# Mak-GIBA/research_image_retrieval

Measured on AMD Instinct MI355X. Metric: images embedded+ranked/sec on 1.6M×2048 gallery; mAP on ROxf/RPar, higher is better.
Workload: dtype fp32

## Files before the change

include/rr.h:

```cpp
#ifndef RR_H_
#define RR_H_

#include <stddef.h>
#include <stdint.h>

#ifdef __cplusplus
extern "C" {
#endif

#define RR_OK 0
#define RR_EINVAL (-1)
#define RR_EHIP (-2)
#define RR_EWORKSPACE (-3)
#define RR_EOVERFLOW (-4)

#define RR_AMAX_SLOTS 64

typedef struct rr_handle_s* rr_handle_t;

#define RR_ABI_VERSION 7
int rr_abi_version(void);

const char* rr_version(void);
int rr_create(int device, rr_handle_t* out);
int rr_destroy(rr_handle_t h);
const char* rr_last_error(rr_handle_t h);

int rr_timing_enable(rr_handle_t h, int enable);
int rr_timing_collect(rr_handle_t h, int cls, double* ms, long long* launches);

int rr_get_device(rr_handle_t h, int* device);

#define RR_TUNE_GEMM_CFG 1
#define RR_TUNE_GEMM_BK 2
#define RR_TUNE_LP_CFG 3
#define RR_TUNE_S3_CFG 4
#define RR_TUNE_S3_STAGGER 5
#define RR_TUNE_SWEEP_MF16 8
#define RR_TUNE_SWEEP_IL 9
#define RR_TUNE_CONV_IL 10
#define RR_TUNE_HALO_MF 11
#define RR_TUNE_S3_CFG_RES 13
#define RR_TUNE_SWEEP_FORM 14
#define RR_TUNE_HALO_2D 15
int rr_set_tuning(rr_handle_t h, int key, int value);

size_t rr_cosine_topk_workspace_size(int nq, long long n, int d, int k);
size_t rr_cosine_topk_workspace_size_cap(int nq, long long n, int d, int k, long long cap);
long long rr_cosine_topk_cap_for(int nq, long long n, int d, int k, size_t workspace_bytes);
size_t rr_cosine_topk_counts_offset(int nq, long long n, int d, int k);
size_t rr_cosine_topk_overflow_offset(int nq, long long n, int d, int k);
int rr_cosine_topk(rr_handle_t h, const float* queries, int nq,
                   const float* gallery, long long n, int d, int k,
                   long long idx_offset, float* out_scores, long long* out_idx,
                   void* workspace, size_t workspace_bytes, void* stream);

int rr_cosine_scores(rr_handle_t h, const float* queries, int nq,
                     const float* gallery, long long n, int d, float* scores,
                     void* stream);

int rr_topk_merge(rr_handle_t h, const float* part_scores,
                  const long long* part_idx, int nparts, int nq, int k_in,
                  int k_out, float* out_scores, long long* out_idx,
                  void* stream);

int rr_quantize_rows(rr_handle_t h, const float* x, long long rows, int d,
                     int dtype, void* y, float* row_scale, void* stream);

int rr_cosine_topk_lp(rr_handle_t h, const void* queries, const float* q_scale,
                      int nq, const void* gallery, const float* g_scale,
                      long long n, int d, int dtype, int k, long long idx_offset,
                      float* out_scores, long long* out_idx, void* workspace,
                      size_t workspace_bytes, void* stream);

int rr_alpha_qe(rr_handle_t h, const float* queries, int nq,
                const float* gallery, long long n_rows, int d, const long long* top_idx,
                const float* top_scores, int k, int n, float alpha,
                long long idx_offset, float* out, void* stream);

int rr_prefilter_gallery_bound(rr_handle_t h, const float* gallery,
                               const void* gallery_bf16, long long n, int d,
                               double* bound3, void* stream);
size_t rr_cosine_topk_prefilter_workspace_size(int nq, long long n, int d, int k);
size_t rr_cosine_topk_prefilter_counts_offset(int nq, long long n, int d, int k);
size_t rr_cosine_topk_prefilter_overflow_offset(int nq, long long n, int d, int k);
size_t rr_cosine_topk_prefilter_workspace_size_cap(int nq, long long n, int d, int k, long long cap);
long long rr_cosine_topk_prefilter_cap_for(int nq, long long n, int d, int k, size_t workspace_bytes);
int rr_cosine_topk_prefilter(rr_handle_t h, const float* queries, int nq,
                             const float* gallery, const void* gallery_bf16,
                             const double* bound3, long long n, int d, int k,
                             long long idx_offset, float* out_scores,
                             long long* out_idx, void* workspace,
                             size_t workspace_bytes, void* stream);

size_t rr_pcaw_gram_workspace_size(long long n, int d);
int rr_pcaw_gram(rr_handle_t h, const float* x, long long n, int d,
                 void* workspace, size_t workspace_bytes, double* mean_out,
                 double* gram_out, void* stream);

int rr_preprocess_u8(rr_handle_t h, const uint8_t* img_nhwc, int b, int hgt,
                     int wid, const float* mean3, const float* std3,
                     float* out_nhwc, void* stream);

int rr_preprocess_u8_ex(rr_handle_t h, const uint8_t* img_nhwc, int b, int hgt,
                        int wid, const float* mean3, const float* std3,
                        int out_c, float* out_nhwc, void* stream);

int rr_nchw_to_nhwc(rr_handle_t h, const float* in, int b, int c, int hgt,
                    int wid, float* out, void* stream);
int rr_nchw_to_nhwc_ex(rr_handle_t h, const float* in, int b, int c, int hgt,
                       int wid, int out_c, float* out, void* stream);

int rr_conv2d(rr_handle_t h, const float* x, int b, int hgt, int wid, int cin,
              const float* w, const float* bias, int cout, int kh, int kw,
              int stride, int pad, const float* residual, int relu, float* y,
              void* stream);

int rr_resize_bilinear(rr_handle_t h, const float* x, int b, int hgt, int wid,
                       int c, int out_h, int out_w, float inv_scale_h,
                       float inv_scale_w, float* y, void* stream);

int rr_conv2d_h2(rr_handle_t h, const float* x, const unsigned* x_amax, int b,
                 int hgt, int wid, int cin, const void* w2,
                 const float* w_iscale, const float* bias, int cout, int kh,
                 int kw, int stride, int pad, const float* residual, int relu,
                 float* y, unsigned* y_amax, void* stream);

int rr_bottleneck_out_h2(rr_handle_t h, const float* y, const unsigned* y_amax,
                         int b, int oh, int ow, int planes, const float* x,
                         const unsigned* x_amax, int hx, int wx, int cin,
                         int stride, const void* w2, const float* w_iscale,
                         const float* bias, int cout, float* out,
                         unsigned* out_amax, void* stream);

int rr_stem_pool_h2(rr_handle_t h, const float* x, const unsigned* x_amax,
                    int b, int hgt, int wid, const void* w2,
                    const float* w_iscale, const float* bias, int cout, int kh,
                    int kw, int stride, int pad, float* y_pool,
                    unsigned* y_amax, void* stream);

int rr_split2_f16(rr_handle_t h, const float* w, int rows, int k, int kpad,
                  void* planes, float* iscale, void* stream);

int rr_amax_f32(rr_handle_t h, const float* x, long long n, unsigned* amax,
                void* stream);

int rr_maxpool2d(rr_handle_t h, const float* x, int b, int hgt, int wid, int c,
                 int k, int stride, int pad, float* y, void* stream);

int rr_gem_pool(rr_handle_t h, const float* x, int b, int hw, int c, float p,
                float eps, float* out, void* stream);

int rr_linear(rr_handle_t h, const float* x, int m, int k, const float* w,
              const float* bias, int n, float* y, void* stream);

int rr_linear_ex(rr_handle_t h, const float* x, int m, int k, const float* w,
                 const float* bias, int n, const float* residual, int act,
                 float* y, void* stream);

int rr_linear_bf16(rr_handle_t h, const void* x, int m, int k, const void* w,
                   const float* bias, int n, const float* residual, int act,
                   int out_bf16, void* y, void* stream);

int rr_linear_bf16_ln(rr_handle_t h, const void* x, int m, int k, const void* w,
                      const float* bias, int n, const float* residual, int act,
                      int out_bf16, void* y, const float* stats_in,
                      const float* colsum, float eps, float* stats_out,
                      void* xb_out, void* stream);

int rr_ln_partials_bf16(rr_handle_t h, const float* x, int m, int d, void* xb,
                        float* stats, void* stream);

int rr_layernorm(rr_handle_t h, const float* x, long long ldx, int m, int d,
                 const float* gamma, const float* beta, float eps, float* y,
                 void* stream);

int rr_layernorm_ex(rr_handle_t h, const float* x, long long ldx, int m, int d,
                    const float* gamma, const float* beta, float eps,
                    int out_dtype, void* y, void* stream);

int rr_patchify(rr_handle_t h, const float* x, int b, int hgt, int wid, int c,
                int patch, float* y, void* stream);

int rr_patchify_ex(rr_handle_t h, const float* x, int b, int hgt, int wid,
                   int c, int patch, int out_dtype, void* y, void* stream);

int rr_vit_tokens(rr_handle_t h, const float* patches, int b, int npatch,
                  int width, const float* cls, const float* pos, float* y,
                  void* stream);

int rr_vit_tokens_ex(rr_handle_t h, const float* patches, int b, int npatch,
                     int width, const float* cls, const float* pos,
                     const float* gamma, const float* beta, float eps,
                     float* y, void* stream);

int rr_attention(rr_handle_t h, const float* qkv, int b, int seq, int heads,
                 int head_dim, float* out, void* stream);
int rr_attention_ex(rr_handle_t h, const float* qkv, int b, int seq, int heads,
                    int head_dim, int out_dtype, void* out, void* stream);

int rr_attention_bf16(rr_handle_t h, const float* qkv, int b, int seq, int heads,
                      int head_dim, int out_dtype, void* out, void* stream);
int rr_attention_bf16_qkv16(rr_handle_t h, const void* qkv_bf16, int b, int seq,
                            int heads, int head_dim, int out_dtype, void* out,
                            void* stream);

int rr_l2_normalize(rr_handle_t h, const float* x, int m, int d, float eps,
                    float* y, void* stream);

int rr_dolg_local_pool(rr_handle_t h, const float* y, int b, int hw, int c,
                       const float* w2, float b2, float* out, void* stream);

int rr_dolg_orth_fuse(rr_handle_t h, const float* fg, const float* m, int b,
                      int c, float* out, void* stream);

#ifdef __cplusplus
}
#endif
#endif
```

research_image_retrieval_amd/_lib.py:

```python
import ctypes
import os
import subprocess
import threading

_HERE = os.path.dirname(os.path.abspath(__file__))
LIB_PATH = os.environ.get("RR_LIB_PATH") or os.path.join(_HERE, "librr.so")
CSRC = os.path.join(_HERE, "csrc")

RR_OK, RR_EINVAL, RR_EHIP, RR_EWORKSPACE, RR_EOVERFLOW = 0, -1, -2, -3, -4
ABI_VERSION = 7
AMAX_SLOTS = 64

TIME_COSINE, TIME_GEMM, TIME_SELECT, TIME_ELEM, TIME_COSINE_SEED, TIME_ATTN = 0, 1, 2, 3, 4, 5
TUNE_GEMM_CFG, TUNE_GEMM_BK, TUNE_LP_CFG, TUNE_S3_CFG, TUNE_S3_STAGGER, \
    TUNE_SWEEP_MF16, TUNE_SWEEP_IL, TUNE_CONV_IL, TUNE_HALO_MF, TUNE_S3_CFG_RES, TUNE_SWEEP_FORM, TUNE_HALO_2D = \
    1, 2, 3, 4, 5, 8, 9, 10, 11, 13, 14, 15

_lib = None
_lock = threading.RLock()

_vp = ctypes.c_void_p
_i = ctypes.c_int
_ll = ctypes.c_longlong
_f = ctypes.c_float
_sz = ctypes.c_size_t

SIGNATURES = {
    "rr_version": (ctypes.c_char_p, []),
    "rr_abi_version": (_i, []),
    "rr_create": (_i, [_i, ctypes.POINTER(_vp)]),
    "rr_destroy": (_i, [_vp]),
    "rr_last_error": (ctypes.c_char_p, [_vp]),
    "rr_timing_enable": (_i, [_vp, _i]),
    "rr_timing_collect": (_i, [_vp, _i, ctypes.POINTER(ctypes.c_double), ctypes.POINTER(_ll)]),
    "rr_get_device": (_i, [_vp, ctypes.POINTER(_i)]),
    "rr_set_tuning": (_i, [_vp, _i, _i]),
    "rr_cosine_topk_workspace_size": (_sz, [_i, _ll, _i, _i]),
    "rr_cosine_topk_workspace_size_cap": (_sz, [_i, _ll, _i, _i, _ll]),
    "rr_cosine_topk_cap_for": (_ll, [_i, _ll, _i, _i, _sz]),
    "rr_cosine_topk_counts_offset": (_sz, [_i, _ll, _i, _i]),
    "rr_cosine_topk_overflow_offset": (_sz, [_i, _ll, _i, _i]),
    "rr_cosine_topk": (_i, [_vp, _vp, _i, _vp, _ll, _i, _i, _ll, _vp, _vp, _vp, _sz, _vp]),
    "rr_cosine_scores": (_i, [_vp, _vp, _i, _vp, _ll, _i, _vp, _vp]),
    "rr_topk_merge": (_i, [_vp, _vp, _vp, _i, _i, _i, _i, _vp, _vp, _vp]),
    "rr_preprocess_u8": (_i, [_vp, _vp, _i, _i, _i, _vp, _vp, _vp, _vp]),
    "rr_nchw_to_nhwc": (_i, [_vp, _vp, _i, _i, _i, _i, _vp, _vp]),
    "rr_preprocess_u8_ex": (_i, [_vp, _vp, _i, _i, _i, _vp, _vp, _i, _vp, _vp]),
    "rr_nchw_to_nhwc_ex": (_i, [_vp, _vp, _i, _i, _i, _i, _i, _vp, _vp]),
    "rr_conv2d": (_i, [_vp, _vp, _i, _i, _i, _i, _vp, _vp, _i, _i, _i, _i, _i, _vp, _i, _vp, _vp]),
    "rr_conv2d_h2": (_i, [_vp, _vp, _vp, _i, _i, _i, _i, _vp, _vp, _vp, _i, _i, _i, _i, _i, _vp, _i, _vp, _vp, _vp]),
    "rr_split2_f16": (_i, [_vp, _vp, _i, _i, _i, _vp, _vp, _vp]),
    "rr_stem_pool_h2": (_i, [_vp, _vp, _vp, _i, _i, _i, _vp, _vp, _vp, _i, _i, _i, _i, _i, _vp, _vp, _vp]),
    "rr_bottleneck_out_h2": (_i, [_vp, _vp, _vp, _i, _i, _i, _i, _vp, _vp, _i, _i, _i, _i, _vp, _vp, _vp, _i, _vp,
                                  _vp, _vp]),
    "rr_amax_f32": (_i, [_vp, _vp, _ll, _vp, _vp]),
    "rr_resize_bilinear": (_i, [_vp, _vp, _i, _i, _i, _i, _i, _i, _f, _f, _vp, _vp]),
    "rr_maxpool2d": (_i, [_vp, _vp, _i, _i, _i, _i, _i, _i, _i, _vp, _vp]),
    "rr_gem_pool": (_i, [_vp, _vp, _i, _i, _i, _f, _f, _vp, _vp]),
    "rr_linear": (_i, [_vp, _vp, _i, _i, _vp, _vp, _i, _vp, _vp]),
    "rr_l2_normalize": (_i, [_vp, _vp, _i, _i, _f, _vp, _vp]),
    "rr_dolg_local_pool": (_i, [_vp, _vp, _i, _i, _i, _vp, _f, _vp, _vp]),
    "rr_dolg_orth_fuse": (_i, [_vp, _vp, _vp, _i, _i, _vp, _vp]),
    "rr_linear_ex": (_i, [_vp, _vp, _i, _i, _vp, _vp, _i, _vp, _i, _vp, _vp]),
    "rr_layernorm": (_i, [_vp, _vp, _ll, _i, _i, _vp, _vp, _f, _vp, _vp]),
    "rr_patchify": (_i, [_vp, _vp, _i, _i, _i, _i, _i, _vp, _vp]),
    "rr_vit_tokens": (_i, [_vp, _vp, _i, _i, _i, _vp, _vp, _vp, _vp]),
    "rr_patchify_ex": (_i, [_vp, _vp, _i, _i, _i, _i, _i, _i, _vp, _vp]),
    "rr_vit_tokens_ex": (_i, [_vp, _vp, _i, _i, _i, _vp, _vp, _vp, _vp, _f, _vp, _vp]),
    "rr_attention": (_i, [_vp, _vp, _i, _i, _i, _i, _vp, _vp]),
    "rr_attention_ex": (_i, [_vp, _vp, _i, _i, _i, _i, _i, _vp, _vp]),
    "rr_attention_bf16": (_i, [_vp, _vp, _i, _i, _i, _i, _i, _vp, _vp]),
    "rr_attention_bf16_qkv16": (_i, [_vp, _vp, _i, _i, _i, _i, _i, _vp, _vp]),
    "rr_layernorm_ex": (_i, [_vp, _vp, _ll, _i, _i, _vp, _vp, _f, _i, _vp, _vp]),
    "rr_linear_bf16": (_i, [_vp, _vp, _i, _i, _vp, _vp, _i, _vp, _i, _i, _vp, _vp]),
    "rr_linear_bf16_ln": (_i, [_vp, _vp, _i, _i, _vp, _vp, _i, _vp, _i, _i, _vp, _vp, _vp, _f, _vp, _vp, _vp]),
    "rr_ln_partials_bf16": (_i, [_vp, _vp, _i, _i, _vp, _vp, _vp]),
    "rr_alpha_qe": (_i, [_vp, _vp, _i, _vp, _ll, _i, _vp, _vp, _i, _i, _f, _ll, _vp, _vp]),
    "rr_prefilter_gallery_bound": (_i, [_vp, _vp, _vp, _ll, _i, _vp, _vp]),
    "rr_cosine_topk_prefilter_workspace_size": (_sz, [_i, _ll, _i, _i]),
    "rr_cosine_topk_prefilter_counts_offset": (_sz, [_i, _ll, _i, _i]),
    "rr_cosine_topk_prefilter_overflow_offset": (_sz, [_i, _ll, _i, _i]),
    "rr_cosine_topk_prefilter_workspace_size_cap": (_sz, [_i, _ll, _i, _i, _ll]),
    "rr_cosine_topk_prefilter_cap_for": (_ll, [_i, _ll, _i, _i, _sz]),
    "rr_cosine_topk_prefilter": (_i, [_vp, _vp, _i, _vp, _vp, _vp, _ll, _i, _i, _ll, _vp, _vp, _vp, _sz, _vp]),
    "rr_pcaw_gram_workspace_size": (_sz, [_ll, _i]),
    "rr_pcaw_gram": (_i, [_vp, _vp, _ll, _i, _vp, _sz, _vp, _vp, _vp]),
    "rr_quantize_rows": (_i, [_vp, _vp, _ll, _i, _i, _vp, _vp, _vp]),
    "rr_cosine_topk_lp": (_i, [_vp, _vp, _vp, _i, _vp, _vp, _ll, _i, _i, _i, _ll, _vp, _vp, _vp, _sz, _vp]),
}


class RRError(RuntimeError):
    pass


def build(force=False):
    if force or not os.path.exists(LIB_PATH):
        subprocess.run(["make", "-s", "-C", CSRC, "-j4"], check=True)


def lib():
    global _lib
    if _lib is not None:
        return _lib
    with _lock:
        if _lib is None:
            if not os.path.exists(LIB_PATH):
                raise RRError(
                    f"librr.so not found at {LIB_PATH}: build it with `make -C {CSRC}` "
                    "(there is deliberately no CPU/eager fallback)")
            L = ctypes.CDLL(LIB_PATH)
            for name, (res, args) in SIGNATURES.items():
                if os.environ.get("RR_LIB_PATH") and not hasattr(L, name):
                    continue
                fn = getattr(L, name)
                fn.restype = res
                fn.argtypes = args
            if not os.environ.get("RR_LIB_PATH") and L.rr_abi_version() != ABI_VERSION:
                raise RRError(f"librr.so ABI {L.rr_abi_version()} != {ABI_VERSION} this binding was written "
                              f"against: rebuild it with `make -C {CSRC}`")
            _lib = L
    return _lib


_handles = {}


def handle(device_index):
    h = _handles.get(device_index)
    if h is None:
        with _lock:
            h = _handles.get(device_index)
            if h is None:
                out = _vp()
                rc = lib().rr_create(int(device_index), ctypes.byref(out))
                if rc != RR_OK:
                    raise RRError(f"rr_create(device={device_index}) failed with {rc}")
                h = out.value
                _handles[device_index] = h
    return h


def check(rc, h, what):
    if rc != RR_OK:
        msg = lib().rr_last_error(h)
        raise RRError(f"{what} failed ({rc}): {msg.decode() if msg else ''}")
```

research_image_retrieval_amd/csrc/embed_ops.hip:

```cpp
#include "rr_internal.hpp"

namespace rr {

__global__ void preprocess_u8_kernel(const uint8_t* __restrict__ in, long long n_px, float m0, float m1, float m2,
                                     float s0, float s1, float s2, int out_c, float* __restrict__ out) {
  const long long stride = (long long)gridDim.x * blockDim.x;
  for (long long p = (long long)blockIdx.x * blockDim.x + threadIdx.x; p < n_px; p += stride) {
    const uint8_t* px = in + p * 3;
    const float r = ((float)px[0] / 255.0f - m0) / s0;
    const float g = ((float)px[1] / 255.0f - m1) / s1;
    const float b = ((float)px[2] / 255.0f - m2) / s2;
    if (out_c == 4) {
      *reinterpret_cast<float4*>(out + p * 4) = make_float4(r, g, b, 0.f);
    } else {
      float* o = out + p * 3;
      o[0] = r;
      o[1] = g;
      o[2] = b;
    }
  }
}

__global__ void nchw_to_nhwc_kernel(const float* __restrict__ in, int C, int CO, long long HW, long long total,
                                    float* __restrict__ out) {
  const long long stride = (long long)gridDim.x * blockDim.x;
  for (long long o = (long long)blockIdx.x * blockDim.x + threadIdx.x; o < total; o += stride) {
    const int c = (int)(o % CO);
    const long long t = o / CO;
    const long long hw = t % HW;
    const long long b = t / HW;
    out[o] = c < C ? in[(b * C + c) * HW + hw] : 0.f;
  }
}

__global__ void resize_bilinear_kernel(const float* __restrict__ x, int B, int H, int W, int C, int OH, int OW,
                                       float sh, float sw, float* __restrict__ y) {
  const long long total = (long long)B * OH * OW * C;
  const long long gstride = (long long)gridDim.x * blockDim.x;
  for (long long o = (long long)blockIdx.x * blockDim.x + threadIdx.x; o < total; o += gstride) {
    const int c = (int)(o % C);
    long long t = o / C;
    const int ow = (int)(t % OW);
    t /= OW;
    const int oh = (int)(t % OH);
    const int b = (int)(t / OH);
    float rh = sh * ((float)oh + 0.5f) - 0.5f;
    float rw = sw * ((float)ow + 0.5f) - 0.5f;
    rh = rh < 0.f ? 0.f : rh;
    rw = rw < 0.f ? 0.f : rw;
    const int h0 = (int)rh, w0 = (int)rw;
    const int h1 = h0 + (h0 < H - 1 ? 1 : 0), w1 = w0 + (w0 < W - 1 ? 1 : 0);
    const float lh1 = fminf(fmaxf(rh - (float)h0, 0.f), 1.f), lw1 = fminf(fmaxf(rw - (float)w0, 0.f), 1.f);
    const float lh0 = 1.f - lh1, lw0 = 1.f - lw1;
    const float* xb = x + (long long)b * H * W * C + c;
    const float v00 = xb[((long long)h0 * W + w0) * C], v01 = xb[((long long)h0 * W + w1) * C];
    const float v10 = xb[((long long)h1 * W + w0) * C], v11 = xb[((long long)h1 * W + w1) * C];
    y[o] = (v00 * lw0 + v01 * lw1) * lh0 + (v10 * lw0 + v11 * lw1) * lh1;
  }
}

__global__ __launch_bounds__(256) void maxpool4_row_kernel(const float* __restrict__ x, int H, int W, int C, int k,
                                                           int stride, int pad, int OH, int OW, float* __restrict__ y) {
  const int C4 = C >> 2;
  const int row = blockIdx.x;
  const int b = row / OH, oh = row - b * OH;
  const float* xb = x + (long long)b * H * W * C;
  float* yr = y + (long long)row * OW * C;
  const int n = OW * C4;
  for (int o = threadIdx.x; o < n; o += blockDim.x) {
    const int ow = o / C4, c4 = o - ow * C4;
    float4 m = make_float4(-__builtin_inff(), -__builtin_inff(), -__builtin_inff(), -__builtin_inff());
    for (int dh = 0; dh < k; ++dh) {
      const int ih = oh * stride - pad + dh;
      if ((unsigned)ih >= (unsigned)H) continue;
      const float* xr = xb + (long long)ih * W * C + c4 * 4;
      for (int dw = 0; dw < k; ++dw) {
        const int iw = ow * stride - pad + dw;
        if ((unsigned)iw >= (unsigned)W) continue;
        const float4 v = *reinterpret_cast<const float4*>(xr + iw * C);
        m.x = fmaxf(m.x, v.x);
        m.y = fmaxf(m.y, v.y);
        m.z = fmaxf(m.z, v.z);
        m.w = fmaxf(m.w, v.w);
      }
    }
    *reinterpret_cast<float4*>(yr + o * 4) = m;
  }
}

typedef float mp_f32x4 __attribute__((ext_vector_type(4)));
__global__ __launch_bounds__(256) void maxpool3s2_kernel(const float* __restrict__ x, int H, int W, int C, int OH,
                                                         int OW, float* __restrict__ y) {
  const int C4 = C >> 2;
  const int OH2 = (OH + 1) >> 1, OW2 = (OW + 1) >> 1;
  const int b = blockIdx.x / OH2, oh0 = 2 * (blockIdx.x - b * OH2);
  const float* xb = x + (long long)b * H * W * C;
  float* yb = y + (long long)b * OH * OW * C;
  const float ninf = -__builtin_inff();
  const int n = OW2 * C4;
  for (int o = threadIdx.x; o < n; o += blockDim.x) {
    const int owp = o / C4, c4 = o - owp * C4;
    const int ow0 = 2 * owp;
    mp_f32x4 m[2][2];
#pragma unroll
    for (int r = 0; r < 2; ++r)
#pragma unroll
      for (int q = 0; q < 2; ++q) m[r][q] = mp_f32x4{ninf, ninf, ninf, ninf};
#pragma unroll
    for (int dr = 0; dr < 5; ++dr) {
      const int ih = 2 * oh0 - 1 + dr;
      if ((unsigned)ih >= (unsigned)H) continue;
      const float* xr = xb + (long long)ih * W * C + c4 * 4;
      mp_f32x4 col[5];
#pragma unroll
      for (int dc = 0; dc < 5; ++dc) {
        const int iw = 2 * ow0 - 1 + dc;
        col[dc] = (unsigned)iw < (unsigned)W ? *reinterpret_cast<const mp_f32x4*>(xr + iw * C) : mp_f32x4{ninf, ninf, ninf, ninf};
      }
      mp_f32x4 p0, p1;
#pragma unroll
      for (int e = 0; e < 4; ++e) {
        p0[e] = fmaxf(fmaxf(col[0][e], col[1][e]), col[2][e]);
        p1[e] = fmaxf(fmaxf(col[2][e], col[3][e]), col[4][e]);
      }
#pragma unroll
      for (int e = 0; e < 4; ++e) {
        if (dr <= 2) {
          m[0][0][e] = fmaxf(m[0][0][e], p0[e]);
          m[0][1][e] = fmaxf(m[0][1][e], p1[e]);
        }
        if (dr >= 2) {
          m[1][0][e] = fmaxf(m[1][0][e], p0[e]);
          m[1][1][e] = fmaxf(m[1][1][e], p1[e]);
        }
      }
    }
#pragma unroll
    for (int r = 0; r < 2; ++r) {
      if (oh0 + r >= OH) continue;
#pragma unroll
      for (int q = 0; q < 2; ++q) {
        if (ow0 + q >= OW) continue;
        *reinterpret_cast<mp_f32x4*>(yb + ((long long)(oh0 + r) * OW + ow0 + q) * C + c4 * 4) = m[r][q];
      }
    }
  }
}

__global__ void maxpool4_kernel(const float* __restrict__ x, int B, int H, int W, int C, int k, int stride, int pad,
                                int OH, int OW, float* __restrict__ y) {
  const int C4 = C >> 2;
  const long long total = (long long)B * OH * OW * C4;
  const long long gstride = (long long)gridDim.x * blockDim.x;
  for (long long o = (long long)blockIdx.x * blockDim.x + threadIdx.x; o < total; o += gstride) {
    const int c4 = (int)(o % C4);
    long long t = o / C4;
    const int ow = (int)(t % OW);
    t /= OW;
    const int oh = (int)(t % OH);
    const int b = (int)(t / OH);
    float4 m = make_float4(-__builtin_inff(), -__builtin_inff(), -__builtin_inff(), -__builtin_inff());
    for (int dh = 0; dh < k; ++dh) {
      const int ih = oh * stride - pad + dh;
      if ((unsigned)ih >= (unsigned)H) continue;
      for (int dw = 0; dw < k; ++dw) {
        const int iw = ow * stride - pad + dw;
        if ((unsigned)iw >= (unsigned)W) continue;
        const float4 v = *reinterpret_cast<const float4*>(x + (((long long)b * H + ih) * W + iw) * C + c4 * 4);
        m.x = fmaxf(m.x, v.x);
        m.y = fmaxf(m.y, v.y);
        m.z = fmaxf(m.z, v.z);
        m.w = fmaxf(m.w, v.w);
      }
    }
    *reinterpret_cast<float4*>(y + o * 4) = m;
  }
}

__global__ void maxpool_kernel(const float* __restrict__ x, int B, int H, int W, int C, int k, int stride, int pad,
                               int OH, int OW, float* __restrict__ y) {
  const long long total = (long long)B * OH * OW * C;
  const long long gstride = (long long)gridDim.x * blockDim.x;
  for (long long o = (long long)blockIdx.x * blockDim.x + threadIdx.x; o < total; o += gstride) {
    const int c = (int)(o % C);
    long long t = o / C;
    const int ow = (int)(t % OW);
    t /= OW;
    const int oh = (int)(t % OH);
    const int b = (int)(t / OH);
    float m = -__builtin_inff();
    for (int dh = 0; dh < k; ++dh) {
      const int ih = oh * stride - pad + dh;
      if ((unsigned)ih >= (unsigned)H) continue;
      for (int dw = 0; dw < k; ++dw) {
        const int iw = ow * stride - pad + dw;
        if ((unsigned)iw >= (unsigned)W) continue;
        m = fmaxf(m, x[(((long long)b * H + ih) * W + iw) * C + c]);
      }
    }
    y[o] = m;
  }
}

__global__ void gem_kernel(const float* __restrict__ x, int B, int HW, int C, float p, float eps, int p_is_3,
                           float* __restrict__ out) {
  const long long total = (long long)B * C;
  const long long gstride = (long long)gridDim.x * blockDim.x;
  const float inv_p = 1.0f / p;
  for (long long o = (long long)blockIdx.x * blockDim.x + threadIdx.x; o < total; o += gstride) {
    const int c = (int)(o % C);
    const long long b = o / C;
    const float* xp = x + b * (long long)HW * C + c;
    float acc = 0.f;
    for (int i = 0; i < HW; ++i) {
      const float v = fmaxf(xp[(long long)i * C], eps);
      acc += p_is_3 ? (v * v) * v : powf(v, p);
    }
    out[o] = powf(acc / (float)HW, inv_p);
  }
}

__global__ __launch_bounds__(256) void l2norm_kernel(const float* __restrict__ x, int M, int D, float eps,
                                                     float* __restrict__ y) {
  const int wave = (blockIdx.x * blockDim.x + threadIdx.x) >> 6;
  const int lane = threadIdx.x & 63;
  if (wave >= M) return;
  const float* xr = x + (long long)wave * D;
  float* yr = y + (long long)wave * D;
  float ss = 0.f;
  for (int i = lane; i < D; i += 64) ss = fmaf(xr[i], xr[i], ss);
#pragma unroll
  for (int off = 32; off > 0; off >>= 1) ss += __shfl_xor(ss, off, 64);
  const float nrm = fmaxf(sqrtf(ss), eps);
  for (int i = lane; i < D; i += 64) yr[i] = xr[i] / nrm;
}

static dim3 grid_for(long long n, int block) {
  long long g = (n + block - 1) / block;
  if (g > 256 * 16) g = 256 * 16;
  if (g < 1) g = 1;
  return dim3((unsigned)g);
}

}

using namespace rr;

extern "C" int rr_preprocess_u8(rr_handle_t h, const uint8_t* img, int b, int hgt, int wid, const float* mean3,
                                const float* std3, float* out, void* stream) {
  return rr_preprocess_u8_ex(h, img, b, hgt, wid, mean3, std3, 3, out, stream);
}

extern "C" int rr_preprocess_u8_ex(rr_handle_t h, const uint8_t* img, int b, int hgt, int wid, const float* mean3,
                                   const float* std3, int out_c, float* out, void* stream) {
  RR_ENTRY(h);
  if (!img || !out || !mean3 || !std3 || b < 0 || hgt < 0 || wid < 0 || (out_c != 3 && out_c != 4) ||
      (out_c == 4 && ((uintptr_t)out & 15)))
    return set_error(h, RR_EINVAL, "rr_preprocess_u8: bad argument (out_c 3 or 4, 16-B aligned out)");
  const long long npx = (long long)b * hgt * wid;
  if (npx == 0) return RR_OK;
  hipStream_t s = (hipStream_t)stream;
  TimedLaunch tl(h, kTimeElem, s);
  hipLaunchKernelGGL(preprocess_u8_kernel, grid_for(npx, 256), dim3(256), 0, s, img, npx, mean3[0], mean3[1],
                     mean3[2], std3[0], std3[1], std3[2], out_c, out);
  return check_hip(h, hipGetLastError(), "preprocess launch");
}

extern "C" int rr_nchw_to_nhwc(rr_handle_t h, const float* in, int b, int c, int hgt, int wid, float* out,
                               void* stream) {
  return rr_nchw_to_nhwc_ex(h, in, b, c, hgt, wid, c, out, stream);
}

extern "C" int rr_nchw_to_nhwc_ex(rr_handle_t h, const float* in, int b, int c, int hgt, int wid, int out_c,
                                  float* out, void* stream) {
  RR_ENTRY(h);
  if (!in || !out || b < 0 || c <= 0 || hgt < 0 || wid < 0 || out_c < c)
    return set_error(h, RR_EINVAL, "rr_nchw_to_nhwc: bad argument");
  const long long total = (long long)b * out_c * hgt * wid;
  if (total == 0) return RR_OK;
  hipStream_t s = (hipStream_t)stream;
  TimedLaunch tl(h, kTimeElem, s);
  hipLaunchKernelGGL(nchw_to_nhwc_kernel, grid_for(total, 256), dim3(256), 0, s, in, c, out_c, (long long)hgt * wid,
                     total, out);
  return check_hip(h, hipGetLastError(), "nchw_to_nhwc launch");
}

extern "C" int rr_maxpool2d(rr_handle_t h, const float* x, int b, int hgt, int wid, int c, int k, int stride, int pad,
                            float* y, void* stream) {
  RR_ENTRY(h);
  if (!x || !y || b < 0 || c <= 0 || k <= 0 || stride <= 0 || pad < 0 || 2 * pad > k)
    return set_error(h, RR_EINVAL, "rr_maxpool2d: bad argument");
  const int oh = (hgt + 2 * pad - k) / stride + 1, ow = (wid + 2 * pad - k) / stride + 1;
  if (oh <= 0 || ow <= 0) return set_error(h, RR_EINVAL, "rr_maxpool2d: empty output");
  const long long total = (long long)b * oh * ow * c;
  if (total == 0) return RR_OK;
  hipStream_t s = (hipStream_t)stream;
  TimedLaunch tl(h, kTimeElem, s);
  const bool vec = (c & 3) == 0 && ((uintptr_t)x & 15) == 0 && ((uintptr_t)y & 15) == 0;
  if (vec && k == 3 && stride == 2 && pad == 1 && (long long)b * ((oh + 1) / 2) <= 0x7fffffffLL &&
      (long long)wid * c < 0x7fffffffLL)
    hipLaunchKernelGGL(maxpool3s2_kernel, dim3((unsigned)((long long)b * ((oh + 1) / 2))), dim3(256), 0, s, x, hgt,
                       wid, c, oh, ow, y);
  else if (vec && (long long)b * oh <= 0x7fffffffLL && (long long)wid * c < 0x7fffffffLL)
    hipLaunchKernelGGL(maxpool4_row_kernel, dim3((unsigned)((long long)b * oh)), dim3(256), 0, s, x, hgt, wid, c, k,
                       stride, pad, oh, ow, y);
  else if (vec)
    hipLaunchKernelGGL(maxpool4_kernel, grid_for(total / 4, 256), dim3(256), 0, s, x, b, hgt, wid, c, k, stride, pad,
                       oh, ow, y);
  else
    hipLaunchKernelGGL(maxpool_kernel, grid_for(total, 256), dim3(256), 0, s, x, b, hgt, wid, c, k, stride, pad, oh,
                       ow, y);
  return check_hip(h, hipGetLastError(), "maxpool launch");
}

extern "C" int rr_gem_pool(rr_handle_t h, const float* x, int b, int hw, int c, float p, float eps, float* out,
                           void* stream) {
  RR_ENTRY(h);
  if (!x || !out || b < 0 || hw <= 0 || c <= 0 || !(p > 0.f)) return set_error(h, RR_EINVAL, "rr_gem_pool: bad argument");
  const long long total = (long long)b * c;
  if (total == 0) return RR_OK;
  hipStream_t s = (hipStream_t)stream;
  TimedLaunch tl(h, kTimeElem, s);
  hipLaunchKernelGGL(gem_kernel, grid_for(total, 256), dim3(256), 0, s, x, b, hw, c, p, eps, p == 3.0f ? 1 : 0, out);
  return check_hip(h, hipGetLastError(), "gem launch");
}

extern "C" int rr_l2_normalize(rr_handle_t h, const float* x, int m, int d, float eps, float* y, void* stream) {
  RR_ENTRY(h);
  if (!x || !y || m < 0 || d <= 0) return set_error(h, RR_EINVAL, "rr_l2_normalize: bad argument");
  if (m == 0) return RR_OK;
  hipStream_t s = (hipStream_t)stream;
  TimedLaunch tl(h, kTimeElem, s);
  const long long threads = (long long)m * 64;
  hipLaunchKernelGGL(l2norm_kernel, dim3((unsigned)((threads + 255) / 256)), dim3(256), 0, s, x, m, d, eps, y);
  return check_hip(h, hipGetLastError(), "l2norm launch");
}

extern "C" int rr_resize_bilinear(rr_handle_t h, const float* x, int b, int hgt, int wid, int c, int out_h, int out_w,
                                  float inv_scale_h, float inv_scale_w, float* y, void* stream) {
  RR_ENTRY(h);
  if (!x || !y || b < 0 || hgt <= 0 || wid <= 0 || c <= 0 || out_h <= 0 || out_w <= 0)
    return set_error(h, RR_EINVAL, "rr_resize_bilinear: bad argument");
  const float sh = inv_scale_h > 0.f ? inv_scale_h : (float)hgt / (float)out_h;
  const float sw = inv_scale_w > 0.f ? inv_scale_w : (float)wid / (float)out_w;
  const long long total = (long long)b * out_h * out_w * c;
  if (total == 0) return RR_OK;
  hipStream_t s = (hipStream_t)stream;
  TimedLaunch tl(h, kTimeElem, s);
  hipLaunchKernelGGL(resize_bilinear_kernel, grid_for(total, 256), dim3(256), 0, s, x, b, hgt, wid, c, out_h, out_w, sh,
                     sw, y);
  return check_hip(h, hipGetLastError(), "resize launch");
}

namespace rr {
__global__ __launch_bounds__(256) void alpha_qe_kernel(const float* __restrict__ q, const float* __restrict__ g,
                                                       const long long* __restrict__ idx,
                                                       const float* __restrict__ sc, int k, int n, int d,
                                                       float alpha, long long idx_offset, long long n_rows,
                                                       float* __restrict__ out) {
  __shared__ float red[256 / 64];
  const int qi = blockIdx.x;
  const int d4 = d >> 2;
  float ss = 0.f;
  for (int c = threadIdx.x; c < d4; c += 256) {
    float4 acc = reinterpret_cast<const float4*>(q + (long long)qi * d)[c];
    for (int r = 0; r < n; ++r) {
      const long long j = idx[(long long)qi * k + r] - idx_offset;
      if (j < 0 || j >= n_rows) continue;
      const float s = sc[(long long)qi * k + r];
      const float w = s > 0.f ? powf(s, alpha) : 0.f;
      const float4 v = reinterpret_cast<const float4*>(g + j * d)[c];
      acc.x = fmaf(w, v.x, acc.x);
      acc.y = fmaf(w, v.y, acc.y);
      acc.z = fmaf(w, v.z, acc.z);
      acc.w = fmaf(w, v.w, acc.w);
    }
    reinterpret_cast<float4*>(out + (long long)qi * d)[c] = acc;
    ss = fmaf(acc.x, acc.x, fmaf(acc.y, acc.y, fmaf(acc.z, acc.z, fmaf(acc.w, acc.w, ss))));
  }
#pragma unroll
  for (int off = 32; off > 0; off >>= 1) ss += __shfl_xor(ss, off, 64);
  if ((threadIdx.x & 63) == 0) red[threadIdx.x >> 6] = ss;
  __syncthreads();
  const float tot = red[0] + red[1] + red[2] + red[3];
  const float inv = 1.0f / fmaxf(sqrtf(tot), 1e-12f);
  for (int c = threadIdx.x; c < d4; c += 256) {
    float4 v = reinterpret_cast<float4*>(out + (long long)qi * d)[c];
    v.x *= inv;
    v.y *= inv;
    v.z *= inv;
    v.w *= inv;
    reinterpret_cast<float4*>(out + (long long)qi * d)[c] = v;
  }
}
}

extern "C" int rr_alpha_qe(rr_handle_t h, const float* queries, int nq, const float* gallery, long long n_rows,
                           int d, const long long* top_idx, const float* top_scores, int k, int n, float alpha,
                           long long idx_offset, float* out, void* stream) {
  RR_ENTRY(h);
  if (!queries || !top_idx || !top_scores || !out || nq < 0 || n_rows < 0 || (n_rows > 0 && !gallery) || d <= 0 ||
      (d & 3) || k <= 0 || n < 0 ||
      n > k || ((uintptr_t)queries & 15) || ((uintptr_t)gallery & 15) || ((uintptr_t)out & 15))
    return set_error(h, RR_EINVAL, "rr_alpha_qe: bad argument (d % 4 == 0, 0 <= n <= k, 16-B aligned rows)");
  if (nq == 0) return RR_OK;
  hipStream_t s = (hipStream_t)stream;
  TimedLaunch tl(h, kTimeElem, s);
  hipLaunchKernelGGL(alpha_qe_kernel, dim3((unsigned)nq), dim3(256), 0, s, queries, gallery, top_idx, top_scores, k,
                     n, d, alpha, idx_offset, n_rows, out);
  return check_hip(h, hipGetLastError(), "alpha_qe launch");
}
```

research_image_retrieval_amd/csrc/h2_dispatch.hip:

```cpp
#include <algorithm>

#include "gemm_epilogue.hpp"
#include "rr_internal.hpp"

namespace rr {

static int pick_s3(const GemmArgs& g, int forced) {
  if (forced >= 1 && forced <= 8) return forced;
  if ((g.N % 256) == 0) return 4;
  auto cost = [&](long long bm, long long bn, long long per_cu, double speed) {
    const long long slots = 256 * per_cu;
    const long long t = ((g.M + bm - 1) / bm) * ((g.N + bn - 1) / bn);
    return (double)((t + slots - 1) / slots) * bm * bn * per_cu / speed;
  };
  double best = cost(128, 128, 2, 1.0);
  int cfg = 1;
  if (cost(256, 128, 1, 1.15) < best) best = cost(256, 128, 1, 1.15), cfg = 3;
  if (cost(256, 64, 2, 1.0) < best) best = cost(256, 64, 2, 1.0), cfg = 7;
  return cfg;
}
static int pick_h2(const GemmArgs& g, int forced) {
  if (forced == 9) return (g.N % 256) == 0 ? 9 : pick_h2(g, 0);
  if (forced == 10) return (g.N % 256) == 0 ? 10 : pick_h2(g, 0);
  if (forced == 11) return (g.N % 128) == 0 ? 11 : pick_h2(g, 0);
  if (forced == 12) return (g.N % 256) == 0 ? 12 : pick_h2(g, 0);
  if (forced == 0 && g.N == 128) return 11;
  int cfg = pick_s3(g, forced);
  if (cfg == 3 || cfg == 4 || cfg == 7 || cfg == 8) return cfg;
  cfg = pick_s3(g, 0);
  if (cfg == 1) cfg = (g.N % 128) == 0 ? 3 : 7;
  return cfg;
}

static bool s3_persist_ok(const GemmArgs& g, int amode) { return (g.N % 256) == 0 && amode == A_DENSE; }

static hipError_t launch_h2_am(int am, const GemmArgs& g, hipStream_t s, int forced, int n_cu, int st) {
  const bool hpers = forced == 0;
  if (am == A_DENSE && (forced == 15 || forced == 0) && s3q_shape(g) && !s3q_fits(g)) {
    const long long per = ((1LL << 32) - 1) / (4LL * std::max(g.lda, g.ldc)) / 256 * 256;
    if (per >= 256) {
      for (long long m0 = 0; m0 < g.M; m0 += per) {
        GemmArgs c = g;
        c.M = (int)std::min<long long>(per, g.M - m0);
        c.A = g.A + m0 * g.lda;
        c.C = g.C + m0 * g.ldc;
        if (g.residual != nullptr) c.residual = g.residual + m0 * g.ldc;
        if (const hipError_t e = launch_h2_am(am, c, s, forced, n_cu, st)) return e;
      }
      return hipSuccess;
    }
  }
  if (forced == 15 || forced == 0) {
    if (am == A_DENSE && s3q_shape(g) && s3q_fits(g)) return launch_s3q(g, s, n_cu, st);
    if (forced == 15) forced = 0;
  }
  if (am == A_CONV) {
    if (forced == 0 && g.halo_2d != 0 && h2_halo_2d_ok(g) && (g.halo_2d == 1 || !h2_halo_rows(g)))
      return launch_h2_halo_2d(g, s);
    if (forced == 13 || forced == 14 || (forced == 0 && ((g.N % 256) == 0 || g.N == 64 || g.N == 128))) {
      if (const int hr = h2_halo_rows(g))
        return launch_h2_halo(g, s, hr,
                              forced == 14 ? 1 : forced == 13 ? 0 : g.halo_mf >= 0 ? g.halo_mf : (hr == 288 || hr == 320 ? 1 : 0),
                              hpers, n_cu);
    }
  }
  if (forced == 13 || forced == 14) forced = 0;
  int cfg = pick_h2(g, forced);
  const bool big = (g.N % 256) == 0 && g.K >= 256;
  if (forced == 0 && big) cfg = 12;
  else if (forced == 0 && s3_persist_ok(g, am)) cfg = 8;
  if (cfg == 8) {
    if (s3_persist_ok(g, am)) return launch_s3p(g, s, n_cu, st);
    cfg = pick_h2(g, 0);
  }
  return launch_h2_tile(cfg, am, g, s, n_cu, st);
}

int launch_gemm_s3(rr_handle_s* h, int amode, const GemmArgs& g, hipStream_t s, int timer_cls) {
  if (g.M < 0 || g.N <= 0 || g.K <= 0) return set_error(h, RR_EINVAL, "gemm_s3: bad shape");
  if (g.K % 32) return set_error(h, RR_EINVAL, "gemm_s3: K must be a multiple of 32");
  if (amode == A_DENSE && ((g.lda & 3) || ((uintptr_t)g.A & 15)))
    return set_error(h, RR_EINVAL, "gemm_s3: dense A needs lda % 4 == 0 and 16-B alignment");
  if (amode == A_CONV && (g.Cin % 32)) return set_error(h, RR_EINVAL, "gemm_s3: conv A needs Cin % 32 == 0");
  if (amode == A_CONV_C4 && (g.Cin != 4 || g.K < g.KH * g.KW * 4 || ((uintptr_t)g.A & 15)))
    return set_error(h, RR_EINVAL, "gemm_s3: NHWC4 A needs Cin == 4, K >= KH*KW*4, 16-B alignment");
  if (amode != A_DENSE && amode != A_CONV && amode != A_CONV_C4)
    return set_error(h, RR_EINVAL, "gemm_s3: unsupported A mode");
  if ((g.ldb & 7) || (g.b_plane & 7) || ((uintptr_t)g.B & 15))
    return set_error(h, RR_EINVAL, "gemm_s3: B planes need ldb % 8 == 0, plane stride % 8 == 0, 16-B alignment");
  if (g.col_scale == nullptr || g.a_amax == nullptr || ((uintptr_t)g.col_scale & 15))
    return set_error(h, RR_EINVAL, "gemm_h2: needs 16-B aligned column scales and the A max-|x| record");
  if (g.relu == 2 || g.out_bf16 || (g.N & 3) || (g.ldc & 3))
    return set_error(h, RR_EINVAL, "gemm_h2: fp32 output, ReLU or none, N % 4 == 0");
  if (g.M == 0) return RR_OK;
  const int st = h->tune.s3_stagger >= 0 ? h->tune.s3_stagger : (g.residual != nullptr ? 8 : 0);
  hipError_t e;
  {
    TimedLaunch tl(h, timer_cls, s);
    const int f = (g.residual != nullptr && h->tune.s3_cfg_res > 0) ? h->tune.s3_cfg_res : h->tune.s3_cfg;
    const int n_cu = device_cu_count(h);
    {
      GemmArgs g2 = g;
      g2.issue_spread = h->tune.conv_il == 1;
      g2.halo_mf = h->tune.halo_mf;
      g2.halo_2d = h->tune.halo_2d;
      e = launch_h2_am(amode, g2, s, f, n_cu, st);
    }
  }
  return check_hip(h, e, "gemm_h2 launch");
}

__global__ __launch_bounds__(256) void split2h_kernel(const float* __restrict__ w, int rows, int k, int kpad,
                                                      uint16_t* __restrict__ planes, float* __restrict__ iscale) {
  __shared__ float red[4];
  const int n = blockIdx.x, tid = threadIdx.x;
  const float* wr = w + (long long)n * k;
  float am = 0.f;
  for (int i = tid; i < k; i += 256) am = amax_acc(am, wr[i]);
#pragma unroll
  for (int o = 32; o > 0; o >>= 1) am = fmaxf(am, __shfl_xor(am, o));
  if ((tid & 63) == 0) red[tid >> 6] = am;
  __syncthreads();
  am = fmaxf(fmaxf(red[0], red[1]), fmaxf(red[2], red[3]));
  const int e = h2_exp(am);
  const float sc = __builtin_amdgcn_ldexpf(1.f, e);
  if (tid == 0) iscale[n] = __builtin_amdgcn_ldexpf(1.f, -e);
  const long long plane = (long long)rows * kpad;
  uint16_t* p0 = planes + (long long)n * kpad;
  for (int i = tid; i < kpad; i += 256) {
    const float v = i < k ? wr[i] * sc : 0.f;
    const _Float16 hi = (_Float16)v;
    const _Float16 lo = (_Float16)(v - (float)hi);
    p0[i] = __builtin_bit_cast(uint16_t, hi);
    p0[plane + i] = __builtin_bit_cast(uint16_t, lo);
  }
}

int launch_split2h(rr_handle_s* h, const float* w, int rows, int k, int kpad, uint16_t* planes, float* iscale,
                   hipStream_t s) {
  if (rows <= 0) return RR_OK;
  hipLaunchKernelGGL(split2h_kernel, dim3((unsigned)rows), dim3(256), 0, s, w, rows, k, kpad, planes, iscale);
  return check_hip(h, hipGetLastError(), "split2h launch");
}

__global__ __launch_bounds__(256) void amax_kernel(const float* __restrict__ x, long long n, uint32_t* slots) {
  float am = 0.f;
  const long long gs = (long long)gridDim.x * blockDim.x;
  const long long i0 = (long long)blockIdx.x * blockDim.x + threadIdx.x;
  if (((uintptr_t)x & 15) == 0) {
    const long long n4 = n >> 2;
    const f32x4* x4 = reinterpret_cast<const f32x4*>(x);
    for (long long i = i0; i < n4; i += gs) {
      const f32x4 v = x4[i];
      am = amax_acc(amax_acc(am, v[0]), v[1]);
      am = amax_acc(amax_acc(am, v[2]), v[3]);
    }
    for (long long i = (n4 << 2) + i0; i < n; i += gs) am = amax_acc(am, x[i]);
  } else {
    for (long long i = i0; i < n; i += gs) am = amax_acc(am, x[i]);
  }
  amax_publish(slots, am, blockIdx.x * 4 + (threadIdx.x >> 6));
}

int launch_amax(rr_handle_s* h, const float* x, long long n, uint32_t* slots, hipStream_t s) {
  if (n <= 0) return RR_OK;
  const long long blocks = std::min<long long>((n / 4 + 255) / 256 + 1, 2048);
  hipLaunchKernelGGL(amax_kernel, dim3((unsigned)blocks), dim3(256), 0, s, x, n, slots);
  return check_hip(h, hipGetLastError(), "amax launch");
}

#if RR_S3_PHASES
int h2_tile_phases(unsigned long long* out);
int h2_stream_phases(unsigned long long* out);
int h2_stream256_phases(unsigned long long* out);
int h2_halo_phases(unsigned long long* out);
#endif

}

#if RR_S3_PHASES
extern "C" int rr_debug_phases(unsigned long long* out) {
  if (const int e = rr::h2_tile_phases(out)) return e;
  if (const int e = rr::h2_stream_phases(out + 8)) return e;
  if (const int e = rr::h2_stream256_phases(out + 16)) return e;
  return rr::h2_halo_phases(out + 24);
}
#endif
```

research_image_retrieval_amd/csrc/h2_stem.hip:

```cpp
#include <algorithm>

#include "h2_common.hpp"

namespace rr {

template <int EPI, int NW = 8, int BREG = 0>
__global__ __launch_bounds__(64 * NW, 1) void stem_pool_halo_kernel(GemmArgs g, int ntiles) {
  constexpr int NT = 64 * NW, BN = 64, HR = 39, HC = 35, HP = HR * HC;
  constexpr int WR = BREG ? 64 : 256 / NW, FM = WR / 32;
  constexpr int JN = BREG ? 1 : 2;
  static_assert(NW == 8 || (NW == 4 && !BREG), "8 waves of 32 rows or 4 of 64");
  constexpr int HS = 36, HPS = HR * HS;
  constexpr int KP = 224, BS = KP + 8;
  constexpr int NKS = 13;
  constexpr int B_U16 = BREG == 1 ? 0 : 2 * BN * BS;
  constexpr int A_U16 = 2 * (HPS + 1) * 4;
  constexpr int CS = BN + 4;
  constexpr int C_U16 = 256 * CS * 2;
  constexpr int A_PASS = (HP + NT - 1) / NT;
  constexpr int C4 = BN / 4, NPOOL = 56 * C4;
  constexpr int QI = (NPOOL + NT - 1) / NT;
  constexpr int PS = NKS / QI;
  __shared__ __attribute__((aligned(16))) uint16_t lds[B_U16 + A_U16 + C_U16];
  uint16_t* lb = lds;
  uint16_t* la = lds + B_U16;
  float* ct = reinterpret_cast<float*>(lds + B_U16 + A_U16);
  typedef f16x8 frag_t;
  typedef _Float16 f16x4 __attribute__((ext_vector_type(4)));

  const int tid = threadIdx.x, lane = tid & 63, wave = tid >> 6;
  const int lr = lane & 31, lh = lane >> 5;
  const int wrg = BREG ? wave % 4 : wave, wn = BREG ? wave / 4 : 0;
  const uint32_t a_amax_w = amax_load_slot(g.a_amax);
  float a_sc, a_isc;
  {
    uint32_t u = a_amax_w;
    const int lo = s3_opaque(lane);
#pragma unroll
    for (int o = 32; o > 0; o >>= 1) {
      const uint32_t v = (uint32_t)__builtin_amdgcn_ds_bpermute((lo ^ o) << 2, (int)u);
      u = v > u ? v : u;
    }
    const int e = __builtin_amdgcn_readfirstlane(h2_exp(__uint_as_float(u)));
    a_sc = __int_as_float((127 + e) << 23);
    a_isc = __int_as_float((127 - e) << 23);
  }

  constexpr int BRP = BREG == 1 ? 2 : 1;
  frag_t breg[BREG ? NKS : 1][BRP];
  if constexpr (BREG != 0) {
    const uint16_t* Bp = reinterpret_cast<const uint16_t*>(g.B) + (long long)(32 * wn + lr) * g.ldb + 8 * lh;
#pragma unroll
    for (int ks = 0; ks < NKS; ++ks)
#pragma unroll
      for (int p = 0; p < BRP; ++p) breg[ks][p] = *reinterpret_cast<const frag_t*>(Bp + p * g.b_plane + 16 * ks);
  }
  if constexpr (BREG != 1) {
    const uint16_t* Bp = reinterpret_cast<const uint16_t*>(g.B);
    for (int i = tid; i < 2 * BN * (KP / 8); i += NT) {
      const int row = i / (KP / 8), c8 = i - row * (KP / 8);
      const int p = row / BN, n = row - p * BN;
      *reinterpret_cast<u32x4*>(lb + row * BS + c8 * 8) =
          *reinterpret_cast<const u32x4*>(Bp + p * g.b_plane + (long long)n * g.ldb + c8 * 8);
    }
  }

  const int tpi = g.pool_tr * g.pool_tc;
  f32x4 px[A_PASS];
  auto load_patch = [&](int tl) {
    const int b = tl / tpi, t2 = tl - b * tpi, pr = t2 / g.pool_tc, pc = t2 - pr * g.pool_tc;
#pragma unroll
    for (int q = 0; q < A_PASS; ++q) {
      const int p = tid + q * NT, hr = p / HC, hc = p - hr * HC;
      const int ih = 32 * pr - 5 + hr, iw = 28 * pc - 5 + hc;
      const bool ok = tl < ntiles && p < HP && (unsigned)ih < (unsigned)g.H && (unsigned)iw < (unsigned)g.W;
      const f32x4* src = ok ? reinterpret_cast<const f32x4*>(g.A + (((long long)b * g.H + ih) * g.W + iw) * 4)
                            : s3_zero_page();
      asm volatile("global_load_dwordx4 %0, %1, off" : "=&v"(px[q]) : "v"(src) : "memory");
    }
  };
  auto store_patch = [&]() {
    asm volatile("s_waitcnt vmcnt(0)" ::: "memory");
#pragma unroll
    for (int q = 0; q < A_PASS; ++q) {
      asm volatile("" : "+v"(px[q]));
      const int p = tid + q * NT, hr = p / HC, hc = p - hr * HC;
      const int slot = hr * HS + (hc & 1) * (HS / 2) + (hc >> 1);
      const f32x4 v = px[q] * a_sc;
      const f16x4 hi = __builtin_convertvector(v, f16x4);
      const f16x4 lo = __builtin_convertvector(v - __builtin_convertvector(hi, f32x4), f16x4);
      if (p < HP) {
        *reinterpret_cast<f16x4*>(la + slot * 4) = hi;
        *reinterpret_cast<f16x4*>(la + (HPS + 1) * 4 + slot * 4) = lo;
      }
    }
    if (tid < 2) *reinterpret_cast<uint2*>(la + tid * (HPS + 1) * 4 + HPS * 4) = uint2{0u, 0u};
  };

  int sbase[FM];
#pragma unroll
  for (int i = 0; i < FM; ++i) {
    const int row = wrg * WR + 32 * i + lr, rq = row / 15, rc = row - rq * 15;
    sbase[i] = row < 255 ? (2 * rq) * HS + rc : -1;
  }

  float am = 0.f;
  auto pool_item = [&](int tl, int it) __attribute__((always_inline)) {
    const int b = tl / tpi, t2 = tl - b * tpi, pr = t2 / g.pool_tc, pc = t2 - pr * g.pool_tc;
    const int qd = it / C4, c4 = it - qd * C4, pi = qd / 7, pj = qd - 7 * pi;
    const int ph = 8 * pr + pi, pw = 7 * pc + pj;
    if (ph >= g.POH || pw >= g.POW) return;
    f32x4 mx = {-__builtin_inff(), -__builtin_inff(), -__builtin_inff(), -__builtin_inff()};
#pragma unroll
    for (int dr = -1; dr <= 1; ++dr)
#pragma unroll
      for (int dc = -1; dc <= 1; ++dc) {
        const int oh = 2 * ph + dr, ow = 2 * pw + dc;
        if ((unsigned)oh >= (unsigned)g.OH || (unsigned)ow >= (unsigned)g.OW) continue;
        const f32x4 v = *reinterpret_cast<const f32x4*>(ct + ((2 * pi + dr + 1) * 15 + 2 * pj + dc + 1) * CS + c4 * 4);
#pragma unroll
        for (int e = 0; e < 4; ++e) mx[e] = __builtin_fmaxf(mx[e], v[e]);
      }
    const f32x4 sc = *reinterpret_cast<const f32x4*>(g.col_scale + c4 * 4) * a_isc;
    const f32x4 bv = g.bias != nullptr ? *reinterpret_cast<const f32x4*>(g.bias + c4 * 4) : f32x4{0.f, 0.f, 0.f, 0.f};
    f32x4 o;
#pragma unroll
    for (int e = 0; e < 4; ++e) {
      o[e] = __builtin_fmaxf(mx[e] * sc[e] + bv[e], 0.f);
      am = amax_acc(am, o[e]);
    }
    *reinterpret_cast<f32x4*>(g.pool_out + (((long long)b * g.POH + ph) * g.POW + pw) * BN + c4 * 4) = o;
  };

  const int G = gridDim.x;
  int tl = blockIdx.x;
  int prev = -1;
  load_patch(tl);
  store_patch();
  __syncthreads();
  for (; tl < ntiles; tl += G) {
    load_patch(tl + G);
    f32x16 hi[FM][JN], lo[FM][JN];
#pragma unroll
    for (int i = 0; i < FM; ++i)
#pragma unroll
      for (int j = 0; j < JN; ++j)
#pragma unroll
        for (int r = 0; r < 16; ++r) hi[i][j][r] = lo[i][j][r] = 0.f;
#pragma unroll
    for (int ks = 0; ks < NKS; ++ks) {
      frag_t a[2][FM], b[2][2];
      const int t0 = 4 * ks + 2 * lh;
#pragma unroll
      for (int i = 0; i < FM; ++i) {
        int pix[2];
#pragma unroll
        for (int u = 0; u < 2; ++u) {
          const int t = t0 + u, kh = t / 7, kw = t - kh * 7;
          pix[u] = (sbase[i] >= 0 && t < 49) ? sbase[i] + kh * HS + (kw & 1) * (HS / 2) + (kw >> 1) : HPS;
        }
#pragma unroll
        for (int p = 0; p < 2; ++p) {
          const uint16_t* pl = la + p * (HPS + 1) * 4;
          const f16x4 x0 = *reinterpret_cast<const f16x4*>(pl + pix[0] * 4);
          const f16x4 x1 = *reinterpret_cast<const f16x4*>(pl + pix[1] * 4);
          a[p][i] = __builtin_shufflevector(x0, x1, 0, 1, 2, 3, 4, 5, 6, 7);
        }
      }
#pragma unroll
      for (int p = 0; p < 2; ++p)
#pragma unroll
        for (int j = 0; j < JN; ++j)
          b[p][j] = (BREG == 1 || (BREG == 2 && p == 0))
                        ? breg[ks][BREG == 1 ? p : 0]
                        : *reinterpret_cast<const frag_t*>(lb + (p * BN + 32 * (j + wn) + lr) * BS + 16 * ks + 8 * lh);
#pragma unroll
      for (int i = 0; i < FM; ++i)
#pragma unroll
        for (int j = 0; j < JN; ++j) hi[i][j] = s3_mf32(a[0][i], b[0][j], hi[i][j]);
#pragma unroll
      for (int i = 0; i < FM; ++i)
#pragma unroll
        for (int j = 0; j < JN; ++j) {
          lo[i][j] = s3_mf32(a[0][i], b[1][j], lo[i][j]);
          lo[i][j] = s3_mf32(a[1][i], b[0][j], lo[i][j]);
        }
      if (prev >= 0) {
#pragma unroll
        for (int q = 0; q < QI; ++q)
          if (ks == q * PS + PS / 2 && tid + q * NT < NPOOL) pool_item(prev, tid + q * NT);
      }
    }
    __syncthreads();
#pragma unroll
    for (int i = 0; i < FM; ++i)
#pragma unroll
      for (int j = 0; j < JN; ++j)
#pragma unroll
        for (int r = 0; r < 16; ++r)
          ct[(wrg * WR + 32 * i + acc_row<false>(0, r, lane)) * CS + 32 * wn + acc_col<false>(j, r, lane)] =
              hi[i][j][r] + lo[i][j][r];
    store_patch();
    prev = tl;
    __syncthreads();
  }
  if (prev >= 0) {
#pragma unroll
    for (int q = 0; q < QI; ++q)
      if (tid + q * NT < NPOOL) pool_item(prev, tid + q * NT);
  }
  asm volatile("s_waitcnt vmcnt(0)" ::: "memory");
  if constexpr ((EPI & EP_AMAX) != 0) {
    if (g.c_amax != nullptr) amax_publish(g.c_amax, am, blockIdx.x * NW + wave);
  }
}

int launch_stem_pool_h2(rr_handle_s* h, const GemmArgs& g, hipStream_t s, int timer_cls) {
  if (g.N != 64 || g.Cin != 4 || g.K % 32 || g.K < g.KH * g.KW * 4 || g.relu != 1 || g.residual != nullptr ||
      g.col_scale == nullptr || g.a_amax == nullptr || g.pool_out == nullptr || g.POH <= 0 || g.POW <= 0 ||
      g.pool_tr != (g.POH + 7) / 8 || g.pool_tc != (g.POW + 6) / 7 || ((uintptr_t)g.A & 15) || (g.ldb & 7) ||
      (g.b_plane & 7) || ((uintptr_t)g.B & 15) || ((uintptr_t)g.col_scale & 15) || ((uintptr_t)g.pool_out & 15))
    return set_error(h, RR_EINVAL, "stem_pool_h2: NHWC4 input, 64 output channels, ReLU, aligned operands");
  GemmArgs q = g;
  const long long tiles = (long long)(g.M / ((long long)g.OH * g.OW)) * g.pool_tr * g.pool_tc;
  if (tiles * 256 > 0x7fffffffLL) return set_error(h, RR_EINVAL, "stem_pool_h2: too many tiles");
  if (tiles == 0) return RR_OK;
  q.M = (int)(tiles * 256);
  hipError_t e;
  {
    TimedLaunch tl(h, timer_cls, s);
    if (h->tune.s3_cfg != 7 && g.KH == 7 && g.KW == 7 && g.stride == 2 && g.pad == 3 && g.K == 224 && g.ldb == 224) {
      const int grid = (int)std::min<long long>(tiles, device_cu_count(h));
      hipLaunchKernelGGL((stem_pool_halo_kernel<H2_EP | EP_RELU, 8, 2>), dim3((unsigned)grid), dim3(512), 0, s, g, (int)tiles);
      e = hipGetLastError();
    } else {
      e = launch_h2_tile_stem_pool(q, s, device_cu_count(h));
    }
  }
  return check_hip(h, e, "stem_pool_h2 launch");
}

}
```

research_image_retrieval_amd/csrc/rr_api.hip:

```cpp
#include <algorithm>
#include <cstring>
#include <initializer_list>

#include "gemm_epilogue.hpp"
#include "rr_internal.hpp"

namespace rr {

int set_error(rr_handle_s* h, int code, const std::string& msg) {
  if (h) h->last_error = msg;
  return code;
}

int check_hip(rr_handle_s* h, hipError_t e, const char* what) {
  if (e == hipSuccess) return RR_OK;
  return set_error(h, RR_EHIP, std::string(what) + ": " + hipGetErrorString(e));
}

TimedLaunch::TimedLaunch(rr_handle_s* h_, int cls_, hipStream_t s_) : h(h_), cls(cls_), s(s_) {
  if (!h || !h->timing || cls < 0 || cls >= rr_handle_s::kClasses) return;
  const int i = h->n_ev[cls];
  if (i >= (int)h->ev_start[cls].size()) {
    hipEvent_t a = nullptr, b = nullptr;
    if (hipEventCreate(&a) != hipSuccess) return;
    if (hipEventCreate(&b) != hipSuccess) {
      (void)hipEventDestroy(a);
      return;
    }
    h->ev_start[cls].push_back(a);
    h->ev_stop[cls].push_back(b);
  }
  if (hipEventRecord(h->ev_start[cls][i], s) != hipSuccess) return;
  slot = i;
}

TimedLaunch::~TimedLaunch() {
  if (slot < 0) return;
  if (hipEventRecord(h->ev_stop[cls][slot], s) == hipSuccess) h->n_ev[cls] = slot + 1;
}

static long long seed_rows(long long n, int k) { return seed_sample_rows(n, k); }

static inline size_t align256(size_t x) { return (x + 255) & ~(size_t)255; }

struct TopkWs {
  long long s, ld, cap;
  size_t off_scores, off_tau, off_cnt, off_ovf, off_cand, total;
};

static TopkWs topk_layout(int nq, long long n, int k, long long cap = -1) {
  TopkWs w{};
  w.s = seed_rows(n, k);
  w.ld = (w.s + 3) & ~3LL;
  w.cap = k + (n - w.s);
  if (cap >= 0 && cap < w.cap) w.cap = cap;
  size_t o = 0;
  w.off_scores = o;
  o = align256(o + (size_t)nq * w.ld * 4);
  w.off_tau = o;
  o = align256(o + (size_t)nq * 4);
  w.off_cnt = o;
  o = align256(o + (size_t)nq * 4);
  w.off_ovf = o;
  o = align256(o + 4);
  w.off_cand = o;
  o = align256(o + (size_t)nq * w.cap * 8);
  w.total = o;
  return w;
}

}

using namespace rr;

extern "C" {

const char* rr_version(void) { return "librr 0.4.0 (gfx950: fp32 / f16x2 / bf16 / fp8 MFMA)"; }

int rr_abi_version(void) { return RR_ABI_VERSION; }

int rr_create(int device, rr_handle_t* out) {
  if (!out) return RR_EINVAL;
  *out = nullptr;
  int ndev = 0;
  if (hipGetDeviceCount(&ndev) != hipSuccess || device < 0 || device >= ndev) return RR_EHIP;
  rr_handle_s* h = new (std::nothrow) rr_handle_s();
  if (!h) return RR_EINVAL;
  h->device = device;
  *out = h;
  return RR_OK;
}

int rr_destroy(rr_handle_t h) {
  RR_ENTRY(h);
  for (int c = 0; c < rr_handle_s::kClasses; ++c)
    for (size_t i = 0; i < h->ev_start[c].size(); ++i) {
      (void)hipEventDestroy(h->ev_start[c][i]);
      (void)hipEventDestroy(h->ev_stop[c][i]);
    }
  dolg_slab_release(h);
  delete h;
  return RR_OK;
}

const char* rr_last_error(rr_handle_t h) { return h ? h->last_error.c_str() : "null handle"; }

int rr_timing_enable(rr_handle_t h, int enable) {
  RR_ENTRY(h);
  h->timing = enable != 0;
  for (int c = 0; c < rr_handle_s::kClasses; ++c) {
    h->n_ev[c] = 0;
    h->acc_ms[c] = 0;
    h->acc_launches[c] = 0;
  }
  return RR_OK;
}

int rr_get_device(rr_handle_t h, int* device) {
  if (!h || !device) return RR_EINVAL;
  *device = h->device;
  return RR_OK;
}

int rr_set_tuning(rr_handle_t h, int key, int value) {
  if (!h) return RR_EINVAL;
  auto in = [&](std::initializer_list<int> ok) {
    for (int v : ok)
      if (v == value) return true;
    return false;
  };
  switch (key) {
    case RR_TUNE_GEMM_CFG:
      if (!in({0, 22, 41, 88})) break;
      h->tune.gemm_cfg = value;
      return RR_OK;
    case RR_TUNE_GEMM_BK:
      if (!in({0, 16, 32})) break;
      h->tune.gemm_bk = value;
      return RR_OK;
    case RR_TUNE_LP_CFG:
      if (value < 0 || value > 6) break;
      h->tune.lp_cfg = value;
      return RR_OK;
    case RR_TUNE_S3_CFG:
      if (value < 0 || value > 15) break;
      h->tune.s3_cfg = value;
      return RR_OK;
    case RR_TUNE_S3_STAGGER:
      if (value < -1 || value > 200) break;
      h->tune.s3_stagger = value;
      return RR_OK;
    case RR_TUNE_SWEEP_MF16:
      if (!in({-1, 0, 1})) break;
      h->tune.sweep_mf16 = value;
      return RR_OK;
    case RR_TUNE_SWEEP_IL:
      if (!in({-1, 0, 1})) break;
      h->tune.sweep_il = value;
      return RR_OK;
    case RR_TUNE_CONV_IL:
      if (!in({-1, 0, 1})) break;
      h->tune.conv_il = value;
      return RR_OK;
    case RR_TUNE_HALO_MF:
      if (!in({-1, 0, 1, 2, 3, 4})) break;
      h->tune.halo_mf = value;
      return RR_OK;
    case RR_TUNE_S3_CFG_RES:
      if (value < 0 || value > 15) break;
      h->tune.s3_cfg_res = value;
      return RR_OK;
    case RR_TUNE_SWEEP_FORM:
      if (!in({-1, 0, 1, 2})) break;
      h->tune.sweep_form = value;
      return RR_OK;
    case RR_TUNE_HALO_2D:
      if (!in({-1, 0, 1})) break;
      h->tune.halo_2d = value;
      return RR_OK;
    default:
      return set_error(h, RR_EINVAL, "rr_set_tuning: unknown key");
  }
  return set_error(h, RR_EINVAL, "rr_set_tuning: value out of range for this key");
}

int rr_timing_collect(rr_handle_t h, int cls, double* ms, long long* launches) {
  if (!h || cls < 0 || cls >= rr_handle_s::kClasses) return RR_EINVAL;
  DeviceGuard dg(h);
  for (int i = 0; i < h->n_ev[cls]; ++i) {
    if (int rc = check_hip(h, hipEventSynchronize(h->ev_stop[cls][i]), "timing sync")) return rc;
    float t = 0.f;
    if (int rc = check_hip(h, hipEventElapsedTime(&t, h->ev_start[cls][i], h->ev_stop[cls][i]), "timing elapsed"))
      return rc;
    h->acc_ms[cls] += t;
    h->acc_launches[cls] += 1;
  }
  h->n_ev[cls] = 0;
  if (ms) *ms = h->acc_ms[cls];
  if (launches) *launches = h->acc_launches[cls];
  h->acc_ms[cls] = 0;
  h->acc_launches[cls] = 0;
  return RR_OK;
}

size_t rr_cosine_topk_workspace_size(int nq, long long n, int d, int k) {
  (void)d;
  if (nq <= 0 || k <= 0) return 256;
  return topk_layout(nq, n > 0 ? n : 1, k).total;
}

size_t rr_cosine_topk_workspace_size_cap(int nq, long long n, int d, int k, long long cap) {
  (void)d;
  if (nq <= 0 || k <= 0 || cap < k) return 0;
  return topk_layout(nq, n > 0 ? n : 1, k, cap).total;
}

long long rr_cosine_topk_cap_for(int nq, long long n, int d, int k, size_t workspace_bytes) {
  (void)d;
  if (nq <= 0 || k <= 0) return 0;
  const TopkWs L = topk_layout(nq, n > 0 ? n : 1, k);
  return workspace_bytes >= L.total ? L.cap : cap_that_fits(L.off_cand, nq, workspace_bytes, L.cap);
}

size_t rr_cosine_topk_counts_offset(int nq, long long n, int d, int k) {
  (void)d;
  if (nq <= 0 || k <= 0) return 0;
  return topk_layout(nq, n > 0 ? n : 1, k).off_cnt;
}

size_t rr_cosine_topk_overflow_offset(int nq, long long n, int d, int k) {
  (void)d;
  if (nq <= 0 || k <= 0) return 0;
  return topk_layout(nq, n > 0 ? n : 1, k).off_ovf;
}

}

namespace rr {
static int cosine_topk_impl(rr_handle_t h, const void* queries, const float* q_scale, int nq, const void* gallery,
                            const float* g_scale, long long n, int d, int k, long long idx_offset, float* out_scores,
                            long long* out_idx, void* workspace, size_t workspace_bytes, hipStream_t s, int dt) {
  if (nq < 0 || n < 0 || d <= 0 || (d & 3) || k < 1 || k > 16384)
    return set_error(h, RR_EINVAL, "rr_cosine_topk: need nq,n >= 0, d % 4 == 0, 1 <= k <= 16384");
  if (n >= 0xffffffffLL) return set_error(h, RR_EINVAL, "rr_cosine_topk: gallery shard must have < 2^32 rows");
  if (nq == 0) return RR_OK;
  if (!queries || !out_scores || !out_idx || (n > 0 && !gallery))
    return set_error(h, RR_EINVAL, "rr_cosine_topk: null pointer");
  if (((uintptr_t)queries & 15) || ((uintptr_t)gallery & 15))
    return set_error(h, RR_EINVAL, "rr_cosine_topk: queries/gallery must be 16-byte aligned");
  const int es = dt == DT_F32 ? 4 : (dt == DT_BF16 ? 2 : 1);
  TopkWs L = topk_layout(nq, n > 0 ? n : 1, k);
  if (workspace && workspace_bytes < L.total) {
    const long long cap = cap_that_fits(L.off_cand, nq, workspace_bytes, L.cap);
    if (cap >= k) L = topk_layout(nq, n > 0 ? n : 1, k, cap);
  }
  if (!workspace || workspace_bytes < L.total)
    return set_error(h, RR_EWORKSPACE,
                     "rr_cosine_topk: workspace too small (at least rr_cosine_topk_workspace_size_cap(..., k))");
  char* ws = (char*)workspace;
  float* scores_t = (float*)(ws + L.off_scores);
  float* tau = (float*)(ws + L.off_tau);
  int* cnt = (int*)(ws + L.off_cnt);
  int* ovf = (int*)(ws + L.off_ovf);
  unsigned long long* cand = (unsigned long long*)(ws + L.off_cand);
  if (int rc = check_hip(h, hipMemsetAsync(ovf, 0, 4, s), "memset")) return rc;
  if (n == 0) {
    if (int rc = check_hip(h, hipMemsetAsync(cnt, 0, (size_t)nq * 4, s), "memset")) return rc;
    return launch_select_final(h, cand, L.cap, cnt, nq, k, idx_offset, out_scores, out_idx, ovf, s);
  }
  GemmArgs g;
  g.A = (const float*)gallery;
  g.lda = d;
  g.M = (int)L.s;
  g.K = d;
  g.B = (const float*)queries;
  g.ldb = d;
  g.N = nq;
  g.C = scores_t;
  g.ldc = L.ld;
  g.scale_a = g_scale;
  g.scale_b = q_scale;
  if (int rc = launch_gemm(h, A_DENSE, E_SCORES_T, g, s, kTimeCosineSeed, dt)) return rc;
  if (int rc = launch_select_dense_seed(h, scores_t, L.ld, (int)L.s, nq, k, 0, cand, L.cap, cnt, tau, s)) return rc;
  long long done = L.s;
  while (done < n) {
    const long long rows = std::min<long long>(n - done, 0x7fffff00LL);
    GemmArgs f;
    f.A = (const float*)((const char*)gallery + done * d * es);
    f.lda = d;
    f.M = (int)rows;
    f.K = d;
    f.B = (const float*)queries;
    f.ldb = d;
    f.N = nq;
    f.tau = tau;
    f.cand = cand;
    f.cnt = cnt;
    f.cap = L.cap;
    f.row_offset = done;
    f.scale_a = g_scale ? g_scale + done : nullptr;
    f.scale_b = q_scale;
    if (int rc = launch_gemm(h, A_DENSE, E_FILTER, f, s, kTimeCosine, dt)) return rc;
    done += rows;
  }
  return launch_select_final(h, cand, L.cap, cnt, nq, k, idx_offset, out_scores, out_idx, ovf, s);
}
}

extern "C" {

int rr_cosine_topk(rr_handle_t h, const float* queries, int nq, const float* gallery, long long n, int d, int k,
                   long long idx_offset, float* out_scores, long long* out_idx, void* workspace,
                   size_t workspace_bytes, void* stream) {
  RR_ENTRY(h);
  return cosine_topk_impl(h, queries, nullptr, nq, gallery, nullptr, n, d, k, idx_offset, out_scores, out_idx,
                          workspace, workspace_bytes, (hipStream_t)stream, DT_F32);
}

int rr_cosine_topk_lp(rr_handle_t h, const void* queries, const float* q_scale, int nq, const void* gallery,
                      const float* g_scale, long long n, int d, int dtype, int k, long long idx_offset,
                      float* out_scores, long long* out_idx, void* workspace, size_t workspace_bytes,
                      void* stream) {
  RR_ENTRY(h);
  if (dtype != DT_BF16 && dtype != DT_FP8) return set_error(h, RR_EINVAL, "rr_cosine_topk_lp: dtype must be 1 or 2");
  if (dtype == DT_FP8 && (!q_scale || !g_scale))
    return set_error(h, RR_EINVAL, "rr_cosine_topk_lp: fp8 needs per-row scales");
  if ((d % (dtype == DT_BF16 ? 8 : 16)) != 0)
    return set_error(h, RR_EINVAL, "rr_cosine_topk_lp: rows must be multiples of 16 bytes");
  return cosine_topk_impl(h, queries, q_scale, nq, gallery, g_scale, n, d, k, idx_offset, out_scores, out_idx,
                          workspace, workspace_bytes, (hipStream_t)stream, dtype);
}

int rr_linear_bf16(rr_handle_t h, const void* x, int m, int k, const void* w, const float* bias, int n,
                   const float* residual, int act, int out_bf16, void* y, void* stream) {
  RR_ENTRY(h);
  if (!x || !w || !y || m < 0 || k <= 0 || n <= 0 || (k & 7) || act < 0 || act > 2)
    return set_error(h, RR_EINVAL, "rr_linear_bf16: bad argument (k % 8 == 0)");
  if (((uintptr_t)x & 15) || ((uintptr_t)w & 15)) return set_error(h, RR_EINVAL, "rr_linear_bf16: 16-B alignment");
  GemmArgs g;
  g.A = (const float*)x;
  g.lda = k;
  g.M = m;
  g.K = k;
  g.B = (const float*)w;
  g.ldb = k;
  g.N = n;
  g.C = (float*)y;
  g.ldc = n;
  g.bias = bias;
  g.residual = residual;
  g.relu = act;
  g.out_bf16 = out_bf16 ? 1 : 0;
  return launch_gemm(h, A_DENSE, E_STORE, g, (hipStream_t)stream, kTimeGemm, DT_BF16);
}

int rr_linear_bf16_ln(rr_handle_t h, const void* x, int m, int k, const void* w, const float* bias, int n,
                      const float* residual, int act, int out_bf16, void* y, const float* stats_in,
                      const float* colsum, float eps, float* stats_out, void* xb_out, void* stream) {
  RR_ENTRY(h);
  if (!x || !w || !y || m < 0 || k <= 0 || n <= 0 || (k & 7) || act < 0 || act > 2)
    return set_error(h, RR_EINVAL, "rr_linear_bf16_ln: bad argument (k % 8 == 0)");
  if (((uintptr_t)x & 15) || ((uintptr_t)w & 15) || ((uintptr_t)y & 15) || (bias && ((uintptr_t)bias & 15)) ||
      (residual && ((uintptr_t)residual & 15)))
    return set_error(h, RR_EINVAL, "rr_linear_bf16_ln: 16-B alignment");
  if ((stats_in == nullptr) == (stats_out == nullptr))
    return set_error(h, RR_EINVAL, "rr_linear_bf16_ln: exactly one of stats_in (fold) and stats_out (produce)");
  if (stats_out) {
    if (!xb_out || !residual || !bias || act != 0 || out_bf16 || (n % 256) || (k % 64) || ((uintptr_t)xb_out & 15) ||
        ((uintptr_t)stats_out & 7))
      return set_error(h, RR_EINVAL,
                       "rr_linear_bf16_ln: stats_out needs bias, residual, fp32 output, n % 256 == 0, k % 64 == 0");
  } else {
    if (!colsum || !bias || residual || !out_bf16 || (k % 64) || k > 256 * LN_TMAX || (n & 3) ||
        ((uintptr_t)colsum & 15) || !(eps >= 0.f))
      return set_error(h, RR_EINVAL,
                       "rr_linear_bf16_ln: stats_in needs colsum, bias, bf16 output, k % 64 == 0, k <= 768");
  }
  if (m == 0) return RR_OK;
  GemmArgs g;
  g.A = (const float*)x;
  g.lda = k;
  g.M = m;
  g.K = k;
  g.B = (const float*)w;
  g.ldb = k;
  g.N = n;
  g.C = (float*)y;
  g.ldc = n;
  g.bias = bias;
  g.residual = residual;
  g.relu = act;
  g.out_bf16 = out_bf16 ? 1 : 0;
  g.stats_out = stats_out;
  g.c2 = (uint16_t*)xb_out;
  g.stats_in = stats_in;
  g.colsum = colsum;
  g.stats_k = k;
  g.ln_eps = eps;
  return launch_gemm(h, A_DENSE, E_STORE, g, (hipStream_t)stream, kTimeGemm, DT_BF16);
}

int rr_cosine_scores(rr_handle_t h, const float* queries, int nq, const float* gallery, long long n, int d,
                     float* scores, void* stream) {
  RR_ENTRY(h);
  if (nq < 0 || n < 0 || n > 0x7fffffffLL || d <= 0 || (d & 3))
    return set_error(h, RR_EINVAL, "rr_cosine_scores: bad shape");
  if (nq == 0 || n == 0) return RR_OK;
  if (!queries || !gallery || !scores) return set_error(h, RR_EINVAL, "rr_cosine_scores: null pointer");
  GemmArgs g;
  g.A = gallery;
  g.lda = d;
  g.M = (int)n;
  g.K = d;
  g.B = queries;
  g.ldb = d;
  g.N = nq;
  g.C = scores;
  g.ldc = nq;
  return launch_gemm(h, A_DENSE, E_STORE, g, (hipStream_t)stream, kTimeCosineSeed);
}

int rr_topk_merge(rr_handle_t h, const float* ps, const long long* pi, int nparts, int nq, int k_in, int k_out,
                  float* os, long long* oi, void* stream) {
  RR_ENTRY(h);
  if (!ps || !pi || !os || !oi) return set_error(h, RR_EINVAL, "rr_topk_merge: null pointer");
  return launch_merge(h, ps, pi, nparts, nq, k_in, k_out, os, oi, (hipStream_t)stream);
}

int rr_conv2d(rr_handle_t h, const float* x, int b, int hgt, int wid, int cin, const float* w, const float* bias,
              int cout, int kh, int kw, int stride, int pad, const float* residual, int relu, float* y,
              void* stream) {
  RR_ENTRY(h);
  if (!x || !w || !y || b < 0 || hgt <= 0 || wid <= 0 || cin <= 0 || cout <= 0 || kh <= 0 || kw <= 0 ||
      stride <= 0 || pad < 0)
    return set_error(h, RR_EINVAL, "rr_conv2d: bad argument");
  const int oh = (hgt + 2 * pad - kh) / stride + 1, ow = (wid + 2 * pad - kw) / stride + 1;
  if (oh <= 0 || ow <= 0) return set_error(h, RR_EINVAL, "rr_conv2d: empty output");
  const long long M = (long long)b * oh * ow;
  if (M > 0x7fffffffLL) return set_error(h, RR_EINVAL, "rr_conv2d: too many output pixels");
  GemmArgs g;
  g.A = x;
  g.M = (int)M;
  g.K = kh * kw * cin;
  g.H = hgt;
  g.W = wid;
  g.Cin = cin;
  g.OH = oh;
  g.OW = ow;
  g.KH = kh;
  g.KW = kw;
  g.stride = stride;
  g.pad = pad;
  g.B = w;
  g.ldb = g.K;
  g.N = cout;
  g.C = y;
  g.ldc = cout;
  g.bias = bias;
  g.residual = residual;
  g.relu = relu;
  int amode;
  if (kh == 1 && kw == 1 && stride == 1 && pad == 0 && (cin & 3) == 0) {
    amode = A_DENSE;
    g.lda = cin;
  } else if (cin % 32 == 0) {
    amode = A_CONV;
  } else if (cin == 4) {
    amode = A_CONV_C4;
  } else {
    amode = A_CONV_GENERIC;
  }
  if (amode != A_CONV_GENERIC && (((uintptr_t)x & 15) || ((uintptr_t)w & 15)))
    return set_error(h, RR_EINVAL, "rr_conv2d: x/w must be 16-byte aligned");
  if ((cout & 3) == 0 && (((uintptr_t)y & 15) || (bias && ((uintptr_t)bias & 15)) || (residual && ((uintptr_t)residual & 15))))
    return set_error(h, RR_EINVAL, "rr_conv2d: bias/residual/y must be 16-byte aligned");
  return launch_gemm(h, amode, E_STORE, g, (hipStream_t)stream, kTimeGemm);
}

int rr_conv2d_h2(rr_handle_t h, const float* x, const unsigned* x_amax, int b, int hgt, int wid, int cin,
                 const void* w2, const float* w_iscale, const float* bias, int cout, int kh, int kw, int stride,
                 int pad, const float* residual, int relu, float* y, unsigned* y_amax, void* stream) {
  RR_ENTRY(h);
  if (!x || !x_amax || !w2 || !w_iscale || !y || b < 0 || hgt <= 0 || wid <= 0 || cin <= 0 || cout <= 0 ||
      kh <= 0 || kw <= 0 || stride <= 0 || pad < 0 || relu < 0 || relu > 1)
    return set_error(h, RR_EINVAL, "rr_conv2d_h2: bad argument");
  if (cin % 32 && cin != 4) return set_error(h, RR_EINVAL, "rr_conv2d_h2: cin must be a multiple of 32, or 4 (NHWC4 stem)");
  if (cout % 4) return set_error(h, RR_EINVAL, "rr_conv2d_h2: cout must be a multiple of 4");
  const int oh = (hgt + 2 * pad - kh) / stride + 1, ow = (wid + 2 * pad - kw) / stride + 1;
  if (oh <= 0 || ow <= 0) return set_error(h, RR_EINVAL, "rr_conv2d_h2: empty output");
  const long long M = (long long)b * oh * ow;
  if (M > 0x7fffffffLL) return set_error(h, RR_EINVAL, "rr_conv2d_h2: too many output pixels");
  if (((uintptr_t)x & 15) || ((uintptr_t)w2 & 15) || ((uintptr_t)w_iscale & 15) || ((uintptr_t)y & 15) ||
      (bias && ((uintptr_t)bias & 15)) || (residual && ((uintptr_t)residual & 15)))
    return set_error(h, RR_EINVAL, "rr_conv2d_h2: x/w2/w_iscale/bias/residual/y must be 16-byte aligned");
  GemmArgs g;
  g.A = x;
  g.M = (int)M;
  g.K = kh * kw * cin;
  g.H = hgt;
  g.W = wid;
  g.Cin = cin;
  g.OH = oh;
  g.OW = ow;
  g.KH = kh;
  g.KW = kw;
  g.stride = stride;
  g.pad = pad;
  if (cin == 4) g.K = (g.K + 31) / 32 * 32;
  g.B = reinterpret_cast<const float*>(w2);
  g.ldb = g.K;
  g.b_plane = (long long)cout * g.K;
  g.N = cout;
  g.C = y;
  g.ldc = cout;
  g.bias = bias;
  g.residual = residual;
  g.relu = relu;
  g.col_scale = w_iscale;
  g.a_amax = x_amax;
  g.c_amax = y_amax;
  const bool dense = kh == 1 && kw == 1 && stride == 1 && pad == 0 && cin != 4;
  if (dense) g.lda = cin;
  return launch_gemm_s3(h, dense ? A_DENSE : (cin == 4 ? A_CONV_C4 : A_CONV), g, (hipStream_t)stream, kTimeGemm);
}

int rr_stem_pool_h2(rr_handle_t h, const float* x, const unsigned* x_amax, int b, int hgt, int wid, const void* w2,
                    const float* w_iscale, const float* bias, int cout, int kh, int kw, int stride, int pad,
                    float* y_pool, unsigned* y_amax, void* stream) {
  RR_ENTRY(h);
  if (!x || !x_amax || !w2 || !w_iscale || !y_pool || b < 0 || hgt <= 0 || wid <= 0 || kh <= 0 || kw <= 0 ||
      stride <= 0 || pad < 0)
    return set_error(h, RR_EINVAL, "rr_stem_pool_h2: bad argument");
  if (cout != 64) return set_error(h, RR_EINVAL, "rr_stem_pool_h2: cout must be 64");
  const int oh = (hgt + 2 * pad - kh) / stride + 1, ow = (wid + 2 * pad - kw) / stride + 1;
  if (oh <= 0 || ow <= 0) return set_error(h, RR_EINVAL, "rr_stem_pool_h2: empty output");
  const int ph = (oh - 1) / 2 + 1, pw = (ow - 1) / 2 + 1;
  if ((long long)b * oh * ow > 0x7fffffffLL || (long long)b * ph * pw * cout > (1LL << 40))
    return set_error(h, RR_EINVAL, "rr_stem_pool_h2: too many output pixels");
  if (((uintptr_t)x & 15) || ((uintptr_t)w2 & 15) || ((uintptr_t)w_iscale & 15) || ((uintptr_t)y_pool & 15) ||
      (bias && ((uintptr_t)bias & 15)))
    return set_error(h, RR_EINVAL, "rr_stem_pool_h2: x/w2/w_iscale/bias/y_pool must be 16-byte aligned");
  GemmArgs g;
  g.A = x;
  g.M = (int)((long long)b * oh * ow);
  g.K = (kh * kw * 4 + 31) / 32 * 32;
  g.H = hgt;
  g.W = wid;
  g.Cin = 4;
  g.OH = oh;
  g.OW = ow;
  g.KH = kh;
  g.KW = kw;
  g.stride = stride;
  g.pad = pad;
  g.B = reinterpret_cast<const float*>(w2);
  g.ldb = g.K;
  g.b_plane = (long long)cout * g.K;
  g.N = cout;
  g.ldc = cout;
  g.bias = bias;
  g.relu = 1;
  g.col_scale = w_iscale;
  g.a_amax = x_amax;
  g.c_amax = y_amax;
  g.pool_out = y_pool;
  g.POH = ph;
  g.POW = pw;
  g.pool_tr = (ph + 7) / 8;
  g.pool_tc = (pw + 6) / 7;
  return launch_stem_pool_h2(h, g, (hipStream_t)stream, kTimeGemm);
}

int rr_bottleneck_out_h2(rr_handle_t h, const float* y, const unsigned* y_amax, int b, int oh, int ow, int planes,
                         const float* x, const unsigned* x_amax, int hx, int wx, int cin, int stride, const void* w2,
                         const float* w_iscale, const float* bias, int cout, float* out, unsigned* out_amax,
                         void* stream) {
  RR_ENTRY(h);
  if (!y || !y_amax || !x || !x_amax || !w2 || !w_iscale || !out || b < 0 || oh <= 0 || ow <= 0 || planes <= 0 ||
      hx <= 0 || wx <= 0 || cin <= 0 || stride <= 0 || cout <= 0)
    return set_error(h, RR_EINVAL, "rr_bottleneck_out_h2: bad argument");
  if ((planes % 32) || (cin % 32) || (cout % 256))
    return set_error(h, RR_EINVAL, "rr_bottleneck_out_h2: planes % 32, cin % 32 and cout % 256 must be 0");
  if ((long long)(oh - 1) * stride >= hx || (long long)(ow - 1) * stride >= wx)
    return set_error(h, RR_EINVAL, "rr_bottleneck_out_h2: the strided samples leave x");
  const long long M = (long long)b * oh * ow;
  if (M > 0x7fffffffLL || (long long)b * hx * wx > 0x7fffffffLL)
    return set_error(h, RR_EINVAL, "rr_bottleneck_out_h2: too many pixels");
  if (((uintptr_t)y & 15) || ((uintptr_t)x & 15) || ((uintptr_t)w2 & 15) || ((uintptr_t)w_iscale & 15) ||
      ((uintptr_t)out & 15) || (bias && ((uintptr_t)bias & 15)))
    return set_error(h, RR_EINVAL, "rr_bottleneck_out_h2: y/x/w2/w_iscale/bias/out must be 16-byte aligned");
  GemmArgs g;
  g.A = y;
  g.lda = planes;
  g.M = (int)M;
  g.K = planes + cin;
  g.K1 = planes;
  g.A2 = x;
  g.lda2 = cin;
  g.H2 = hx;
  g.W2 = wx;
  g.s2 = stride;
  g.OH = oh;
  g.OW = ow;
  g.B = reinterpret_cast<const float*>(w2);
  g.ldb = g.K;
  g.b_plane = (long long)cout * g.K;
  g.N = cout;
  g.C = out;
  g.ldc = cout;
  g.bias = bias;
  g.relu = 1;
  g.col_scale = w_iscale;
  g.a_amax = y_amax;
  g.a2_amax = x_amax;
  g.c_amax = out_amax;
  return launch_gemm_h2_seg2(h, g, (hipStream_t)stream, kTimeGemm);
}

int rr_split2_f16(rr_handle_t h, const float* w, int rows, int k, int kpad, void* planes, float* iscale,
                  void* stream) {
  RR_ENTRY(h);
  if (!w || !planes || !iscale || rows < 0 || k <= 0 || kpad < k) return set_error(h, RR_EINVAL, "rr_split2_f16: bad argument");
  TimedLaunch tl(h, kTimeElem, (hipStream_t)stream);
  return launch_split2h(h, w, rows, k, kpad, reinterpret_cast<uint16_t*>(planes), iscale, (hipStream_t)stream);
}

int rr_amax_f32(rr_handle_t h, const float* x, long long n, unsigned* amax, void* stream) {
  RR_ENTRY(h);
  if (!x || !amax || n < 0) return set_error(h, RR_EINVAL, "rr_amax_f32: bad argument");
  TimedLaunch tl(h, kTimeElem, (hipStream_t)stream);
  return launch_amax(h, x, n, amax, (hipStream_t)stream);
}


int rr_linear(rr_handle_t h, const float* x, int m, int k, const float* w, const float* bias, int n, float* y,
              void* stream) {
  return rr_linear_ex(h, x, m, k, w, bias, n, nullptr, 0, y, stream);
}

int rr_linear_ex(rr_handle_t h, const float* x, int m, int k, const float* w, const float* bias, int n,
                 const float* residual, int act, float* y, void* stream) {
  RR_ENTRY(h);
  if (!x || !w || !y || m < 0 || k <= 0 || n <= 0 || (k & 3)) return set_error(h, RR_EINVAL, "rr_linear: bad argument");
  if (((uintptr_t)x & 15) || ((uintptr_t)w & 15)) return set_error(h, RR_EINVAL, "rr_linear: x/w must be 16-byte aligned");
  GemmArgs g;
  g.A = x;
  g.lda = k;
  g.M = m;
  g.K = k;
  g.B = w;
  g.ldb = k;
  g.N = n;
  g.C = y;
  g.ldc = n;
  g.bias = bias;
  g.residual = residual;
  if (act < 0 || act > 2) return set_error(h, RR_EINVAL, "rr_linear_ex: act must be 0, 1 or 2");
  g.relu = act;
  return launch_gemm(h, A_DENSE, E_STORE, g, (hipStream_t)stream, kTimeGemm);
}

}
```

research_image_retrieval_amd/csrc/rr_internal.hpp:

```cpp
#pragma once

#include <type_traits>

#include <hip/hip_runtime.h>
#include <stdint.h>
#include <string>
#include <vector>

#include "../../include/rr.h"

struct rr_handle_s {
  int device = 0;
  std::string last_error;
  struct Tuning {
    int gemm_cfg = 0;
    int gemm_bk = 0;
    int lp_cfg = 0;
    int s3_cfg = 0;
    int s3_stagger = -1;
    int sweep_mf16 = -1;
    int sweep_il = -1;
    int conv_il = -1;
    int halo_mf = -1;
    int halo_2d = -1;
    int s3_cfg_res = 0;
    int sweep_form = -1;
  } tune;
  int n_cu = 0;
  bool timing = false;
  static constexpr int kClasses = 6;
  std::vector<hipEvent_t> ev_start[kClasses], ev_stop[kClasses];
  int n_ev[kClasses] = {};
  double acc_ms[kClasses] = {};
  long long acc_launches[kClasses] = {};
};

namespace rr {

struct DeviceGuard {
  int prev = -1;
  int rc = 0;
  explicit DeviceGuard(const rr_handle_s* h) {
    int cur = -1;
    if (hipGetDevice(&cur) != hipSuccess) {
      rc = RR_EHIP;
      return;
    }
    if (cur != h->device) {
      if (hipSetDevice(h->device) != hipSuccess) {
        rc = RR_EHIP;
        return;
      }
      prev = cur;
    }
  }
  ~DeviceGuard() {
    if (prev >= 0) (void)hipSetDevice(prev);
  }
};
#define RR_ENTRY(h)                                                                 \
  if (!(h)) return RR_EINVAL;                                                       \
  rr::DeviceGuard rr_device_guard_(h);                                              \
  if (rr_device_guard_.rc) return rr::set_error(h, rr_device_guard_.rc, "cannot select the handle's device")

enum TimerClass { kTimeCosine = 0, kTimeGemm = 1, kTimeSelect = 2, kTimeElem = 3, kTimeCosineSeed = 4, kTimeAttn = 5 };

struct TimedLaunch {
  rr_handle_s* h;
  int cls;
  hipStream_t s;
  int slot = -1;
  TimedLaunch(rr_handle_s* h_, int cls_, hipStream_t s_);
  ~TimedLaunch();
};

int set_error(rr_handle_s* h, int code, const std::string& msg);
int check_hip(rr_handle_s* h, hipError_t e, const char* what);

__host__ __device__ inline uint32_t ord_f32(float f) {
  uint32_t u;
  __builtin_memcpy(&u, &f, 4);
  if ((u & 0x7fffffffu) > 0x7f800000u) return 0u;
  if (u == 0x80000000u) u = 0u;
  return (u & 0x80000000u) ? ~u : (u | 0x80000000u);
}
__host__ __device__ inline float unord_f32(uint32_t o) {
  uint32_t u = (o & 0x80000000u) ? (o & 0x7fffffffu) : ~o;
  float f;
  __builtin_memcpy(&f, &u, 4);
  return f;
}
__host__ __device__ inline float next_down(float f) {
  uint32_t u;
  __builtin_memcpy(&u, &f, 4);
  if ((u & 0x7fffffffu) == 0) u = 0x80000001u;
  else if (u == 0xff800000u || (u & 0x7fffffffu) > 0x7f800000u) {
  } else if (u & 0x80000000u) ++u;
  else --u;
  __builtin_memcpy(&f, &u, 4);
  return f;
}
__host__ __device__ inline float next_up(float f) { return -next_down(-f); }
__host__ __device__ inline unsigned long long make_key(float s, uint32_t idx) {
  return ((unsigned long long)ord_f32(s) << 32) | (unsigned long long)(~idx);
}
__host__ __device__ inline uint32_t key_idx(unsigned long long k) {
  return ~(uint32_t)(k & 0xffffffffull);
}
__host__ __device__ inline float key_score(unsigned long long k) {
  return unord_f32((uint32_t)(k >> 32));
}

inline long long seed_sample_rows(long long n, int k) {
  long long s = n / 48;
  if (s > 32768) s = 32768;
  if (s < 4096) s = 4096;
  if (s < k) s = k;
  return n < s ? n : s;
}

inline int device_cu_count(rr_handle_s* h) {
  if (h->n_cu <= 0) {
    int v = 0;
    if (hipDeviceGetAttribute(&v, hipDeviceAttributeMultiprocessorCount, h->device) != hipSuccess || v <= 0) v = 256;
    h->n_cu = v;
  }
  return h->n_cu;
}

inline long long cap_that_fits(size_t off_cand, int nq, size_t bytes, long long worst) {
  const size_t usable = bytes & ~(size_t)255;
  if (nq <= 0 || usable <= off_cand) return 0;
  const long long cap = (long long)((usable - off_cand) / ((size_t)nq * 8));
  return cap < worst ? cap : worst;
}

enum AMode { A_DENSE = 0, A_CONV = 1, A_CONV_GENERIC = 2, A_CONV_C4 = 3 };
enum EMode { E_STORE = 0, E_SCORES_T = 1, E_FILTER = 2 };
enum DType { DT_F32 = 0, DT_BF16 = 1, DT_FP8 = 2 };

struct GemmArgs {
  const float* A = nullptr;
  long long lda = 0;
  int M = 0, K = 0;
  int H = 0, W = 0, Cin = 0, OH = 0, OW = 0, KH = 1, KW = 1, stride = 1, pad = 0;
  const float* B = nullptr;
  long long ldb = 0;
  int N = 0;
  float* C = nullptr;
  long long ldc = 0;
  const float* bias = nullptr;
  const float* residual = nullptr;
  int relu = 0;
  const float* tau = nullptr;
  unsigned long long* cand = nullptr;
  int* cnt = nullptr;
  long long cap = 0;
  long long row_offset = 0;
  const float* scale_a = nullptr;
  const float* scale_b = nullptr;
  int out_bf16 = 0;
  int k_split = 0;
  long long c_split_stride = 0;
  int sym = 0;
  long long b_plane = 0;
  const float* col_scale = nullptr;
  const uint32_t* a_amax = nullptr;
  uint32_t* c_amax = nullptr;
  int stagger_blocks = 0, stagger_sleeps = 0;
  const float* A2 = nullptr;
  long long lda2 = 0;
  int K1 = 0, H2 = 0, W2 = 0, s2 = 1;
  const uint32_t* a2_amax = nullptr;
  float* pool_out = nullptr;
  int POH = 0, POW = 0, pool_tr = 0, pool_tc = 0;
  uint16_t* c2 = nullptr;
  float* stats_out = nullptr;
  const float* stats_in = nullptr;
  const float* colsum = nullptr;
  int stats_k = 0;
  float ln_eps = 0.f;
  int mf16_sweep = 0;
  int issue_spread = 0;
  int halo_mf = -1;
  int halo_2d = -1;
};

__device__ __forceinline__ float wave_sum(float x) {
  auto shr = [](float v, auto ctrl) {
    return __int_as_float(__builtin_amdgcn_mov_dpp(__float_as_int(v), decltype(ctrl)::value, 0xf, 0xf, true));
  };
  x += shr(x, std::integral_constant<int, 0x111>{});
  x += shr(x, std::integral_constant<int, 0x112>{});
  x += shr(x, std::integral_constant<int, 0x114>{});
  x += shr(x, std::integral_constant<int, 0x118>{});
  const int xi = __float_as_int(x);
  return (__int_as_float(__builtin_amdgcn_readlane(xi, 15)) + __int_as_float(__builtin_amdgcn_readlane(xi, 31))) +
         (__int_as_float(__builtin_amdgcn_readlane(xi, 47)) + __int_as_float(__builtin_amdgcn_readlane(xi, 63)));
}

__device__ __forceinline__ void tile_coords(int bid, int nwg, int tiles_n, int& tm, int& tn) {
  const int xcd = bid & 7, q8 = nwg >> 3, r8 = nwg & 7;
  const int wgid = (xcd < r8 ? xcd * (q8 + 1) : r8 * (q8 + 1) + (xcd - r8) * q8) + (bid >> 3);
  tn = wgid % tiles_n;
  tm = wgid / tiles_n;
}

int launch_gemm(rr_handle_s* h, int amode, int emode, const GemmArgs& a, hipStream_t s, int timer_cls,
                int dt = DT_F32);

int launch_gemm_s3(rr_handle_s* h, int amode, const GemmArgs& g, hipStream_t s, int timer_cls);
hipError_t launch_h2_tile(int cfg, int amode, const GemmArgs& g, hipStream_t s, int n_cu, int st);
hipError_t launch_h2_tile_stem_pool(const GemmArgs& q, hipStream_t s, int n_cu);
hipError_t launch_s3p(const GemmArgs& g, hipStream_t s, int n_cu, int st);
bool s3q_shape(const GemmArgs& g);
bool s3q_fits(const GemmArgs& g);
hipError_t launch_s3q(const GemmArgs& g, hipStream_t s, int n_cu, int st);
int h2_halo_rows(const GemmArgs& g);
hipError_t launch_h2_halo(const GemmArgs& g, hipStream_t s, int hr, int mf, bool pers, int n_cu);
bool h2_halo_2d_ok(const GemmArgs& g);
hipError_t launch_h2_halo_2d(const GemmArgs& g, hipStream_t s);
int launch_gemm_h2_seg2(rr_handle_s* h, const GemmArgs& g, hipStream_t s, int timer_cls);
int launch_stem_pool_h2(rr_handle_s* h, const GemmArgs& g, hipStream_t s, int timer_cls);
int launch_split2h(rr_handle_s* h, const float* w, int rows, int k, int kpad, uint16_t* planes, float* iscale,
                   hipStream_t s);
int launch_amax(rr_handle_s* h, const float* x, long long n, uint32_t* slots, hipStream_t s);

bool gemm_8p_eligible(const GemmArgs& g, int dt);
hipError_t launch_gemm_8p(const GemmArgs& g, int emode, hipStream_t s, int dt);

int launch_select_dense_seed(rr_handle_s* h, const float* scores_t, long long ld, int rows, int nq,
                             int k, long long row_offset, unsigned long long* cand, long long cap,
                             int* cnt, float* tau, hipStream_t s);
int launch_select_final(rr_handle_s* h, const unsigned long long* cand, long long cap,
                        const int* cnt, int nq, int k, long long idx_offset, float* out_scores,
                        long long* out_idx, int* overflow_flag, hipStream_t s);
int launch_prefilter_rescore(rr_handle_s* h, unsigned long long* cand, long long cap, const int* cnt, int nq, int k,
                             const float* eps2, float* t2, const float* q, const float* g, int d, hipStream_t s);
int launch_merge(rr_handle_s* h, const float* ps, const long long* pi, int nparts, int nq, int kin,
                 int kout, float* os, long long* oi, hipStream_t s);

bool sweep16_eligible(const GemmArgs& g);
hipError_t launch_sweep16(const GemmArgs& g, hipStream_t s, int rows128);

bool lpp_eligible(const GemmArgs& g);
hipError_t launch_lpp(const GemmArgs& g, hipStream_t s, int n_cu);
bool lpp3_eligible(const GemmArgs& g);
hipError_t launch_lpp3(const GemmArgs& g, hipStream_t s, int n_cu);

void dolg_slab_release(rr_handle_s* h);

}
```

research_image_retrieval_amd/models.py:

```python
import torch

from . import ops
from . import weights as W
from .networks import ResNet, _Extractor, EPS_L2


class GeMPooling:

    def __init__(self, p=3.0, eps=1e-6):
        self.p = torch.ones(1) * p
        self.eps = eps

    def __call__(self, x_nhwc):
        return ops.gem_pool(x_nhwc, float(self.p.item()), self.eps)


class GeMModel(_Extractor):

    in_channels = 4

    def __init__(self, backbone="resnet50", pretrained=False, num_classes=1000, feature_dim=2048, gem_p=3.0,
                 state_dict=None, seed=0, device="cuda", conv_math="h2", stride_on="3x3"):
        if pretrained:
            raise ValueError("pretrained weights need a download; pass a local state_dict instead "
                             "(models/gem_pooling.py:35 defaults to pretrained=True)")
        if backbone not in ("resnet50", "resnet101"):
            raise ValueError(f"Unsupported backbone: {backbone}")
        self.device = torch.device(device)
        self.backbone = ResNet(backbone, state_dict, seed, device, conv_math=conv_math, stride_on=stride_on)
        self.gem_pool = GeMPooling(p=gem_p)
        backbone_dim = 2048
        pw, pb = _from_sd(state_dict, "feature_proj") or W.synthetic_linear(feature_dim, backbone_dim, seed + 2)
        self.proj_w = pw.float().contiguous().to(self.device)
        self.proj_b = pb.float().contiguous().to(self.device)
        cw, cb = _from_sd(state_dict, "classifier") or W.synthetic_linear(num_classes, feature_dim, seed + 3)
        self.cls_w = cw.float().contiguous().to(self.device)
        self.cls_b = cb.float().contiguous().to(self.device)
        self.feature_dim = feature_dim
        self.outputdim = feature_dim

    def extract_features_nhwc(self, x_nhwc):
        f = self.backbone(x_nhwc)
        f = self.gem_pool(f)
        return ops.linear(f, self.proj_w, self.proj_b)

    @torch.no_grad()
    def extract_features(self, x):
        return self.extract_features_nhwc(self._input(x))

    def forward_test_nhwc(self, x_nhwc):
        f = self.extract_features_nhwc(x_nhwc)
        return ops.l2_normalize(f, EPS_L2, out=f)

    @torch.no_grad()
    def extract_descriptor(self, x):
        return self.forward_test(x)

    @torch.no_grad()
    def forward(self, x, targets=None):
        feats = self.extract_features(x)
        return None, ops.linear(feats, self.cls_w, self.cls_b)

    __call__ = forward


def _from_sd(sd, name):
    if sd is None:
        return None
    for pre in ("", "backbone.", "module.backbone."):
        k = f"{pre}{name}.weight"
        if k in sd:
            return sd[k], sd[f"{pre}{name}.bias"]
    return None


class GeMWrapper(_Extractor):

    in_channels = 4

    def __init__(self, num_classes, backbone="resnet50", feature_dim=2048, gem_p=3.0, **kw):
        self.backbone = GeMModel(backbone=backbone, num_classes=num_classes, feature_dim=feature_dim, gem_p=gem_p,
                                 **kw)
        self.outputdim = feature_dim

    def forward_test_nhwc(self, x_nhwc):
        return self.backbone.forward_test_nhwc(x_nhwc)

    @torch.no_grad()
    def forward(self, x, targets=None):
        return self.backbone(x)

    __call__ = forward

    @torch.no_grad()
    def extract_global_descriptor(self, x):
        return self.backbone.extract_descriptor(x)


def get_gem_model(num_classes, backbone="resnet50", **kwargs):
    return GeMWrapper(num_classes=num_classes, backbone=backbone, **kwargs)


MODEL_REGISTRY = {
    "gem_r50": lambda num_classes, **kw: get_gem_model(num_classes, backbone="resnet50", **kw),
    "gem_r101": lambda num_classes, **kw: get_gem_model(num_classes, backbone="resnet101", **kw),
}

OUT_OF_SCOPE = ("delg_r50", "delg_r101", "token_r50", "token_r101", "how_vlad_r50", "how_vlad_r101",
                "how_asmk_r50", "how_asmk_r101", "senet_g2_50", "senet_g2_101", "sosnet_r50", "sosnet_r101",
                "spoc_r50", "spoc_r101")


def get_model(model_name, num_classes, **kwargs):
    if model_name not in MODEL_REGISTRY:
        if model_name in OUT_OF_SCOPE:
            raise NotImplementedError(f"{model_name} is outside the accelerated hot path (SURVEY.md §2)")
        raise ValueError(f"Unknown model: {model_name}. Available models: {list(MODEL_REGISTRY)}")
    return MODEL_REGISTRY[model_name](num_classes, **kwargs)
```

research_image_retrieval_amd/networks.py:

```python
import numpy as np
import torch

from . import ops
from . import weights as W

EPS_L2 = 1e-12


class ResNet:

    outputdim_block5 = 2048
    outputdim_block4 = 1024

    def __init__(self, name="resnet101", state_dict=None, seed=0, device="cuda", conv_math="h2", stride_on="3x3"):
        if conv_math not in ("h2", "f32"):
            raise ValueError("conv_math must be 'h2' or 'f32'")
        W.block_strides(1, stride_on)
        self.stride_on = stride_on
        if name not in W.RESNET_LAYERS:
            raise ValueError(f"Unsupported or unknown architecture: {name}!")
        self.name = name
        sd = W.synthetic_resnet_state_dict(name, seed) if state_dict is None else W.to_torchvision_keys(state_dict)
        self.device = torch.device(device)
        folded = W.folded_resnet(sd, name)
        w1, b1 = folded["conv1"]
        folded["conv1"] = (torch.nn.functional.pad(w1, (0, 1)).contiguous(), b1)
        self.convs = {k: (w.to(self.device), b.to(self.device)) for k, (w, b) in folded.items()}
        self.layers = W.RESNET_LAYERS[name]
        self.conv_math = conv_math
        self.convs_h2 = {}
        if conv_math == "h2":
            self.convs_h2 = {k: ops.H2Conv(w) for k, (w, _) in self.convs.items()}
            self.fuse_downsample = True
            self.fuse_stem_pool = True
            self.bneck_h2 = {}
            for li in range(len(self.layers)):
                p = f"layer{li + 1}.0"
                (w3, b3), (wd, bd) = self.convs[p + ".conv3"], self.convs[p + ".downsample.0"]
                if w3.shape[0] % 256 == 0:
                    self.bneck_h2[p] = ops.H2Bottleneck(w3, b3, wd, bd)

    def _conv(self, x, name, stride, pad, relu, residual=None):
        w, b = self.convs[name]
        return ops.conv2d(x, w, b, stride, pad, residual, relu)

    def _forward_h2(self, x, return_x3, hook=None, return_x3_amax=False):
        cv, h2 = self.convs, self.convs_h2
        hook = hook or (lambda i: None)
        rec = ops.amax_records(2 + 3 * sum(self.layers), x.device)
        ops.amax_f32(x, rec[0])
        if self.fuse_stem_pool and h2["conv1"].cout == 64:
            x = ops.stem_pool_h2(x, rec[0], h2["conv1"], cv["conv1"][1], 2, 3, rec[1])
        else:
            x = ops.conv2d_h2(x, rec[0], h2["conv1"], cv["conv1"][1], 2, 3, None, True, rec[1])
            x = ops.maxpool2d(x, 3, 2, 1)
        hook(0)
        xa, r, x3, x3a, ci = rec[1], 2, None, None, 1
        for li, nb in enumerate(self.layers):
            for bi in range(nb):
                p = f"layer{li + 1}.{bi}"
                s1, s2 = W.block_strides(2 if (bi == 0 and li > 0) else 1, self.stride_on)
                d = f"{p}.downsample.0"
                fused = bi == 0 and self.fuse_downsample and p in self.bneck_h2
                idn = ops.conv2d_h2(x, xa, h2[d], cv[d][1], s1 * s2, 0, None, False) if bi == 0 and not fused else x
                y = ops.conv2d_h2(x, xa, h2[f"{p}.conv1"], cv[f"{p}.conv1"][1], s1, 0, None, True, rec[r])
                hook(ci)
                y = ops.conv2d_h2(y, rec[r], h2[f"{p}.conv2"], cv[f"{p}.conv2"][1], s2, 1, None, True, rec[r + 1])
                hook(ci + 1)
                if fused:
                    x = ops.bottleneck_out_h2(y, rec[r + 1], x, xa, self.bneck_h2[p], s1 * s2, rec[r + 2])
                else:
                    x = ops.conv2d_h2(y, rec[r + 1], h2[f"{p}.conv3"], cv[f"{p}.conv3"][1], 1, 0, idn, True,
                                      rec[r + 2])
                hook(ci + 2)
                ci += 3
                xa, r = rec[r + 2], r + 3
            if li == 2:
                x3, x3a = x, xa
        if return_x3 and return_x3_amax:
            return x3, x, x3a
        return (x3, x) if return_x3 else x

    def forward(self, x, return_x3=False, hook=None, return_x3_amax=False):
        if x.shape[-1] == 3:
            x = torch.nn.functional.pad(x, (0, 1))
        if self.conv_math == "h2":
            return self._forward_h2(x.contiguous(), return_x3, hook, return_x3_amax)
        if return_x3_amax:
            raise ValueError("return_x3_amax: only the f16x2 trunk (conv_math='h2') keeps max-|x| records")
        x = self._conv(x, "conv1", 2, 3, True)
        x = ops.maxpool2d(x, 3, 2, 1)
        x3 = None
        for li, nb in enumerate(self.layers):
            for bi in range(nb):
                p = f"layer{li + 1}.{bi}"
                s1, s2 = W.block_strides(2 if (bi == 0 and li > 0) else 1, self.stride_on)
                idn = self._conv(x, f"{p}.downsample.0", s1 * s2, 0, False) if bi == 0 else x
                y = self._conv(x, f"{p}.conv1", s1, 0, True)
                y = self._conv(y, f"{p}.conv2", s2, 1, True)
                x = self._conv(y, f"{p}.conv3", 1, 0, True, residual=idn)
            if li == 2:
                x3 = x
        return (x3, x) if return_x3 else x

    __call__ = forward


class gem:

    def __init__(self, p=3.0, eps=1e-6):
        self.p = float(p)
        self.eps = float(eps)

    def __call__(self, x_nhwc):
        return ops.gem_pool(x_nhwc, self.p, self.eps)


class _Extractor:
    def eval(self):
        return self

    def train(self, mode=False):
        if mode:
            raise NotImplementedError("training is out of scope (SURVEY.md §2: row 13)")
        return self

    def to(self, *_a, **_k):
        return self

    in_channels = 3

    def _input(self, x):
        if not isinstance(x, torch.Tensor) or not x.is_cuda:
            raise ValueError("forward_test expects a float32 [B,3,H,W] tensor on a ROCm device")
        x = x.float() if x.dtype != torch.float32 else x
        return ops.nchw_to_nhwc(x.contiguous(), out_c=self.in_channels)

    def forward_test_nhwc(self, x_nhwc):
        raise NotImplementedError

    @torch.no_grad()
    def forward_test(self, x):
        return self.forward_test_nhwc(self._input(x))

    @torch.no_grad()
    def forward_test_u8(self, img_nhwc_u8):
        return self.forward_test_nhwc(ops.preprocess_u8(img_nhwc_u8, out_c=self.in_channels))

    @torch.no_grad()
    def forward_test_u8_streams(self, img_nhwc_u8, streams, lag=1):
        x = img_nhwc_u8
        dev = x.device
        cur = torch.cuda.current_stream(dev)
        n = len(streams)
        b = x.shape[0]
        cuts = [b * i // n for i in range(n + 1)]
        outs, gate = [], None
        for i, s in enumerate(streams):
            if cuts[i] == cuts[i + 1]:
                continue
            s.wait_stream(cur)
            if gate is not None:
                s.wait_event(gate)
            ev = torch.cuda.Event()

            def hook(ci, ev=ev, s=s):
                if ci == lag:
                    ev.record(s)

            with torch.cuda.stream(s):
                f = self.forward_test_nhwc(ops.preprocess_u8(x[cuts[i]:cuts[i + 1]], out_c=self.in_channels),
                                           hook=hook)
            outs.append(f)
            gate = ev
        if not outs:
            return self.forward_test_u8(x)
        for s in streams:
            cur.wait_stream(s)
        for f in outs:
            f.record_stream(cur)
        return torch.cat(outs)


class GeM(_Extractor):

    in_channels = 4

    def __init__(self, outputdim=2048, backbone="resnet101", state_dict=None, whiten=None, seed=0, device="cuda",
                 conv_math="h2"):
        if outputdim != 2048:
            raise ValueError("networks.GeM requires outputdim == 2048 (whiten is Conv2d(outputdim, 2048), "
                             "networks/RetrievalNet.py:332)")
        self.device = torch.device(device)
        self.backbone = ResNet(backbone, state_dict, seed, device, conv_math)
        self.pooling = gem()
        if whiten is None:
            ww, wb = W.synthetic_linear(2048, outputdim, seed + 1)
        else:
            ww, wb = whiten
            ww = ww.reshape(ww.shape[0], -1)
        self.whiten_w = ww.float().contiguous().to(self.device)
        self.whiten_b = wb.float().contiguous().to(self.device)
        self.outputdim = outputdim

    def forward_test_nhwc(self, x_nhwc, hook=None):
        f = self.backbone(x_nhwc, hook=hook)
        f = self.pooling(f)
        f = ops.linear(f, self.whiten_w, self.whiten_b)
        return ops.l2_normalize(f, EPS_L2, out=f)


class DOLG(_Extractor):

    in_channels = 4

    def __init__(self, pretrained=None, with_aspp=False, backbone="resnet101", state_dict=None, seed=0,
                 device="cuda", conv_math="h2", stride_on="3x3"):
        if with_aspp:
            raise ValueError("networks.DOLG: with_aspp=True is not supported (ASPP needs dilated 3x3 convs)")
        if pretrained is not None:
            raise ValueError("networks.DOLG: pretrained weights cannot be downloaded; pass state_dict")
        self.device = torch.device(device)
        if state_dict is None:
            head = W.dolg_head_from_state_dict(W.synthetic_dolg_head(seed + 1))
        else:
            head = W.dolg_head_from_state_dict(state_dict)
        self.globalmodel = ResNet(backbone, state_dict, seed, device, conv_math, stride_on)
        cin = self.globalmodel.outputdim_block4
        if tuple(head["conv1_w"].shape[1:]) != (1, 1, cin) or head["fc_t_w"].shape[1] != ResNet.outputdim_block5 or \
                head["fc_t_w"].shape[0] != head["conv1_w"].shape[0] or head["fc_w"].shape[1] != 2 * head["conv1_w"].shape[0]:
            raise ValueError("networks.DOLG: head weight shapes do not fit the trunk")
        self.conv_math = conv_math
        self.pool_g = gem(3.0)
        self.conv1_w = head["conv1_w"].to(self.device)
        self.conv1_b = head["conv1_b"].to(self.device)
        self.conv1_h2 = ops.H2Conv(self.conv1_w) if conv_math == "h2" else None
        self.conv2_w = head["conv2_w"].to(self.device)
        self.conv2_b = head["conv2_b"]
        self.fc_t = (head["fc_t_w"].to(self.device), head["fc_t_b"].to(self.device))
        self.fc = (head["fc_w"].to(self.device), head["fc_b"].to(self.device))
        self.outputdim = head["fc_w"].shape[0]
        self.meta = {"outputdim": self.outputdim}

    def local_mean(self, x3, x3_amax=None):
        if self.conv_math == "h2":
            y = ops.conv2d_h2(x3, x3_amax, self.conv1_h2, self.conv1_b, 1, 0, None, False)
        else:
            y = ops.conv2d(x3, self.conv1_w, self.conv1_b, 1, 0, None, False)
        return ops.dolg_local_pool(y, self.conv2_w, self.conv2_b)

    def forward_test_nhwc(self, x_nhwc, hook=None):
        if self.conv_math == "h2":
            x3, x4, x3a = self.globalmodel(x_nhwc, return_x3=True, hook=hook, return_x3_amax=True)
        else:
            (x3, x4), x3a = self.globalmodel(x_nhwc, return_x3=True), None
        return self.head(x3, x4, x3a)

    def head(self, x3, x4, x3_amax=None):
        m = self.local_mean(x3, x3_amax)
        fg = ops.linear(self.pool_g(x4), *self.fc_t)
        f = ops.linear(ops.dolg_orth_fuse(fg, m), *self.fc)
        return ops.l2_normalize(f, EPS_L2, out=f)


class ConvDimReduction:

    def __init__(self, input_dim, dim, device="cuda"):
        self.input_dim, self.dim = input_dim, dim
        self.device = torch.device(device)
        self.weight = None
        self.bias = None

    def initialize_pca_whitening(self, des):
        m, P = pcawhitenlearn_shrinkage(des, device=self.device)
        m, P = m.T, P.T
        self.weight = torch.tensor(P[: self.dim, :], dtype=torch.float32).contiguous().to(self.device)
        shift = -torch.mm(torch.tensor(P, dtype=torch.float32), torch.tensor(m, dtype=torch.float32)).squeeze()
        self.bias = shift[: self.dim].contiguous().to(self.device)
        return m.T, P.T

    def set_params(self, weight, bias):
        self.weight = weight.reshape(weight.shape[0], -1).float().contiguous().to(self.device)
        self.bias = bias.float().contiguous().to(self.device)

    def __call__(self, x):
        if self.weight is None:
            raise RuntimeError("ConvDimReduction: call initialize_pca_whitening or set_params first")
        return ops.linear(x, self.weight, self.bias)


def pcawhitenlearn_shrinkage(X, s=1.0, device="cuda"):
    if isinstance(X, torch.Tensor):
        dt = np.float64 if X.dtype == torch.float64 else np.float32
    else:
        X = np.asarray(X)
        dt = X.dtype if X.dtype in (np.float32, np.float64) else np.float32
    x = torch.as_tensor(X).to(device=device, dtype=torch.float32).contiguous()
    n = x.shape[0]
    mean64, gram = ops.pcaw_gram(x)
    gram = gram.cpu().numpy()
    cov = ((gram + gram.T) / (2 * n)).astype(dt)
    lam, vec = np.linalg.eig(cov)
    desc = np.argsort(lam)[::-1]
    lam, vec = lam[desc], vec[:, desc]
    proj = np.linalg.inv(np.diag(np.power(lam, 0.5 * s))) @ vec.T
    return mean64.cpu().numpy()[None, :].astype(dt), proj.T


class GeMPCAw(_Extractor):

    def __init__(self, net, pcaw):
        self.in_channels = net.in_channels
        self.net = net
        self.pcaw = pcaw
        self.outputdim = pcaw.dim

    def forward_test_nhwc(self, x_nhwc, hook=None):
        f = self.net.forward_test_nhwc(x_nhwc, hook=hook)
        f = self.pcaw(f)
        return ops.l2_normalize(f, EPS_L2, out=f)


class VisionTransformer(_Extractor):

    def __init__(self, input_resolution=224, patch_size=16, width=768, layers=12, heads=12, output_dim=512,
                 state_dict=None, device="cuda", dtype="fp32"):
        if width % heads or width // heads != 64:
            raise ValueError("VisionTransformer: librr's fused attention needs head_dim == 64")
        if state_dict is None:
            raise ValueError("VisionTransformer needs a state_dict (no pretrained download offline)")
        self.device = torch.device(device)
        self.res, self.patch, self.width, self.layers, self.heads = input_resolution, patch_size, width, layers, heads
        self.output_dim = self.outputdim = output_dim
        self.seq = (input_resolution // patch_size) ** 2 + 1
        if self.seq > 256:
            raise ValueError("VisionTransformer: sequence longer than 256 tokens")
        t = lambda k: state_dict[k].float().contiguous().to(self.device)
        self.conv_w = state_dict["conv1.weight"].float().permute(0, 2, 3, 1).reshape(width, -1).contiguous().to(
            self.device)
        self.cls = t("class_embedding")
        self.pos = t("positional_embedding")
        self.ln_pre = (t("ln_pre.weight"), t("ln_pre.bias"))
        self.blocks = []
        for i in range(layers):
            p = f"transformer.resblocks.{i}."
            self.blocks.append({k: t(p + k) for k in (
                "attn.in_proj_weight", "attn.in_proj_bias", "attn.out_proj.weight", "attn.out_proj.bias",
                "ln_1.weight", "ln_1.bias", "mlp.c_fc.weight", "mlp.c_fc.bias", "mlp.c_proj.weight",
                "mlp.c_proj.bias", "ln_2.weight", "ln_2.bias")})
        self.ln_post = (t("ln_post.weight"), t("ln_post.bias"))
        self.proj_t = state_dict["proj"].float().t().contiguous().to(self.device)
        if dtype not in ("fp32", "bf16"):
            raise ValueError("VisionTransformer dtype must be fp32 or bf16")
        self.dtype = dtype
        if dtype == "bf16":
            self.conv_w_bf = self.conv_w.to(torch.bfloat16)
            for blk in self.blocks:
                for k in ("attn.in_proj_weight", "attn.out_proj.weight", "mlp.c_fc.weight", "mlp.c_proj.weight"):
                    blk[k + ".bf16"] = blk[k].to(torch.bfloat16)
                if not ops.ln_fold_supported(width, dtype):
                    continue
                blk["qkv.fold"] = ops.ln_fold_weights(blk["attn.in_proj_weight"], blk["attn.in_proj_bias"],
                                                      blk["ln_1.weight"], blk["ln_1.bias"])
                blk["fc.fold"] = ops.ln_fold_weights(blk["mlp.c_fc.weight"], blk["mlp.c_fc.bias"],
                                                     blk["ln_2.weight"], blk["ln_2.bias"])
        self.ln_fold = ops.ln_fold_supported(width, dtype)

    def _forward_bf16(self, x_nhwc, b):
        p = ops.patchify(x_nhwc, self.patch, out_bf16=True)
        x = ops.vit_tokens(ops.linear_bf16(p, self.conv_w_bf), b, self.cls, self.pos, ln=self.ln_pre)
        if self.ln_fold:
            xb, st = ops.ln_partials_bf16(x)
            for li, blk in enumerate(self.blocks):
                qkv = ops.linear_bf16_ln_fold(xb, st, *blk["qkv.fold"])
                a = ops.attention_bf16(qkv, b, self.seq, self.heads)
                x, xb, st = ops.linear_bf16_ln_produce(a, blk["attn.out_proj.weight.bf16"], blk["attn.out_proj.bias"], x)
                y = ops.linear_bf16_ln_fold(xb, st, *blk["fc.fold"], act=2)
                if li + 1 < len(self.blocks):
                    x, xb, st = ops.linear_bf16_ln_produce(y, blk["mlp.c_proj.weight.bf16"], blk["mlp.c_proj.bias"], x)
                else:
                    x = ops.linear_bf16(y, blk["mlp.c_proj.weight.bf16"], blk["mlp.c_proj.bias"], residual=x)
            cls = ops.layernorm(x, *self.ln_post, rows=b, row_stride=self.seq * self.width)
            return ops.linear(cls, self.proj_t)
        for blk in self.blocks:
            y = ops.layernorm_bf16(x, blk["ln_1.weight"], blk["ln_1.bias"])
            qkv = ops.linear_bf16(y, blk["attn.in_proj_weight.bf16"], blk["attn.in_proj_bias"], out_bf16=True)
            a = ops.attention_bf16(qkv, b, self.seq, self.heads)
            x = ops.linear_bf16(a, blk["attn.out_proj.weight.bf16"], blk["attn.out_proj.bias"], residual=x)
            y = ops.layernorm_bf16(x, blk["ln_2.weight"], blk["ln_2.bias"])
            y = ops.linear_bf16(y, blk["mlp.c_fc.weight.bf16"], blk["mlp.c_fc.bias"], act=2, out_bf16=True)
            x = ops.linear_bf16(y, blk["mlp.c_proj.weight.bf16"], blk["mlp.c_proj.bias"], residual=x)
        cls = ops.layernorm(x, *self.ln_post, rows=b, row_stride=self.seq * self.width)
        return ops.linear(cls, self.proj_t)

    def forward_nhwc(self, x_nhwc):
        b, h, w, _ = x_nhwc.shape
        if self.dtype == "bf16" and h == self.res and w == self.res:
            return self._forward_bf16(x_nhwc, b)
        if h != self.res or w != self.res:
            raise ValueError(f"VisionTransformer: fixed {self.res}x{self.res} input (positional embedding has "
                             f"{self.seq} tokens; networks/model.py:228)")
        x = ops.linear(ops.patchify(x_nhwc, self.patch), self.conv_w)
        x = ops.vit_tokens(x, b, self.cls, self.pos, ln=self.ln_pre)
        for blk in self.blocks:
            y = ops.layernorm(x, blk["ln_1.weight"], blk["ln_1.bias"])
            qkv = ops.linear(y, blk["attn.in_proj_weight"], blk["attn.in_proj_bias"])
            a = ops.attention(qkv, b, self.seq, self.heads)
            x = ops.linear_ex(a, blk["attn.out_proj.weight"], blk["attn.out_proj.bias"], residual=x)
            y = ops.layernorm(x, blk["ln_2.weight"], blk["ln_2.bias"])
            y = ops.linear_ex(y, blk["mlp.c_fc.weight"], blk["mlp.c_fc.bias"], act=2)
            x = ops.linear_ex(y, blk["mlp.c_proj.weight"], blk["mlp.c_proj.bias"], residual=x)
        cls = ops.layernorm(x, *self.ln_post, rows=b, row_stride=self.seq * self.width)
        return ops.linear(cls, self.proj_t)

    @torch.no_grad()
    def forward(self, x):
        return self.forward_nhwc(self._input(x))

    __call__ = forward

    def forward_test_nhwc(self, x_nhwc):
        f = self.forward_nhwc(x_nhwc)
        return ops.l2_normalize(f, EPS_L2, out=f)
```

research_image_retrieval_amd/ops.py:

```python
import ctypes

import torch

from . import _lib

_NULL = None


def _dev(t):
    if not t.is_cuda:
        raise ValueError("librr ops need ROCm device tensors (got a CPU tensor)")
    return t.device.index if t.device.index is not None else torch.cuda.current_device()


def _ptr(t):
    return None if t is None else ctypes.c_void_p(t.data_ptr())


def _stream(dev):
    return ctypes.c_void_p(torch.cuda.current_stream(dev).cuda_stream)


def _f32(t, name):
    if t.dtype != torch.float32:
        raise TypeError(f"{name}: expected float32, got {t.dtype}")
    if not t.is_contiguous():
        raise ValueError(f"{name}: must be contiguous")
    return t


def preprocess_u8(img_nhwc, mean=(0.485, 0.456, 0.406), std=(0.229, 0.224, 0.225), out_c=3):
    if img_nhwc.dtype != torch.uint8 or img_nhwc.dim() != 4 or img_nhwc.shape[3] != 3:
        raise ValueError("preprocess_u8: expected uint8 [B,H,W,3]")
    img_nhwc = img_nhwc.contiguous()
    dev = _dev(img_nhwc)
    b, h, w, _ = img_nhwc.shape
    out = torch.empty((b, h, w, out_c), dtype=torch.float32, device=img_nhwc.device)
    m = (ctypes.c_float * 3)(*mean)
    s = (ctypes.c_float * 3)(*std)
    hd = _lib.handle(dev)
    _lib.check(_lib.lib().rr_preprocess_u8_ex(hd, _ptr(img_nhwc), b, h, w, ctypes.cast(m, ctypes.c_void_p),
                                              ctypes.cast(s, ctypes.c_void_p), int(out_c), _ptr(out), _stream(dev)),
               hd, "rr_preprocess_u8")
    return out


def nchw_to_nhwc(x, out_c=None):
    x = _f32(x.contiguous(), "nchw_to_nhwc")
    dev = _dev(x)
    b, c, h, w = x.shape
    oc = c if out_c is None else int(out_c)
    out = torch.empty((b, h, w, oc), dtype=torch.float32, device=x.device)
    hd = _lib.handle(dev)
    _lib.check(_lib.lib().rr_nchw_to_nhwc_ex(hd, _ptr(x), b, c, h, w, oc, _ptr(out), _stream(dev)), hd,
               "rr_nchw_to_nhwc")
    return out


def conv2d(x, w, bias, stride=1, pad=0, residual=None, relu=False):
    _f32(x, "conv2d x")
    _f32(w, "conv2d w")
    dev = _dev(x)
    b, h, wd, cin = x.shape
    cout, kh, kw, cin_w = w.shape
    if cin_w != cin:
        raise ValueError(f"conv2d: Cin mismatch {cin} vs {cin_w}")
    oh = (h + 2 * pad - kh) // stride + 1
    ow = (wd + 2 * pad - kw) // stride + 1
    y = torch.empty((b, oh, ow, cout), dtype=torch.float32, device=x.device)
    if residual is not None:
        _f32(residual, "conv2d residual")
        if tuple(residual.shape) != tuple(y.shape):
            raise ValueError("conv2d: residual shape mismatch")
    if bias is not None:
        _f32(bias, "conv2d bias")
    hd = _lib.handle(dev)
    _lib.check(_lib.lib().rr_conv2d(hd, _ptr(x), b, h, wd, cin, _ptr(w), _ptr(bias), cout, kh, kw, stride, pad,
                                    _ptr(residual), int(relu), _ptr(y), _stream(dev)), hd, "rr_conv2d")
    return y


AMAX_SLOTS = 64


def amax_records(n, device):
    return torch.zeros((n, AMAX_SLOTS), dtype=torch.int32, device=device)


def amax_f32(x, record):
    x = _f32(x.contiguous(), "amax_f32")
    if record.dtype != torch.int32 or record.numel() != AMAX_SLOTS or not record.is_contiguous():
        raise ValueError("amax_f32: record must be contiguous int32 [RR_AMAX_SLOTS]")
    dev = _dev(x)
    hd = _lib.handle(dev)
    _lib.check(_lib.lib().rr_amax_f32(hd, _ptr(x), x.numel(), _ptr(record), _stream(dev)), hd, "rr_amax_f32")
    return record


def amax_value(record):
    return float(record.view(torch.float32).max().item())


def split2_f16(w, kpad=None):
    w = _f32(w.contiguous(), "split2_f16")
    dev = _dev(w)
    rows = w.shape[0]
    k = w.numel() // max(rows, 1)
    kpad = k if kpad is None else int(kpad)
    if kpad < k:
        raise ValueError("split2_f16: kpad < K")
    planes = torch.empty((2, rows, kpad), dtype=torch.int16, device=w.device)
    iscale = torch.empty((rows,), dtype=torch.float32, device=w.device)
    hd = _lib.handle(dev)
    _lib.check(_lib.lib().rr_split2_f16(hd, _ptr(w), rows, k, kpad, _ptr(planes), _ptr(iscale), _stream(dev)), hd,
               "rr_split2_f16")
    return planes, iscale


class H2Conv:

    def __init__(self, w):
        w = _f32(w.contiguous(), "H2Conv")
        cout, kh, kw, cin = w.shape
        if cin % 32 and cin != 4:
            raise ValueError("H2Conv: Cin must be a multiple of 32, or 4 (NHWC4 stem)")
        k = kh * kw * cin
        self.kpad = (k + 31) // 32 * 32 if cin == 4 else k
        self.planes, self.iscale = split2_f16(w.reshape(cout, k), self.kpad)
        self.cout, self.kh, self.kw, self.cin = cout, kh, kw, cin


def conv2d_h2(x, x_amax, wc, bias, stride=1, pad=0, residual=None, relu=False, y_amax=None):
    _f32(x, "conv2d_h2 x")
    if not isinstance(wc, H2Conv):
        raise TypeError("conv2d_h2: wc must be an ops.H2Conv")
    dev = _dev(x)
    b, h, wd, cin = x.shape
    if cin != wc.cin:
        raise ValueError(f"conv2d_h2: Cin mismatch {cin} vs {wc.cin}")
    for r, nm in ((x_amax, "x_amax"), (y_amax, "y_amax")):
        if r is not None and (r.dtype != torch.int32 or r.numel() != AMAX_SLOTS or not r.is_contiguous()):
            raise ValueError(f"conv2d_h2: {nm} must be a contiguous int32 [RR_AMAX_SLOTS] record")
    oh = (h + 2 * pad - wc.kh) // stride + 1
    ow = (wd + 2 * pad - wc.kw) // stride + 1
    y = torch.empty((b, oh, ow, wc.cout), dtype=torch.float32, device=x.device)
    if residual is not None:
        _f32(residual, "conv2d_h2 residual")
        if tuple(residual.shape) != tuple(y.shape):
            raise ValueError("conv2d_h2: residual shape mismatch")
    if bias is not None:
        _f32(bias, "conv2d_h2 bias")
    hd = _lib.handle(dev)
    _lib.check(_lib.lib().rr_conv2d_h2(hd, _ptr(x), _ptr(x_amax), b, h, wd, cin, _ptr(wc.planes), _ptr(wc.iscale),
                                       _ptr(bias), wc.cout, wc.kh, wc.kw, stride, pad, _ptr(residual), int(relu),
                                       _ptr(y), _ptr(y_amax), _stream(dev)), hd, "rr_conv2d_h2")
    return y


def stem_pool_h2(x, x_amax, wc, bias, stride=2, pad=3, y_amax=None):
    _f32(x, "stem_pool_h2 x")
    if not isinstance(wc, H2Conv) or wc.cin != 4 or wc.cout != 64:
        raise TypeError("stem_pool_h2: wc must be an ops.H2Conv with Cin 4 and Cout 64")
    dev = _dev(x)
    b, h, wd, cin = x.shape
    if cin != 4:
        raise ValueError("stem_pool_h2: x must be NHWC4")
    oh = (h + 2 * pad - wc.kh) // stride + 1
    ow = (wd + 2 * pad - wc.kw) // stride + 1
    y = torch.empty((b, (oh - 1) // 2 + 1, (ow - 1) // 2 + 1, 64), dtype=torch.float32, device=x.device)
    if bias is not None:
        _f32(bias, "stem_pool_h2 bias")
    hd = _lib.handle(dev)
    _lib.check(_lib.lib().rr_stem_pool_h2(hd, _ptr(x), _ptr(x_amax), b, h, wd, _ptr(wc.planes), _ptr(wc.iscale),
                                          _ptr(bias), 64, wc.kh, wc.kw, stride, pad, _ptr(y), _ptr(y_amax),
                                          _stream(dev)), hd, "rr_stem_pool_h2")
    return y


class H2Bottleneck:

    def __init__(self, w3, b3, wd, bd):
        w3, wd = _f32(w3.contiguous(), "H2Bottleneck w3"), _f32(wd.contiguous(), "H2Bottleneck wd")
        cout, planes = w3.shape[0], w3.numel() // w3.shape[0]
        cin = wd.numel() // wd.shape[0]
        if wd.shape[0] != cout or tuple(w3.shape[1:3]) != (1, 1) or tuple(wd.shape[1:3]) != (1, 1):
            raise ValueError("H2Bottleneck: 1x1 conv3 and downsample with the same Cout")
        self.planes, self.cin, self.cout = planes, cin, cout
        self.planes2, self.iscale = split2_f16(torch.cat([w3.reshape(cout, planes), wd.reshape(cout, cin)], 1))
        self.bias = (b3.double() + bd.double()).float().contiguous() if b3 is not None else bd.contiguous()


def bottleneck_out_h2(y, y_amax, x, x_amax, wb, stride, out_amax=None):
    _f32(y, "bottleneck_out_h2 y")
    _f32(x, "bottleneck_out_h2 x")
    if not isinstance(wb, H2Bottleneck):
        raise TypeError("bottleneck_out_h2: wb must be an ops.H2Bottleneck")
    b, oh, ow, planes = y.shape
    bx, hx, wx, cin = x.shape
    if planes != wb.planes or cin != wb.cin or bx != b:
        raise ValueError("bottleneck_out_h2: shape mismatch")
    dev = _dev(y)
    out = torch.empty((b, oh, ow, wb.cout), dtype=torch.float32, device=y.device)
    hd = _lib.handle(dev)
    _lib.check(_lib.lib().rr_bottleneck_out_h2(hd, _ptr(y), _ptr(y_amax), b, oh, ow, planes, _ptr(x), _ptr(x_amax),
                                               hx, wx, cin, int(stride), _ptr(wb.planes2), _ptr(wb.iscale),
                                               _ptr(wb.bias), wb.cout, _ptr(out), _ptr(out_amax), _stream(dev)),
               hd, "rr_bottleneck_out_h2")
    return out


def resize_bilinear(x_nhwc, out_h, out_w, scale_factor=None):
    _f32(x_nhwc, "resize_bilinear")
    dev = _dev(x_nhwc)
    b, h, w, c = x_nhwc.shape
    y = torch.empty((b, out_h, out_w, c), dtype=torch.float32, device=x_nhwc.device)
    inv = 0.0 if scale_factor is None else float(1.0 / scale_factor)
    hd = _lib.handle(dev)
    _lib.check(_lib.lib().rr_resize_bilinear(hd, _ptr(x_nhwc), b, h, w, c, int(out_h), int(out_w), inv, inv, _ptr(y),
                                             _stream(dev)), hd, "rr_resize_bilinear")
    return y


def maxpool2d(x, k=3, stride=2, pad=1):
    _f32(x, "maxpool2d")
    dev = _dev(x)
    b, h, w, c = x.shape
    oh = (h + 2 * pad - k) // stride + 1
    ow = (w + 2 * pad - k) // stride + 1
    y = torch.empty((b, oh, ow, c), dtype=torch.float32, device=x.device)
    hd = _lib.handle(dev)
    _lib.check(_lib.lib().rr_maxpool2d(hd, _ptr(x), b, h, w, c, k, stride, pad, _ptr(y), _stream(dev)), hd,
               "rr_maxpool2d")
    return y


def gem_pool(x_nhwc, p=3.0, eps=1e-6):
    _f32(x_nhwc, "gem_pool")
    dev = _dev(x_nhwc)
    b, c = x_nhwc.shape[0], x_nhwc.shape[-1]
    hw = x_nhwc.numel() // (b * c) if b * c else 0
    out = torch.empty((b, c), dtype=torch.float32, device=x_nhwc.device)
    hd = _lib.handle(dev)
    _lib.check(_lib.lib().rr_gem_pool(hd, _ptr(x_nhwc), b, hw, c, float(p), float(eps), _ptr(out), _stream(dev)), hd,
               "rr_gem_pool")
    return out


def linear(x, w, bias=None):
    _f32(x, "linear x")
    _f32(w, "linear w")
    dev = _dev(x)
    m, k = x.shape
    n = w.shape[0]
    y = torch.empty((m, n), dtype=torch.float32, device=x.device)
    hd = _lib.handle(dev)
    _lib.check(_lib.lib().rr_linear(hd, _ptr(x), m, k, _ptr(w), _ptr(bias), n, _ptr(y), _stream(dev)), hd,
               "rr_linear")
    return y


def l2_normalize(x, eps=1e-12, out=None):
    _f32(x, "l2_normalize")
    dev = _dev(x)
    m, d = x.shape
    y = torch.empty_like(x) if out is None else out
    hd = _lib.handle(dev)
    _lib.check(_lib.lib().rr_l2_normalize(hd, _ptr(x), m, d, float(eps), _ptr(y), _stream(dev)), hd,
               "rr_l2_normalize")
    return y


def dolg_local_pool(y_nhwc, w2, b2):
    _f32(y_nhwc, "dolg_local_pool y")
    _f32(w2, "dolg_local_pool w2")
    dev = _dev(y_nhwc)
    b, c = y_nhwc.shape[0], y_nhwc.shape[-1]
    if w2.numel() != c:
        raise ValueError(f"dolg_local_pool: w2 has {w2.numel()} weights for {c} channels")
    hw = y_nhwc.numel() // (b * c) if b * c else 1
    out = torch.empty((b, c), dtype=torch.float32, device=y_nhwc.device)
    hd = _lib.handle(dev)
    _lib.check(_lib.lib().rr_dolg_local_pool(hd, _ptr(y_nhwc), b, hw, c, _ptr(w2), float(b2), _ptr(out), _stream(dev)),
               hd, "rr_dolg_local_pool")
    return out


def dolg_orth_fuse(fg, m):
    _f32(fg, "dolg_orth_fuse fg")
    _f32(m, "dolg_orth_fuse m")
    if fg.dim() != 2 or tuple(fg.shape) != tuple(m.shape):
        raise ValueError("dolg_orth_fuse: fg and m must both be [B,C]")
    dev = _dev(fg)
    b, c = fg.shape
    out = torch.empty((b, 2 * c), dtype=torch.float32, device=fg.device)
    hd = _lib.handle(dev)
    _lib.check(_lib.lib().rr_dolg_orth_fuse(hd, _ptr(fg), _ptr(m), b, c, _ptr(out), _stream(dev)), hd,
               "rr_dolg_orth_fuse")
    return out


def cosine_topk_workspace_size(nq, n, d, k):
    return int(_lib.lib().rr_cosine_topk_workspace_size(int(nq), int(n), int(d), int(k)))


_WS_FUNCS = {
    "exact": ("rr_cosine_topk_workspace_size", "rr_cosine_topk_workspace_size_cap", "rr_cosine_topk_cap_for",
              "rr_cosine_topk_counts_offset", "rr_cosine_topk_overflow_offset"),
    "prefilter": ("rr_cosine_topk_prefilter_workspace_size", "rr_cosine_topk_prefilter_workspace_size_cap",
                  "rr_cosine_topk_prefilter_cap_for", "rr_cosine_topk_prefilter_counts_offset",
                  "rr_cosine_topk_prefilter_overflow_offset"),
}


def _wsf(kind, i):
    return getattr(_lib.lib(), _WS_FUNCS[kind][i])


def ranker_workspace_bounds(kind, nq, n, d, k):
    a = (int(nq), int(n), int(d), int(k))
    return int(_wsf(kind, 1)(*a, int(k))), int(_wsf(kind, 0)(*a))


def _ranker_workspace(kind, nq, n, d, k, workspace, max_workspace_bytes, device):
    lo, full = ranker_workspace_bounds(kind, nq, n, d, k)
    budget = full if max_workspace_bytes is None else max(lo, min(full, int(max_workspace_bytes)))
    if workspace is None or workspace.numel() < budget:
        workspace = torch.empty(budget, dtype=torch.uint8, device=device)
    return workspace, workspace.numel() < full


def _recover_overflow(kind, nq, n, d, k, workspace, rerun, os_, oi):
    a = (int(nq), int(n), int(d), int(k))
    ovf_off = int(_wsf(kind, 4)(*a))
    if int(workspace[ovf_off:ovf_off + 4].view(torch.int32).item()) == 0:
        return 0
    cap = int(_wsf(kind, 2)(*a, workspace.numel()))
    cnt_off = int(_wsf(kind, 3)(*a))
    bad = torch.nonzero(workspace[cnt_off:cnt_off + 4 * int(nq)].view(torch.int32) > cap).flatten()
    c = max(1, bad.numel())
    while c > 1 and int(_wsf(kind, 0)(c, int(n), int(d), int(k))) > workspace.numel():
        c = (c + 1) // 2
    need = int(_wsf(kind, 0)(c, int(n), int(d), int(k)))
    ws = workspace if need <= workspace.numel() else torch.empty(need, dtype=torch.uint8, device=workspace.device)
    for part in bad.split(c):
        s_, i_ = rerun(part, ws)
        os_[part] = s_
        oi[part] = i_
    return int(bad.numel())


def cosine_topk(queries, gallery, k, idx_offset=0, workspace=None, max_workspace_bytes=None):
    _f32(queries, "cosine_topk queries")
    _f32(gallery, "cosine_topk gallery")
    dev = _dev(queries)
    nq, d = queries.shape
    n = gallery.shape[0]
    if gallery.shape[1] != d:
        raise ValueError("cosine_topk: descriptor dims differ")
    workspace, bounded = _ranker_workspace("exact", nq, n, d, k, workspace, max_workspace_bytes, queries.device)
    os_ = torch.empty((nq, k), dtype=torch.float32, device=queries.device)
    oi = torch.empty((nq, k), dtype=torch.int64, device=queries.device)
    hd = _lib.handle(dev)
    _lib.check(_lib.lib().rr_cosine_topk(hd, _ptr(queries), nq, _ptr(gallery), n, d, k, int(idx_offset), _ptr(os_),
                                         _ptr(oi), _ptr(workspace), workspace.numel(), _stream(dev)), hd,
               "rr_cosine_topk")
    if bounded and nq > 0:
        _recover_overflow("exact", nq, n, d, k, workspace,
                          lambda r, ws: cosine_topk(queries[r].contiguous(), gallery, k, idx_offset, ws), os_, oi)
    return os_, oi


def cosine_scores(queries, gallery):
    _f32(queries, "cosine_scores queries")
    _f32(gallery, "cosine_scores gallery")
    dev = _dev(queries)
    nq, d = queries.shape
    n = gallery.shape[0]
    out = torch.empty((n, nq), dtype=torch.float32, device=queries.device)
    hd = _lib.handle(dev)
    _lib.check(_lib.lib().rr_cosine_scores(hd, _ptr(queries), nq, _ptr(gallery), n, d, _ptr(out), _stream(dev)), hd,
               "rr_cosine_scores")
    return out


def topk_merge(part_scores, part_idx, k_out):
    _f32(part_scores, "topk_merge scores")
    if part_idx.dtype != torch.int64 or not part_idx.is_contiguous():
        raise TypeError("topk_merge: idx must be contiguous int64")
    dev = _dev(part_scores)
    p, nq, kin = part_scores.shape
    os_ = torch.empty((nq, k_out), dtype=torch.float32, device=part_scores.device)
    oi = torch.empty((nq, k_out), dtype=torch.int64, device=part_scores.device)
    hd = _lib.handle(dev)
    _lib.check(_lib.lib().rr_topk_merge(hd, _ptr(part_scores), _ptr(part_idx), p, nq, kin, k_out, _ptr(os_), _ptr(oi),
                                        _stream(dev)), hd, "rr_topk_merge")
    return os_, oi


_TUNE_KEYS = {"gemm_cfg": _lib.TUNE_GEMM_CFG, "gemm_bk": _lib.TUNE_GEMM_BK, "lp_cfg": _lib.TUNE_LP_CFG,
              "s3_cfg": _lib.TUNE_S3_CFG, "s3_stagger": _lib.TUNE_S3_STAGGER, "sweep_mf16": _lib.TUNE_SWEEP_MF16,
              "sweep_il": _lib.TUNE_SWEEP_IL, "conv_il": _lib.TUNE_CONV_IL,
              "halo_mf": _lib.TUNE_HALO_MF, "s3_cfg_res": _lib.TUNE_S3_CFG_RES,
              "sweep_form": _lib.TUNE_SWEEP_FORM, "halo_2d": _lib.TUNE_HALO_2D}
_TUNE_DEFAULT = {"s3_stagger": -1, "sweep_mf16": -1, "sweep_il": -1,
                 "conv_il": -1, "halo_mf": -1, "sweep_form": -1, "halo_2d": -1}


class tuning:

    def __init__(self, device_index, **kw):
        for k in kw:
            if k not in _TUNE_KEYS:
                raise ValueError(f"unknown tuning key {k!r}")
        self.h = _lib.handle(device_index)
        self.kw = kw

    def __enter__(self):
        for k, v in self.kw.items():
            _lib.check(_lib.lib().rr_set_tuning(self.h, _TUNE_KEYS[k], int(v)), self.h, "rr_set_tuning")
        return self

    def __exit__(self, *exc):
        for k in self.kw:
            _lib.lib().rr_set_tuning(self.h, _TUNE_KEYS[k], _TUNE_DEFAULT.get(k, 0))
        return False


class KernelTimer:

    def __init__(self, device_index):
        self.h = _lib.handle(device_index)

    def enable(self, on=True):
        _lib.check(_lib.lib().rr_timing_enable(self.h, int(on)), self.h, "rr_timing_enable")

    def collect(self, cls):
        ms = ctypes.c_double()
        n = ctypes.c_longlong()
        _lib.check(_lib.lib().rr_timing_collect(self.h, cls, ctypes.byref(ms), ctypes.byref(n)), self.h,
                   "rr_timing_collect")
        return ms.value, n.value


def linear_ex(x, w, bias=None, residual=None, act=0):
    _f32(x, "linear_ex x")
    _f32(w, "linear_ex w")
    dev = _dev(x)
    m, k = x.shape
    n = w.shape[0]
    y = torch.empty((m, n), dtype=torch.float32, device=x.device)
    if residual is not None:
        _f32(residual, "linear_ex residual")
        if tuple(residual.shape) != (m, n):
            raise ValueError("linear_ex: residual shape mismatch")
    hd = _lib.handle(dev)
    _lib.check(_lib.lib().rr_linear_ex(hd, _ptr(x), m, k, _ptr(w), _ptr(bias), n, _ptr(residual), int(act), _ptr(y),
                                       _stream(dev)), hd, "rr_linear_ex")
    return y


def layernorm(x, gamma, beta, eps=1e-5, rows=None, row_stride=None):
    _f32(x, "layernorm")
    dev = _dev(x)
    d = x.shape[-1]
    m = x.numel() // d if rows is None else int(rows)
    ld = d if row_stride is None else int(row_stride)
    y = torch.empty((m, d), dtype=torch.float32, device=x.device)
    hd = _lib.handle(dev)
    _lib.check(_lib.lib().rr_layernorm(hd, _ptr(x), ld, m, d, _ptr(gamma), _ptr(beta), float(eps), _ptr(y),
                                       _stream(dev)), hd, "rr_layernorm")
    return y


def patchify(x_nhwc, patch, out_bf16=False):
    _f32(x_nhwc, "patchify")
    dev = _dev(x_nhwc)
    b, h, w, c = x_nhwc.shape
    y = torch.empty((b * (h // patch) * (w // patch), patch * patch * c),
                    dtype=torch.bfloat16 if out_bf16 else torch.float32, device=x_nhwc.device)
    hd = _lib.handle(dev)
    _lib.check(_lib.lib().rr_patchify_ex(hd, _ptr(x_nhwc), b, h, w, c, patch, int(out_bf16), _ptr(y), _stream(dev)),
               hd, "rr_patchify_ex")
    return y


def vit_tokens(patches, b, cls, pos, ln=None, eps=1e-5):
    _f32(patches, "vit_tokens")
    dev = _dev(patches)
    width = patches.shape[1]
    npatch = patches.shape[0] // b
    y = torch.empty((b * (npatch + 1), width), dtype=torch.float32, device=patches.device)
    hd = _lib.handle(dev)
    gamma, beta = ln if ln is not None else (None, None)
    _lib.check(_lib.lib().rr_vit_tokens_ex(hd, _ptr(patches), b, npatch, width, _ptr(cls), _ptr(pos), _ptr(gamma),
                                           _ptr(beta), float(eps), _ptr(y), _stream(dev)), hd, "rr_vit_tokens_ex")
    return y


def attention(qkv, b, seq, heads, head_dim=64):
    _f32(qkv, "attention")
    dev = _dev(qkv)
    out = torch.empty((b * seq, heads * head_dim), dtype=torch.float32, device=qkv.device)
    hd = _lib.handle(dev)
    _lib.check(_lib.lib().rr_attention(hd, _ptr(qkv), b, seq, heads, head_dim, _ptr(out), _stream(dev)), hd,
               "rr_attention")
    return out


DT_BF16, DT_FP8 = 1, 2
_LP = {"bf16": DT_BF16, "fp8": DT_FP8}


def quantize_rows(x, dtype):
    _f32(x, "quantize_rows")
    dev = _dev(x)
    dt = _LP[dtype]
    rows, d = x.shape
    if dt == DT_BF16:
        y = torch.empty((rows, d), dtype=torch.bfloat16, device=x.device)
        sc = None
    else:
        y = torch.empty((rows, d), dtype=torch.uint8, device=x.device)
        sc = torch.empty(rows, dtype=torch.float32, device=x.device)
    hd = _lib.handle(dev)
    _lib.check(_lib.lib().rr_quantize_rows(hd, _ptr(x), rows, d, dt, _ptr(y), _ptr(sc), _stream(dev)), hd,
               "rr_quantize_rows")
    return y, sc


def _lp_rows(t, sc, dtype, name):
    if t.dim() != 2 or not t.is_contiguous():
        raise ValueError(f"{name}: expected contiguous [rows, d]")
    if dtype == "bf16":
        if t.dtype != torch.bfloat16:
            raise TypeError(f"{name}: bf16 rows must be torch.bfloat16, got {t.dtype}")
    else:
        if t.dtype not in (torch.uint8, torch.float8_e4m3fn):
            raise TypeError(f"{name}: fp8 rows must be uint8 (e4m3 bytes), got {t.dtype}")
        if sc is None or sc.dtype != torch.float32 or not sc.is_contiguous() or sc.numel() != t.shape[0]:
            raise ValueError(f"{name}: fp8 rows need contiguous fp32 scales, one per row")


def cosine_topk_lp(q, q_scale, g, g_scale, k, dtype, idx_offset=0, workspace=None, max_workspace_bytes=None):
    if dtype not in _LP:
        raise ValueError("cosine_topk_lp: dtype must be 'bf16' or 'fp8'")
    _lp_rows(q, q_scale, dtype, "cosine_topk_lp queries")
    _lp_rows(g, g_scale, dtype, "cosine_topk_lp gallery")
    if q.shape[1] != g.shape[1]:
        raise ValueError("cosine_topk_lp: descriptor dims differ")
    dev = _dev(q)
    dt = _LP[dtype]
    nq, d = q.shape
    n = g.shape[0]
    workspace, bounded = _ranker_workspace("exact", nq, n, d, k, workspace, max_workspace_bytes, q.device)
    os_ = torch.empty((nq, k), dtype=torch.float32, device=q.device)
    oi = torch.empty((nq, k), dtype=torch.int64, device=q.device)
    hd = _lib.handle(dev)
    _lib.check(_lib.lib().rr_cosine_topk_lp(hd, _ptr(q), _ptr(q_scale), nq, _ptr(g), _ptr(g_scale), n, d, dt, k,
                                            int(idx_offset), _ptr(os_), _ptr(oi), _ptr(workspace), workspace.numel(),
                                            _stream(dev)), hd, "rr_cosine_topk_lp")
    if bounded and nq > 0:
        _recover_overflow("exact", nq, n, d, k, workspace,
                          lambda r, ws: cosine_topk_lp(q[r].contiguous(), None if q_scale is None else
                                                       q_scale[r].contiguous(), g, g_scale, k, dtype, idx_offset, ws),
                          os_, oi)
    return os_, oi


def linear_bf16(x, w, bias=None, residual=None, act=0, out_bf16=False):
    if x.dtype != torch.bfloat16 or w.dtype != torch.bfloat16:
        raise TypeError("linear_bf16: x and w must be bfloat16")
    if x.dim() != 2 or w.dim() != 2 or not x.is_contiguous() or not w.is_contiguous() or x.shape[1] != w.shape[1]:
        raise ValueError("linear_bf16: contiguous x [M,K] and w [N,K] with matching K")
    dev = _dev(x)
    m, k = x.shape
    n = w.shape[0]
    if bias is not None and (_f32(bias, "linear_bf16 bias").numel() != n):
        raise ValueError("linear_bf16: bias must have N entries")
    if residual is not None and tuple(_f32(residual, "linear_bf16 residual").shape) != (m, n):
        raise ValueError("linear_bf16: residual shape mismatch")
    y = torch.empty((m, n), dtype=torch.bfloat16 if out_bf16 else torch.float32, device=x.device)
    hd = _lib.handle(dev)
    _lib.check(_lib.lib().rr_linear_bf16(hd, _ptr(x), m, k, _ptr(w), _ptr(bias), n, _ptr(residual), int(act),
                                         int(out_bf16), _ptr(y), _stream(dev)), hd, "rr_linear_bf16")
    return y


def linear_bf16_ln_produce(x, w, bias, residual):
    if x.dtype != torch.bfloat16 or w.dtype != torch.bfloat16:
        raise TypeError("linear_bf16_ln_produce: x and w must be bfloat16")
    if x.dim() != 2 or w.dim() != 2 or not x.is_contiguous() or not w.is_contiguous() or x.shape[1] != w.shape[1]:
        raise ValueError("linear_bf16_ln_produce: contiguous x [M,K] and w [N,K] with matching K")
    dev = _dev(x)
    m, k = x.shape
    n = w.shape[0]
    if n % 256:
        raise ValueError("linear_bf16_ln_produce: N % 256 == 0")
    if _f32(bias, "bias").numel() != n or tuple(_f32(residual, "residual").shape) != (m, n):
        raise ValueError("linear_bf16_ln_produce: bias [N] and residual [M,N]")
    y = torch.empty((m, n), dtype=torch.float32, device=x.device)
    yb = torch.empty((m, n), dtype=torch.bfloat16, device=x.device)
    st = torch.empty((m, n // 256, 2), dtype=torch.float32, device=x.device)
    hd = _lib.handle(dev)
    _lib.check(_lib.lib().rr_linear_bf16_ln(hd, _ptr(x), m, k, _ptr(w), _ptr(bias), n, _ptr(residual), 0, 0, _ptr(y),
                                            None, None, 0.0, _ptr(st), _ptr(yb), _stream(dev)), hd, "rr_linear_bf16_ln")
    return y, yb, st


LN_FOLD_MAX_K = 768


def ln_fold_supported(width, dtype):
    return dtype == "bf16" and width % 256 == 0 and width <= LN_FOLD_MAX_K


def linear_bf16_ln_fold(xb, stats, w_folded, colsum, bias_folded, act=0, eps=1e-5):
    if xb.dtype != torch.bfloat16 or w_folded.dtype != torch.bfloat16:
        raise TypeError("linear_bf16_ln_fold: xb and w_folded must be bfloat16")
    dev = _dev(xb)
    m, k = xb.shape
    n = w_folded.shape[0]
    t = (k + 255) // 256
    if tuple(stats.shape) != (m, t, 2) or w_folded.shape[1] != k or tuple(colsum.shape) != (t, n):
        raise ValueError("linear_bf16_ln_fold: stats [M, ceil(K/256), 2], w_folded [N, K], colsum [ceil(K/256), N]")
    y = torch.empty((m, n), dtype=torch.bfloat16, device=xb.device)
    hd = _lib.handle(dev)
    _lib.check(_lib.lib().rr_linear_bf16_ln(hd, _ptr(xb), m, k, _ptr(w_folded), _ptr(bias_folded), n, None, int(act),
                                            1, _ptr(y), _ptr(stats), _ptr(colsum), float(eps), None, None,
                                            _stream(dev)), hd, "rr_linear_bf16_ln")
    return y


def ln_partials_bf16(x):
    _f32(x, "ln_partials_bf16")
    dev = _dev(x)
    d = x.shape[-1]
    m = x.numel() // d
    xb = torch.empty((m, d), dtype=torch.bfloat16, device=x.device)
    st = torch.empty((m, d // 256, 2), dtype=torch.float32, device=x.device)
    hd = _lib.handle(dev)
    _lib.check(_lib.lib().rr_ln_partials_bf16(hd, _ptr(x), m, d, _ptr(xb), _ptr(st), _stream(dev)), hd,
               "rr_ln_partials_bf16")
    return xb, st


def ln_fold_weights(w, b, gamma, beta):
    wf = (w.float() * gamma.float()[None, :]).to(torch.bfloat16).contiguous()
    n, k = wf.shape
    t = (k + 255) // 256
    colsum = torch.nn.functional.pad(wf.float(), (0, 256 * t - k)).view(n, t, 256).sum(dim=2).t().contiguous()
    bf = (b.double() + w.double() @ beta.double()).float().contiguous()
    return wf, colsum, bf


def layernorm_bf16(x, gamma, beta, eps=1e-5):
    _f32(x, "layernorm_bf16")
    dev = _dev(x)
    d = x.shape[-1]
    m = x.numel() // d
    y = torch.empty((m, d), dtype=torch.bfloat16, device=x.device)
    hd = _lib.handle(dev)
    _lib.check(_lib.lib().rr_layernorm_ex(hd, _ptr(x), d, m, d, _ptr(gamma), _ptr(beta), float(eps), 1, _ptr(y),
                                          _stream(dev)), hd, "rr_layernorm_ex")
    return y


def attention_bf16(qkv, b, seq, heads, head_dim=64, bf16_math=True):
    dev = _dev(qkv)
    if qkv.dtype == torch.bfloat16 and bf16_math:
        if not qkv.is_contiguous():
            raise ValueError("attention_bf16: qkv must be contiguous")
        fn = _lib.lib().rr_attention_bf16_qkv16
    else:
        _f32(qkv, "attention_bf16")
        fn = _lib.lib().rr_attention_bf16 if bf16_math else _lib.lib().rr_attention_ex
    out = torch.empty((b * seq, heads * head_dim), dtype=torch.bfloat16, device=qkv.device)
    hd = _lib.handle(dev)
    _lib.check(fn(hd, _ptr(qkv), b, seq, heads, head_dim, 1, _ptr(out), _stream(dev)), hd, "rr_attention_bf16")
    return out


def alpha_qe(queries, gallery, top_idx, top_scores, n=2, alpha=3.0, idx_offset=0):
    _f32(queries, "alpha_qe queries")
    _f32(gallery, "alpha_qe gallery")
    dev = _dev(queries)
    nq, d = queries.shape
    k = top_idx.shape[1]
    out = torch.empty_like(queries)
    hd = _lib.handle(dev)
    if gallery.shape[1] != d or top_idx.dtype != torch.int64 or top_scores.dtype != torch.float32:
        raise TypeError("alpha_qe: gallery [N, d] fp32, top_idx int64, top_scores fp32")
    _lib.check(_lib.lib().rr_alpha_qe(hd, _ptr(queries), nq, _ptr(gallery), gallery.shape[0], d,
                                      _ptr(top_idx.contiguous()),
                                      _ptr(top_scores.contiguous()), k, int(n), float(alpha), int(idx_offset),
                                      _ptr(out), _stream(dev)), hd, "rr_alpha_qe")
    return out


def pcaw_gram(x):
    _f32(x, "pcaw_gram")
    dev = _dev(x)
    n, d = x.shape
    if n == 0:
        raise ValueError("pcaw_gram: empty descriptor set")
    L = _lib.lib()
    ws = torch.empty(L.rr_pcaw_gram_workspace_size(n, d), dtype=torch.uint8, device=dev)
    mean = torch.empty(d, dtype=torch.float64, device=dev)
    gram = torch.empty((d, d), dtype=torch.float64, device=dev)
    hd = _lib.handle(dev)
    _lib.check(L.rr_pcaw_gram(hd, _ptr(x), n, d, _ptr(ws), ws.numel(), _ptr(mean), _ptr(gram), _stream(dev)),
               hd, "rr_pcaw_gram")
    return mean, gram


def prefilter_gallery_bound(gallery, gallery_bf16):
    _f32(gallery, "prefilter_gallery_bound")
    dev = _dev(gallery)
    n, d = gallery.shape
    out = torch.empty(3, dtype=torch.float64, device=gallery.device)
    hd = _lib.handle(dev)
    _lib.check(_lib.lib().rr_prefilter_gallery_bound(hd, _ptr(gallery), _ptr(gallery_bf16), n, d, _ptr(out),
                                                     _stream(dev)), hd, "rr_prefilter_gallery_bound")
    return out


def cosine_topk_prefilter_workspace_size(nq, n, d, k):
    return int(_lib.lib().rr_cosine_topk_prefilter_workspace_size(nq, n, d, k))


def prefilter_survivors(workspace, nq, n, d, k):
    off = int(_lib.lib().rr_cosine_topk_prefilter_counts_offset(int(nq), int(n), int(d), int(k)))
    return workspace[off:off + 4 * int(nq)].view(torch.int32)


def cosine_topk_prefilter(q, g, g_bf16, bound3, k, idx_offset=0, workspace=None, max_workspace_bytes=None):
    _f32(q, "cosine_topk_prefilter q")
    _f32(g, "cosine_topk_prefilter g")
    dev = _dev(q)
    nq, d = q.shape
    n = g.shape[0]
    workspace, bounded = _ranker_workspace("prefilter", nq, n, d, k, workspace, max_workspace_bytes, q.device)
    s = torch.empty((nq, k), dtype=torch.float32, device=q.device)
    i = torch.empty((nq, k), dtype=torch.int64, device=q.device)
    hd = _lib.handle(dev)
    _lib.check(_lib.lib().rr_cosine_topk_prefilter(hd, _ptr(q), nq, _ptr(g), _ptr(g_bf16), _ptr(bound3), n, d, k,
                                                   int(idx_offset), _ptr(s), _ptr(i), _ptr(workspace),
                                                   workspace.numel(), _stream(dev)), hd, "rr_cosine_topk_prefilter")
    if bounded and nq > 0:
        _recover_overflow("prefilter", nq, n, d, k, workspace,
                          lambda r, ws: cosine_topk_prefilter(q[r].contiguous(), g, g_bf16, bound3, k, idx_offset, ws),
                          s, i)
    return s, i
```

Before: 16740.

## Fuse uint8 normalization into the stem conv+pool kernel and u8 amax

Adds a uint8 path where the 7x7 stem halo kernel reads raw RGB bytes, normalizes them through a per-block LDS lookup table, and splits them into fp16 hi/lo planes. This skips the separate preprocess kernel and the fp32 NHWC4 intermediate tensor. A packed uint8 amax kernel computes the input amax from per-channel min/max instead of scanning fp32 data. It adds per-tile conversion work inside the stem pipeline and special handling for the last pixel to avoid reading past the end of the buffer.

```diff
diff --git a/include/rr.h b/include/rr.h
--- a/include/rr.h
+++ b/include/rr.h
@@ -139,11 +139,22 @@
                     int kw, int stride, int pad, float* y_pool,
                     unsigned* y_amax, void* stream);
 
+int rr_stem_pool_h2_u8(rr_handle_t h, const uint8_t* img_nhwc,
+                       const float* mean3, const float* std3,
+                       const unsigned* x_amax, int b, int hgt, int wid,
+                       const void* w2, const float* w_iscale,
+                       const float* bias, int cout, int kh, int kw, int stride,
+                       int pad, float* y_pool, unsigned* y_amax, void* stream);
+
 int rr_split2_f16(rr_handle_t h, const float* w, int rows, int k, int kpad,
                   void* planes, float* iscale, void* stream);
 
 int rr_amax_f32(rr_handle_t h, const float* x, long long n, unsigned* amax,
                 void* stream);
+
+int rr_amax_u8_norm(rr_handle_t h, const uint8_t* img_nhwc, long long n_px,
+                    const float* mean3, const float* std3, unsigned* amax,
+                    void* stream);
 
 int rr_maxpool2d(rr_handle_t h, const float* x, int b, int hgt, int wid, int c,
                  int k, int stride, int pad, float* y, void* stream);
diff --git a/research_image_retrieval_amd/_lib.py b/research_image_retrieval_amd/_lib.py
--- a/research_image_retrieval_amd/_lib.py
+++ b/research_image_retrieval_amd/_lib.py
@@ -54,6 +54,9 @@
     "rr_bottleneck_out_h2": (_i, [_vp, _vp, _vp, _i, _i, _i, _i, _vp, _vp, _i, _i, _i, _i, _vp, _vp, _vp, _i, _vp,
                                   _vp, _vp]),
     "rr_amax_f32": (_i, [_vp, _vp, _ll, _vp, _vp]),
+    "rr_amax_u8_norm": (_i, [_vp, _vp, _ll, _vp, _vp, _vp, _vp]),
+    "rr_stem_pool_h2_u8": (_i, [_vp, _vp, _vp, _vp, _vp, _i, _i, _i, _vp, _vp, _vp, _i, _i, _i, _i, _i, _vp, _vp,
+                                _vp]),
     "rr_resize_bilinear": (_i, [_vp, _vp, _i, _i, _i, _i, _i, _i, _f, _f, _vp, _vp]),
     "rr_maxpool2d": (_i, [_vp, _vp, _i, _i, _i, _i, _i, _i, _i, _vp, _vp]),
     "rr_gem_pool": (_i, [_vp, _vp, _i, _i, _i, _f, _f, _vp, _vp]),
diff --git a/research_image_retrieval_amd/csrc/embed_ops.hip b/research_image_retrieval_amd/csrc/embed_ops.hip
--- a/research_image_retrieval_amd/csrc/embed_ops.hip
+++ b/research_image_retrieval_amd/csrc/embed_ops.hip
@@ -7,9 +7,9 @@
   const long long stride = (long long)gridDim.x * blockDim.x;
   for (long long p = (long long)blockIdx.x * blockDim.x + threadIdx.x; p < n_px; p += stride) {
     const uint8_t* px = in + p * 3;
-    const float r = ((float)px[0] / 255.0f - m0) / s0;
-    const float g = ((float)px[1] / 255.0f - m1) / s1;
-    const float b = ((float)px[2] / 255.0f - m2) / s2;
+    const float r = norm_u8(px[0], m0, s0);
+    const float g = norm_u8(px[1], m1, s1);
+    const float b = norm_u8(px[2], m2, s2);
     if (out_c == 4) {
       *reinterpret_cast<float4*>(out + p * 4) = make_float4(r, g, b, 0.f);
     } else {
diff --git a/research_image_retrieval_amd/csrc/h2_dispatch.hip b/research_image_retrieval_amd/csrc/h2_dispatch.hip
--- a/research_image_retrieval_amd/csrc/h2_dispatch.hip
+++ b/research_image_retrieval_amd/csrc/h2_dispatch.hip
@@ -169,6 +169,85 @@
   return check_hip(h, hipGetLastError(), "amax launch");
 }
 
+typedef uint16_t u16x2 __attribute__((ext_vector_type(2)));
+
+__global__ __launch_bounds__(256) void amax_u8_norm_kernel(const uint8_t* __restrict__ img, long long n_px, float m0,
+                                                           float m1, float m2, float s0, float s1, float s2,
+                                                           uint32_t* slots) {
+  const long long gs = (long long)gridDim.x * blockDim.x;
+  const long long i0 = (long long)blockIdx.x * blockDim.x + threadIdx.x;
+  const long long head = std::min<long long>((long long)((uintptr_t)img & 3), n_px);
+  const uint32_t* w = reinterpret_cast<const uint32_t*>(img + 3 * head);
+  const long long n4 = (n_px - head) >> 2;
+  u16x2 mx[3][2], mn[3][2];
+#pragma unroll
+  for (int k = 0; k < 3; ++k)
+#pragma unroll
+    for (int o = 0; o < 2; ++o) mx[k][o] = u16x2{0, 0}, mn[k][o] = u16x2{255, 255};
+  auto fold = [&](const uint32_t (&d)[3]) {
+#pragma unroll
+    for (int k = 0; k < 3; ++k)
+#pragma unroll
+      for (int o = 0; o < 2; ++o) {
+        const u16x2 v = __builtin_bit_cast(u16x2, (d[k] >> (8 * o)) & 0x00ff00ffu);
+        mx[k][o] = __builtin_elementwise_max(mx[k][o], v);
+        mn[k][o] = __builtin_elementwise_min(mn[k][o], v);
+      }
+  };
+  long long i = i0;
+  for (; i + 3 * gs < n4; i += 4 * gs) {
+    uint32_t d[4][3];
+#pragma unroll
+    for (int u = 0; u < 4; ++u)
+#pragma unroll
+      for (int k = 0; k < 3; ++k) d[u][k] = w[3 * (i + u * gs) + k];
+#pragma unroll
+    for (int u = 0; u < 4; ++u) fold(d[u]);
+  }
+  for (; i < n4; i += gs) {
+    uint32_t d[3];
+#pragma unroll
+    for (int k = 0; k < 3; ++k) d[k] = w[3 * i + k];
+    fold(d);
+  }
+  int cmax[3] = {0, 0, 0}, cmin[3] = {255, 255, 255};
+#pragma unroll
+  for (int k = 0; k < 3; ++k)
+#pragma unroll
+    for (int j = 0; j < 4; ++j) {
+      const int c = (4 * k + j) % 3;
+      cmax[c] = max(cmax[c], (int)mx[k][j & 1][j >> 1]);
+      cmin[c] = min(cmin[c], (int)mn[k][j & 1][j >> 1]);
+    }
+  const long long rest = n_px - 4 * n4;
+  if (i0 < rest) {
+    const uint8_t* px = img + 3 * (i0 < head ? i0 : i0 + 4 * n4);
+#pragma unroll
+    for (int c = 0; c < 3; ++c) {
+      cmax[c] = max(cmax[c], (int)px[c]);
+      cmin[c] = min(cmin[c], (int)px[c]);
+    }
+  }
+  const float m[3] = {m0, m1, m2}, s[3] = {s0, s1, s2};
+  float am = 0.f;
+#pragma unroll
+  for (int c = 0; c < 3; ++c)
+    if (cmin[c] <= cmax[c]) {
+      am = amax_acc(am, norm_u8((uint8_t)cmin[c], m[c], s[c]));
+      am = amax_acc(am, norm_u8((uint8_t)cmax[c], m[c], s[c]));
+    }
+  amax_publish(slots, am, blockIdx.x * 4 + (threadIdx.x >> 6));
+}
+
+int launch_amax_u8_norm(rr_handle_s* h, const uint8_t* img, long long n_px, const float* mean3, const float* std3,
+                        uint32_t* slots, hipStream_t s) {
+  if (n_px <= 0) return RR_OK;
+  const long long blocks = std::min<long long>((n_px / 4 + 255) / 256 + 1, 512);
+  hipLaunchKernelGGL(amax_u8_norm_kernel, dim3((unsigned)blocks), dim3(256), 0, s, img, n_px, mean3[0], mean3[1],
+                     mean3[2], std3[0], std3[1], std3[2], slots);
+  return check_hip(h, hipGetLastError(), "amax_u8_norm launch");
+}
+
 #if RR_S3_PHASES
 int h2_tile_phases(unsigned long long* out);
 int h2_stream_phases(unsigned long long* out);
diff --git a/research_image_retrieval_amd/csrc/h2_stem.hip b/research_image_retrieval_amd/csrc/h2_stem.hip
--- a/research_image_retrieval_amd/csrc/h2_stem.hip
+++ b/research_image_retrieval_amd/csrc/h2_stem.hip
@@ -4,8 +4,8 @@
 
 namespace rr {
 
-template <int EPI, int NW = 8, int BREG = 0>
-__global__ __launch_bounds__(64 * NW, 1) void stem_pool_halo_kernel(GemmArgs g, int ntiles) {
+template <int EPI, int NW = 8, int BREG = 0, bool U8 = false>
+__global__ __launch_bounds__(64 * NW, 1) void stem_pool_halo_kernel(GemmArgs g, int ntiles, StemU8 u8) {
   constexpr int NT = 64 * NW, BN = 64, HR = 39, HC = 35, HP = HR * HC;
   constexpr int WR = BREG ? 64 : 256 / NW, FM = WR / 32;
   constexpr int JN = BREG ? 1 : 2;
@@ -21,10 +21,12 @@
   constexpr int C4 = BN / 4, NPOOL = 56 * C4;
   constexpr int QI = (NPOOL + NT - 1) / NT;
   constexpr int PS = NKS / QI;
-  __shared__ __attribute__((aligned(16))) uint16_t lds[B_U16 + A_U16 + C_U16];
+  constexpr int T_U16 = U8 ? 3 * 256 * 2 : 0;
+  __shared__ __attribute__((aligned(16))) uint16_t lds[B_U16 + A_U16 + C_U16 + T_U16];
   uint16_t* lb = lds;
   uint16_t* la = lds + B_U16;
   float* ct = reinterpret_cast<float*>(lds + B_U16 + A_U16);
+  [[maybe_unused]] float* nt = reinterpret_cast<float*>(lds + B_U16 + A_U16 + C_U16);
   typedef f16x8 frag_t;
   typedef _Float16 f16x4 __attribute__((ext_vector_type(4)));
 
@@ -46,6 +48,15 @@
     a_isc = __int_as_float((127 - e) << 23);
   }
 
+  if constexpr (U8) {
+    static_assert(NT >= 256, "one table row per thread");
+    if (tid < 256) {
+      nt[tid] = norm_u8((uint8_t)tid, u8.mean[0], u8.sdev[0]);
+      nt[256 + tid] = norm_u8((uint8_t)tid, u8.mean[1], u8.sdev[1]);
+      nt[512 + tid] = norm_u8((uint8_t)tid, u8.mean[2], u8.sdev[2]);
+    }
+  }
+
   constexpr int BRP = BREG == 1 ? 2 : 1;
   frag_t breg[BREG ? NKS : 1][BRP];
   if constexpr (BREG != 0) {
@@ -66,27 +77,56 @@
   }
 
   const int tpi = g.pool_tr * g.pool_tc;
-  f32x4 px[A_PASS];
+  std::conditional_t<U8, uint32_t, f32x4> px[A_PASS];
+  [[maybe_unused]] uint32_t pfl = 0;
   auto load_patch = [&](int tl) {
     const int b = tl / tpi, t2 = tl - b * tpi, pr = t2 / g.pool_tc, pc = t2 - pr * g.pool_tc;
+    if constexpr (U8) pfl = 0;
 #pragma unroll
     for (int q = 0; q < A_PASS; ++q) {
       const int p = tid + q * NT, hr = p / HC, hc = p - hr * HC;
       const int ih = 32 * pr - 5 + hr, iw = 28 * pc - 5 + hc;
       const bool ok = tl < ntiles && p < HP && (unsigned)ih < (unsigned)g.H && (unsigned)iw < (unsigned)g.W;
-      const f32x4* src = ok ? reinterpret_cast<const f32x4*>(g.A + (((long long)b * g.H + ih) * g.W + iw) * 4)
-                            : s3_zero_page();
-      asm volatile("global_load_dwordx4 %0, %1, off" : "=&v"(px[q]) : "v"(src) : "memory");
+      const long long ipx = ((long long)b * g.H + ih) * g.W + iw;
+      if constexpr (U8) {
+        const bool last = ok && ipx == u8.last_px;
+        const void* src = ok && !last ? static_cast<const void*>(u8.img + ipx * 3) : static_cast<const void*>(s3_zero_page());
+        asm volatile("global_load_dword %0, %1, off" : "=&v"(px[q]) : "v"(src) : "memory");
+        pfl |= ((ok ? 1u : 0u) | (last ? 2u : 0u)) << (2 * q);
+      } else {
+        const f32x4* src = ok ? reinterpret_cast<const f32x4*>(g.A + ipx * 4) : s3_zero_page();
+        asm volatile("global_load_dwordx4 %0, %1, off" : "=&v"(px[q]) : "v"(src) : "memory");
+      }
+    }
+  };
+  [[maybe_unused]] f32x4 pv[U8 ? A_PASS : 1];
+  auto convert_patch = [&]() {
+    if constexpr (U8) {
+      asm volatile("s_waitcnt vmcnt(0)" ::: "memory");
+#pragma unroll
+      for (int q = 0; q < A_PASS; ++q) {
+        asm volatile("" : "+v"(px[q]));
+        uint32_t w = px[q];
+        if ((pfl >> (2 * q)) & 2u) {
+          const uint8_t* lp = u8.img + u8.last_px * 3;
+          w = (uint32_t)lp[0] | ((uint32_t)lp[1] << 8) | ((uint32_t)lp[2] << 16);
+        }
+        const uint32_t in = 0u - ((pfl >> (2 * q)) & 1u);
+        auto tab = [&](uint32_t i) { return __uint_as_float(__float_as_uint(nt[i]) & in) * a_sc; };
+        pv[q] = f32x4{tab(w & 255u), tab(256 + ((w >> 8) & 255u)), tab(512 + ((w >> 16) & 255u)), 0.f};
+      }
     }
   };
   auto store_patch = [&]() {
-    asm volatile("s_waitcnt vmcnt(0)" ::: "memory");
+    if constexpr (!U8) asm volatile("s_waitcnt vmcnt(0)" ::: "memory");
 #pragma unroll
     for (int q = 0; q < A_PASS; ++q) {
-      asm volatile("" : "+v"(px[q]));
+      if constexpr (!U8) asm volatile("" : "+v"(px[q]));
       const int p = tid + q * NT, hr = p / HC, hc = p - hr * HC;
       const int slot = hr * HS + (hc & 1) * (HS / 2) + (hc >> 1);
-      const f32x4 v = px[q] * a_sc;
+      f32x4 v;
+      if constexpr (U8) v = pv[q];
+      else v = px[q] * a_sc;
       const f16x4 hi = __builtin_convertvector(v, f16x4);
       const f16x4 lo = __builtin_convertvector(v - __builtin_convertvector(hi, f32x4), f16x4);
       if (p < HP) {
@@ -94,7 +134,8 @@
         *reinterpret_cast<f16x4*>(la + (HPS + 1) * 4 + slot * 4) = lo;
       }
     }
-    if (tid < 2) *reinterpret_cast<uint2*>(la + tid * (HPS + 1) * 4 + HPS * 4) = uint2{0u, 0u};
+    const int zt = U8 ? s3_opaque(tid) : tid;
+    if (tid < 2) *reinterpret_cast<uint2*>(la + zt * (HPS + 1) * 4 + HPS * 4) = uint2{0u, 0u};
   };
 
   int sbase[FM];
@@ -106,6 +147,7 @@
 
   float am = 0.f;
   auto pool_item = [&](int tl, int it) __attribute__((always_inline)) {
+    if constexpr (U8) it = s3_opaque(it);
     const int b = tl / tpi, t2 = tl - b * tpi, pr = t2 / g.pool_tc, pc = t2 - pr * g.pool_tc;
     const int qd = it / C4, c4 = it - qd * C4, pi = qd / 7, pj = qd - 7 * pi;
     const int ph = 8 * pr + pi, pw = 7 * pc + pj;
@@ -136,6 +178,10 @@
   int tl = blockIdx.x;
   int prev = -1;
   load_patch(tl);
+  if constexpr (U8) {
+    __syncthreads();
+    convert_patch();
+  }
   store_patch();
   __syncthreads();
   for (; tl < ntiles; tl += G) {
@@ -190,6 +236,9 @@
         for (int q = 0; q < QI; ++q)
           if (ks == q * PS + PS / 2 && tid + q * NT < NPOOL) pool_item(prev, tid + q * NT);
       }
+      if constexpr (U8) {
+        if (ks == NKS - 1) convert_patch();
+      }
     }
     __syncthreads();
 #pragma unroll
@@ -215,12 +264,15 @@
   }
 }
 
-int launch_stem_pool_h2(rr_handle_s* h, const GemmArgs& g, hipStream_t s, int timer_cls) {
+int launch_stem_pool_h2(rr_handle_s* h, const GemmArgs& g, hipStream_t s, int timer_cls, const StemU8* u8) {
   if (g.N != 64 || g.Cin != 4 || g.K % 32 || g.K < g.KH * g.KW * 4 || g.relu != 1 || g.residual != nullptr ||
       g.col_scale == nullptr || g.a_amax == nullptr || g.pool_out == nullptr || g.POH <= 0 || g.POW <= 0 ||
       g.pool_tr != (g.POH + 7) / 8 || g.pool_tc != (g.POW + 6) / 7 || ((uintptr_t)g.A & 15) || (g.ldb & 7) ||
       (g.b_plane & 7) || ((uintptr_t)g.B & 15) || ((uintptr_t)g.col_scale & 15) || ((uintptr_t)g.pool_out & 15))
     return set_error(h, RR_EINVAL, "stem_pool_h2: NHWC4 input, 64 output channels, ReLU, aligned operands");
+  const bool halo = h->tune.s3_cfg != 7 && g.KH == 7 && g.KW == 7 && g.stride == 2 && g.pad == 3 && g.K == 224 && g.ldb == 224;
+  if (u8 != nullptr && (!halo || u8->img == nullptr))
+    return set_error(h, RR_EINVAL, "stem_pool_h2_u8: only the 7x7 / 2 pad-3 halo stem reads uint8 pixels");
   GemmArgs q = g;
   const long long tiles = (long long)(g.M / ((long long)g.OH * g.OW)) * g.pool_tr * g.pool_tc;
   if (tiles * 256 > 0x7fffffffLL) return set_error(h, RR_EINVAL, "stem_pool_h2: too many tiles");
@@ -229,9 +281,14 @@
   hipError_t e;
   {
     TimedLaunch tl(h, timer_cls, s);
-    if (h->tune.s3_cfg != 7 && g.KH == 7 && g.KW == 7 && g.stride == 2 && g.pad == 3 && g.K == 224 && g.ldb == 224) {
+    if (halo) {
       const int grid = (int)std::min<long long>(tiles, device_cu_count(h));
-      hipLaunchKernelGGL((stem_pool_halo_kernel<H2_EP | EP_RELU, 8, 2>), dim3((unsigned)grid), dim3(512), 0, s, g, (int)tiles);
+      if (u8 != nullptr)
+        hipLaunchKernelGGL((stem_pool_halo_kernel<H2_EP | EP_RELU, 8, 2, true>), dim3((unsigned)grid), dim3(512), 0, s, g,
+                           (int)tiles, *u8);
+      else
+        hipLaunchKernelGGL((stem_pool_halo_kernel<H2_EP | EP_RELU, 8, 2>), dim3((unsigned)grid), dim3(512), 0, s, g,
+                           (int)tiles, StemU8{});
       e = hipGetLastError();
     } else {
       e = launch_h2_tile_stem_pool(q, s, device_cu_count(h));
diff --git a/research_image_retrieval_amd/csrc/rr_api.hip b/research_image_retrieval_amd/csrc/rr_api.hip
--- a/research_image_retrieval_amd/csrc/rr_api.hip
+++ b/research_image_retrieval_amd/csrc/rr_api.hip
@@ -524,11 +524,11 @@
   return launch_gemm_s3(h, dense ? A_DENSE : (cin == 4 ? A_CONV_C4 : A_CONV), g, (hipStream_t)stream, kTimeGemm);
 }
 
-int rr_stem_pool_h2(rr_handle_t h, const float* x, const unsigned* x_amax, int b, int hgt, int wid, const void* w2,
-                    const float* w_iscale, const float* bias, int cout, int kh, int kw, int stride, int pad,
-                    float* y_pool, unsigned* y_amax, void* stream) {
-  RR_ENTRY(h);
-  if (!x || !x_amax || !w2 || !w_iscale || !y_pool || b < 0 || hgt <= 0 || wid <= 0 || kh <= 0 || kw <= 0 ||
+static int stem_pool_h2(rr_handle_t h, const float* x, const rr::StemU8* u8, const unsigned* x_amax, int b, int hgt,
+                        int wid, const void* w2, const float* w_iscale, const float* bias, int cout, int kh, int kw,
+                        int stride, int pad, float* y_pool, unsigned* y_amax, void* stream) {
+  RR_ENTRY(h);
+  if ((!x && !u8) || !x_amax || !w2 || !w_iscale || !y_pool || b < 0 || hgt <= 0 || wid <= 0 || kh <= 0 || kw <= 0 ||
       stride <= 0 || pad < 0)
     return set_error(h, RR_EINVAL, "rr_stem_pool_h2: bad argument");
   if (cout != 64) return set_error(h, RR_EINVAL, "rr_stem_pool_h2: cout must be 64");
@@ -568,7 +568,31 @@
   g.POW = pw;
   g.pool_tr = (ph + 7) / 8;
   g.pool_tc = (pw + 6) / 7;
-  return launch_stem_pool_h2(h, g, (hipStream_t)stream, kTimeGemm);
+  return launch_stem_pool_h2(h, g, (hipStream_t)stream, kTimeGemm, u8);
+}
+
+int rr_stem_pool_h2(rr_handle_t h, const float* x, const unsigned* x_amax, int b, int hgt, int wid, const void* w2,
+                    const float* w_iscale, const float* bias, int cout, int kh, int kw, int stride, int pad,
+                    float* y_pool, unsigned* y_amax, void* stream) {
+  if (h && !x) return set_error(h, RR_EINVAL, "rr_stem_pool_h2: bad argument");
+  return stem_pool_h2(h, x, nullptr, x_amax, b, hgt, wid, w2, w_iscale, bias, cout, kh, kw, stride, pad, y_pool, y_amax,
+                      stream);
+}
+
+int rr_stem_pool_h2_u8(rr_handle_t h, const uint8_t* img_nhwc, const float* mean3, const float* std3,
+                       const unsigned* x_amax, int b, int hgt, int wid, const void* w2, const float* w_iscale,
+                       const float* bias, int cout, int kh, int kw, int stride, int pad, float* y_pool,
+                       unsigned* y_amax, void* stream) {
+  if (!h) return RR_EINVAL;
+  if (!img_nhwc || !mean3 || !std3) return set_error(h, RR_EINVAL, "rr_stem_pool_h2_u8: bad argument");
+  if (cout != 64 || kh != 7 || kw != 7 || stride != 2 || pad != 3)
+    return set_error(h, RR_EINVAL, "rr_stem_pool_h2_u8: 7x7 / 2, pad 3, cout 64 only");
+  rr::StemU8 u8;
+  u8.img = img_nhwc;
+  for (int c = 0; c < 3; ++c) u8.mean[c] = mean3[c], u8.sdev[c] = std3[c];
+  u8.last_px = (long long)b * hgt * wid - 1;
+  return stem_pool_h2(h, nullptr, &u8, x_amax, b, hgt, wid, w2, w_iscale, bias, cout, kh, kw, stride, pad, y_pool,
+                      y_amax, stream);
 }
 
 int rr_bottleneck_out_h2(rr_handle_t h, const float* y, const unsigned* y_amax, int b, int oh, int ow, int planes,
@@ -632,6 +656,14 @@
   return launch_amax(h, x, n, amax, (hipStream_t)stream);
 }
 
+int rr_amax_u8_norm(rr_handle_t h, const uint8_t* img_nhwc, long long n_px, const float* mean3, const float* std3,
+                    unsigned* amax, void* stream) {
+  RR_ENTRY(h);
+  if (!img_nhwc || !mean3 || !std3 || !amax || n_px < 0) return set_error(h, RR_EINVAL, "rr_amax_u8_norm: bad argument");
+  TimedLaunch tl(h, kTimeElem, (hipStream_t)stream);
+  return launch_amax_u8_norm(h, img_nhwc, n_px, mean3, std3, amax, (hipStream_t)stream);
+}
+
 
 int rr_linear(rr_handle_t h, const float* x, int m, int k, const float* w, const float* bias, int n, float* y,
               void* stream) {
diff --git a/research_image_retrieval_amd/csrc/rr_internal.hpp b/research_image_retrieval_amd/csrc/rr_internal.hpp
--- a/research_image_retrieval_amd/csrc/rr_internal.hpp
+++ b/research_image_retrieval_amd/csrc/rr_internal.hpp
@@ -134,6 +134,14 @@
   const long long cap = (long long)((usable - off_cand) / ((size_t)nq * 8));
   return cap < worst ? cap : worst;
 }
+
+__device__ __forceinline__ float norm_u8(uint8_t u, float mean, float sdev) { return ((float)u / 255.0f - mean) / sdev; }
+
+struct StemU8 {
+  const uint8_t* img = nullptr;
+  float mean[3] = {0.f, 0.f, 0.f}, sdev[3] = {1.f, 1.f, 1.f};
+  long long last_px = -1;
+};
 
 enum AMode { A_DENSE = 0, A_CONV = 1, A_CONV_GENERIC = 2, A_CONV_C4 = 3 };
 enum EMode { E_STORE = 0, E_SCORES_T = 1, E_FILTER = 2 };
@@ -221,10 +229,12 @@
 bool h2_halo_2d_ok(const GemmArgs& g);
 hipError_t launch_h2_halo_2d(const GemmArgs& g, hipStream_t s);
 int launch_gemm_h2_seg2(rr_handle_s* h, const GemmArgs& g, hipStream_t s, int timer_cls);
-int launch_stem_pool_h2(rr_handle_s* h, const GemmArgs& g, hipStream_t s, int timer_cls);
+int launch_stem_pool_h2(rr_handle_s* h, const GemmArgs& g, hipStream_t s, int timer_cls, const StemU8* u8 = nullptr);
 int launch_split2h(rr_handle_s* h, const float* w, int rows, int k, int kpad, uint16_t* planes, float* iscale,
                    hipStream_t s);
 int launch_amax(rr_handle_s* h, const float* x, long long n, uint32_t* slots, hipStream_t s);
+int launch_amax_u8_norm(rr_handle_s* h, const uint8_t* img, long long n_px, const float* mean3, const float* std3,
+                        uint32_t* slots, hipStream_t s);
 
 bool gemm_8p_eligible(const GemmArgs& g, int dt);
 hipError_t launch_gemm_8p(const GemmArgs& g, int emode, hipStream_t s, int dt);
diff --git a/research_image_retrieval_amd/models.py b/research_image_retrieval_amd/models.py
--- a/research_image_retrieval_amd/models.py
+++ b/research_image_retrieval_amd/models.py
@@ -48,6 +48,9 @@
     def extract_features(self, x):
         return self.extract_features_nhwc(self._input(x))
 
+    def _takes_u8(self):
+        return self.backbone.takes_u8()
+
     def forward_test_nhwc(self, x_nhwc):
         f = self.extract_features_nhwc(x_nhwc)
         return ops.l2_normalize(f, EPS_L2, out=f)
@@ -83,6 +86,9 @@
                                  **kw)
         self.outputdim = feature_dim
 
+    def _takes_u8(self):
+        return self.backbone._takes_u8()
+
     def forward_test_nhwc(self, x_nhwc):
         return self.backbone.forward_test_nhwc(x_nhwc)
 
diff --git a/research_image_retrieval_amd/networks.py b/research_image_retrieval_amd/networks.py
--- a/research_image_retrieval_amd/networks.py
+++ b/research_image_retrieval_amd/networks.py
@@ -29,6 +29,7 @@
         self.layers = W.RESNET_LAYERS[name]
         self.conv_math = conv_math
         self.convs_h2 = {}
+        self.fuse_u8_stem = True
         if conv_math == "h2":
             self.convs_h2 = {k: ops.H2Conv(w) for k, (w, _) in self.convs.items()}
             self.fuse_downsample = True
@@ -44,12 +45,22 @@
         w, b = self.convs[name]
         return ops.conv2d(x, w, b, stride, pad, residual, relu)
 
+    def takes_u8(self):
+        if self.conv_math != "h2" or not (self.fuse_u8_stem and self.fuse_stem_pool):
+            return False
+        c1 = self.convs_h2["conv1"]
+        dev = self.device.index if self.device.index is not None else torch.cuda.current_device()
+        return (c1.cout, c1.kh, c1.kw) == (64, 7, 7) and ops.tuned(dev, "s3_cfg") != 7
+
     def _forward_h2(self, x, return_x3, hook=None, return_x3_amax=False):
         cv, h2 = self.convs, self.convs_h2
         hook = hook or (lambda i: None)
         rec = ops.amax_records(2 + 3 * sum(self.layers), x.device)
-        ops.amax_f32(x, rec[0])
-        if self.fuse_stem_pool and h2["conv1"].cout == 64:
+        u8 = x.dtype == torch.uint8
+        ops.amax_u8_norm(x, rec[0]) if u8 else ops.amax_f32(x, rec[0])
+        if u8:
+            x = ops.stem_pool_h2_u8(x, rec[0], h2["conv1"], cv["conv1"][1], 2, 3, rec[1])
+        elif self.fuse_stem_pool and h2["conv1"].cout == 64:
             x = ops.stem_pool_h2(x, rec[0], h2["conv1"], cv["conv1"][1], 2, 3, rec[1])
         else:
             x = ops.conv2d_h2(x, rec[0], h2["conv1"], cv["conv1"][1], 2, 3, None, True, rec[1])
@@ -82,6 +93,10 @@
         return (x3, x) if return_x3 else x
 
     def forward(self, x, return_x3=False, hook=None, return_x3_amax=False):
+        if x.dtype == torch.uint8:
+            if not self.takes_u8():
+                raise ValueError("ResNet.forward: this trunk has no uint8 stem (takes_u8); pass ops.preprocess_u8's image")
+            return self._forward_h2(x.contiguous(), return_x3, hook, return_x3_amax)
         if x.shape[-1] == 3:
             x = torch.nn.functional.pad(x, (0, 1))
         if self.conv_math == "h2":
@@ -139,13 +154,19 @@
     def forward_test_nhwc(self, x_nhwc):
         raise NotImplementedError
 
+    def _takes_u8(self):
+        return False
+
+    def _input_u8(self, img_nhwc_u8):
+        return img_nhwc_u8 if self._takes_u8() else ops.preprocess_u8(img_nhwc_u8, out_c=self.in_channels)
+
     @torch.no_grad()
     def forward_test(self, x):
         return self.forward_test_nhwc(self._input(x))
 
     @torch.no_grad()
     def forward_test_u8(self, img_nhwc_u8):
-        return self.forward_test_nhwc(ops.preprocess_u8(img_nhwc_u8, out_c=self.in_channels))
+        return self.forward_test_nhwc(self._input_u8(img_nhwc_u8))
 
     @torch.no_grad()
     def forward_test_u8_streams(self, img_nhwc_u8, streams, lag=1):
@@ -169,8 +190,7 @@
                     ev.record(s)
 
             with torch.cuda.stream(s):
-                f = self.forward_test_nhwc(ops.preprocess_u8(x[cuts[i]:cuts[i + 1]], out_c=self.in_channels),
-                                           hook=hook)
+                f = self.forward_test_nhwc(self._input_u8(x[cuts[i]:cuts[i + 1]]), hook=hook)
             outs.append(f)
             gate = ev
         if not outs:
@@ -202,6 +222,9 @@
         self.whiten_w = ww.float().contiguous().to(self.device)
         self.whiten_b = wb.float().contiguous().to(self.device)
         self.outputdim = outputdim
+
+    def _takes_u8(self):
+        return self.backbone.takes_u8()
 
     def forward_test_nhwc(self, x_nhwc, hook=None):
         f = self.backbone(x_nhwc, hook=hook)
@@ -249,6 +272,9 @@
             y = ops.conv2d(x3, self.conv1_w, self.conv1_b, 1, 0, None, False)
         return ops.dolg_local_pool(y, self.conv2_w, self.conv2_b)
 
+    def _takes_u8(self):
+        return self.globalmodel.takes_u8()
+
     def forward_test_nhwc(self, x_nhwc, hook=None):
         if self.conv_math == "h2":
             x3, x4, x3a = self.globalmodel(x_nhwc, return_x3=True, hook=hook, return_x3_amax=True)
@@ -314,6 +340,9 @@
         self.net = net
         self.pcaw = pcaw
         self.outputdim = pcaw.dim
+
+    def _takes_u8(self):
+        return self.net._takes_u8()
 
     def forward_test_nhwc(self, x_nhwc, hook=None):
         f = self.net.forward_test_nhwc(x_nhwc, hook=hook)
diff --git a/research_image_retrieval_amd/ops.py b/research_image_retrieval_amd/ops.py
--- a/research_image_retrieval_amd/ops.py
+++ b/research_image_retrieval_amd/ops.py
@@ -94,6 +94,29 @@
     dev = _dev(x)
     hd = _lib.handle(dev)
     _lib.check(_lib.lib().rr_amax_f32(hd, _ptr(x), x.numel(), _ptr(record), _stream(dev)), hd, "rr_amax_f32")
+    return record
+
+
+IMAGENET_MEAN, IMAGENET_STD = (0.485, 0.456, 0.406), (0.229, 0.224, 0.225)
+
+
+def _u8_image(img_nhwc, name):
+    if img_nhwc.dtype != torch.uint8 or img_nhwc.dim() != 4 or img_nhwc.shape[3] != 3:
+        raise ValueError(f"{name}: expected uint8 [B,H,W,3]")
+    return img_nhwc.contiguous()
+
+
+def amax_u8_norm(img_nhwc, record, mean=IMAGENET_MEAN, std=IMAGENET_STD):
+    img_nhwc = _u8_image(img_nhwc, "amax_u8_norm")
+    if record.dtype != torch.int32 or record.numel() != AMAX_SLOTS or not record.is_contiguous():
+        raise ValueError("amax_u8_norm: record must be contiguous int32 [RR_AMAX_SLOTS]")
+    dev = _dev(img_nhwc)
+    m = (ctypes.c_float * 3)(*mean)
+    s = (ctypes.c_float * 3)(*std)
+    hd = _lib.handle(dev)
+    _lib.check(_lib.lib().rr_amax_u8_norm(hd, _ptr(img_nhwc), img_nhwc.numel() // 3, ctypes.cast(m, ctypes.c_void_p),
+                                          ctypes.cast(s, ctypes.c_void_p), _ptr(record), _stream(dev)),
+               hd, "rr_amax_u8_norm")
     return record
 
 
@@ -174,6 +197,27 @@
     _lib.check(_lib.lib().rr_stem_pool_h2(hd, _ptr(x), _ptr(x_amax), b, h, wd, _ptr(wc.planes), _ptr(wc.iscale),
                                           _ptr(bias), 64, wc.kh, wc.kw, stride, pad, _ptr(y), _ptr(y_amax),
                                           _stream(dev)), hd, "rr_stem_pool_h2")
+    return y
+
+
+def stem_pool_h2_u8(img_nhwc, x_amax, wc, bias, stride=2, pad=3, y_amax=None, mean=IMAGENET_MEAN, std=IMAGENET_STD):
+    img_nhwc = _u8_image(img_nhwc, "stem_pool_h2_u8")
+    if not isinstance(wc, H2Conv) or wc.cin != 4:
+        raise TypeError("stem_pool_h2_u8: wc must be an ops.H2Conv with Cin 4")
+    dev = _dev(img_nhwc)
+    b, h, wd, _ = img_nhwc.shape
+    oh = (h + 2 * pad - wc.kh) // stride + 1
+    ow = (wd + 2 * pad - wc.kw) // stride + 1
+    y = torch.empty((b, (oh - 1) // 2 + 1, (ow - 1) // 2 + 1, wc.cout), dtype=torch.float32, device=img_nhwc.device)
+    if bias is not None:
+        _f32(bias, "stem_pool_h2_u8 bias")
+    m = (ctypes.c_float * 3)(*mean)
+    s = (ctypes.c_float * 3)(*std)
+    hd = _lib.handle(dev)
+    _lib.check(_lib.lib().rr_stem_pool_h2_u8(hd, _ptr(img_nhwc), ctypes.cast(m, ctypes.c_void_p),
+                                             ctypes.cast(s, ctypes.c_void_p), _ptr(x_amax), b, h, wd, _ptr(wc.planes),
+                                             _ptr(wc.iscale), _ptr(bias), wc.cout, wc.kh, wc.kw, stride, pad, _ptr(y),
+                                             _ptr(y_amax), _stream(dev)), hd, "rr_stem_pool_h2_u8")
     return y
 
 
@@ -418,12 +462,23 @@
     def __enter__(self):
         for k, v in self.kw.items():
             _lib.check(_lib.lib().rr_set_tuning(self.h, _TUNE_KEYS[k], int(v)), self.h, "rr_set_tuning")
+            _TUNE_FORCED[(self.h, k)] = int(v)
         return self
 
     def __exit__(self, *exc):
         for k in self.kw:
             _lib.lib().rr_set_tuning(self.h, _TUNE_KEYS[k], _TUNE_DEFAULT.get(k, 0))
+            _TUNE_FORCED.pop((self.h, k), None)
         return False
+
+
+_TUNE_FORCED = {}
+
+
+def tuned(device_index, key):
+    if key not in _TUNE_KEYS:
+        raise ValueError(f"unknown tuning key {key!r}")
+    return _TUNE_FORCED.get((_lib.handle(device_index), key), _TUNE_DEFAULT.get(key, 0))
 
 
 class KernelTimer:
```

New measurement: 16810 (median of 6 runs). No clear change (+0.5%).
